# bobzhangbo2012/gnss-sdr-new

Hardware: AMD Instinct MI355X
Metric: IQ Msamples/s processed (acq+track), 32 PRN × 81 Doppler; % HBM roofline (higher is better)
Workload: dtype f32; 1 GPU; C2: GPS L1 C/A 4 Msps; per 1 ms block a 32 PRN x 81 Doppler (+-10 kHz, 250 Hz) CFAR PCPS grid + closed-loop DLL/PLL tracking (3-tap E-P-L, dll_pll_veml_tracking) of 8 channels over the same span; fs_sps=4000000, fft_size=4000, prns=32, doppler_bins=81, channels=8, taps=3, item_type=gr_complex, tracking=one continuous stream, one launch per timed region, acq_chains=2, acq_stagger=0, acq_input=each step acquires its own span of the continuous stream (new HBM addresses), carrier=exact, forward_spectra_per_block=4

## Files before the change

gnss-sdr-new_amd/csrc/acq.hip:

```cpp
#include <algorithm>
#include <cmath>
#include <cstring>
#include <memory>
#include <new>
#include <utility>

#include "acq_handle.h"
#include "acq_plans.h"
#include "gsdr_stream_internal.h"

using namespace gsdr_acq_impl;

namespace
{

int dispatch(gsdr_acq* a, const AcqView& v, const AcqOp& op)
{
    if (a->variant >= 20) return dispatch_four(a, v, op);
    if (a->variant >= 10) return dispatch_runtime(a, v, op);
    return dispatch_static(a, v, op);
}

int run_blocks(gsdr_acq* a, const AcqView& v, const void* iq, uint32_t nblocks, uint64_t stride, uint64_t stamp0,
    gsdr_acq_result* res, hipStream_t s)
// ... 226 lines not shown
{
    if (!a) return;
    gsdr::DeviceGuard g(a->device);
    if (a->stream) (void)hipStreamSynchronize(a->stream);
    for (auto& r : a->prof_recs)
        {
            (void)hipEventDestroy(r.a);
            (void)hipEventDestroy(r.b);
        }
    for (hipEvent_t e : a->prof_pool) (void)hipEventDestroy(e);
    for (int i = 0; i < gsdr_acq::kSubs; ++i)
        {
            if (a->sub_done[i]) (void)hipEventDestroy(a->sub_done[i]);
            if (a->h_res[i]) (void)hipHostFree(a->h_res[i]);
        }
    void* bufs[] = {a->st2.d_wipe, a->st2.d_freq, a->d_tw, a->d_wipe, a->d_code_fft, a->d_code_lane, a->d_code_stage, a->d_prn, a->d_X, a->d_stats, a->d_res,
        a->d_iq, a->d_grid, a->d_rowbuf, a->d_keys, a->d_psum, a->d_fscratch, a->d_dgrid, a->d_tw_sub, a->d_scratch, a->d_slots, a->d_resk, a->d_acc, a->d_acc_slots};
    for (void* p : bufs)
        if (p) (void)hipFree(p);
    if (a->stream) (void)hipStreamDestroy(a->stream);
    delete a;
}

int gsdr_acq_get_dims(const gsdr_acq* a, uint32_t* D, uint32_t* N)
{
    GSDR_REQUIRE(a, GSDR_E_ARG, "gsdr_acq_get_dims: null handle");
    if (D) *D = a->D;
    if (N) *N = a->N;
    return GSDR_OK;
}

int gsdr_acq_get_plan(const gsdr_acq* a, int32_t* variant, int32_t* nthreads, int32_t* r1, int32_t* nstages,
    int32_t radix[8])
{
    GSDR_REQUIRE(a, GSDR_E_ARG, "gsdr_acq_get_plan: null handle");
    static_assert(gsdr::fft::kMaxStages == 8, "gsdr_acq_get_plan reports 8 radices");
    const bool four = a->variant >= 20;
    const Plan& p = four ? a->plan4.sub : a->plan;
    if (variant) *variant = a->variant;
    if (nthreads) *nthreads = a->nt;
    if (r1) *r1 = four ? a->plan4.r1 : 0;
    if (nstages) *nstages = p.nstages;
    if (radix)
        for (int i = 0; i < gsdr::fft::kMaxStages; ++i) radix[i] = i < p.nstages ? p.radix[i] : 1;
    return GSDR_OK;
}

int gsdr_acq_get_split(const gsdr_acq* a, int32_t* split)
{
    GSDR_REQUIRE(a && split, GSDR_E_ARG, "gsdr_acq_get_split: null argument");
    *split = a->split;
    return GSDR_OK;
}

int gsdr_acq_set_local_codes(gsdr_acq* a, const float* codes, const uint32_t* prn, uint32_t nprn)
{
    GSDR_REQUIRE(a && codes && prn, GSDR_E_ARG, "gsdr_acq_set_local_codes: null argument");
    GSDR_REQUIRE(nprn > 0 && nprn <= a->conf.max_prns, GSDR_E_ARG, "gsdr_acq_set_local_codes: nprn %u outside [1,%u]",
        nprn, a->conf.max_prns);
    std::lock_guard<std::mutex> lk(a->mu);
    gsdr::DeviceGuard g(a->device);
    GSDR_HIP(hipMemcpyAsync(a->d_code_stage, codes, (size_t)nprn * a->consumed * sizeof(float2),
        hipMemcpyHostToDevice, a->stream));
    GSDR_HIP(hipMemcpyAsync(a->d_prn, prn, nprn * sizeof(uint32_t), hipMemcpyHostToDevice, a->stream));
    int rc = code_fft(a, 0, nprn);
    if (rc != GSDR_OK) return rc;
    GSDR_HIP(hipStreamSynchronize(a->stream));
    a->nprn = nprn;
    return GSDR_OK;
}

int gsdr_acq_set_local_code(gsdr_acq* a, uint32_t slot, const float* code, uint32_t prn)
{
    GSDR_REQUIRE(a && code, GSDR_E_ARG, "gsdr_acq_set_local_code: null argument");
    GSDR_REQUIRE(slot < a->conf.max_prns, GSDR_E_ARG, "gsdr_acq_set_local_code: slot %u outside [0,%u)",
        slot, a->conf.max_prns);
    std::lock_guard<std::mutex> lk(a->mu);
    gsdr::DeviceGuard g(a->device);
    GSDR_HIP(hipMemcpyAsync(a->d_code_stage + (size_t)slot * a->consumed, code, (size_t)a->consumed * sizeof(float2),
        hipMemcpyHostToDevice, a->stream));
    GSDR_HIP(hipMemcpyAsync(a->d_prn + slot, &prn, sizeof(uint32_t), hipMemcpyHostToDevice, a->stream));
    int rc = code_fft(a, slot, 1);
    if (rc != GSDR_OK) return rc;
    GSDR_HIP(hipStreamSynchronize(a->stream));
    if (a->nprn <= slot) a->nprn = slot + 1;
    return GSDR_OK;
}

int gsdr_acq_set_active_prns(gsdr_acq* a, uint32_t nprn)
{
    GSDR_REQUIRE(a, GSDR_E_ARG, "gsdr_acq_set_active_prns: null handle");
    GSDR_REQUIRE(nprn > 0 && nprn <= a->conf.max_prns, GSDR_E_ARG, "gsdr_acq_set_active_prns: %u outside [1,%u]", nprn,
        a->conf.max_prns);
    std::lock_guard<std::mutex> lk(a->mu);
    a->nprn = nprn;
    return GSDR_OK;
}

int gsdr_acq_set_doppler(gsdr_acq* a, int32_t doppler_max, uint32_t doppler_step, int32_t doppler_center)
{
    GSDR_REQUIRE(a, GSDR_E_ARG, "gsdr_acq_set_doppler: null handle");
    GSDR_REQUIRE(doppler_step > 0, GSDR_E_ARG, "gsdr_acq_set_doppler: doppler_step must be > 0");
    std::lock_guard<std::mutex> lk(a->mu);
    gsdr::DeviceGuard g(a->device);
    const uint32_t D = (uint32_t)std::ceil((double)(doppler_max - (-doppler_max)) / (double)doppler_step);
    GSDR_REQUIRE(a->conf.num_doppler_bins != 0 || D == a->D, GSDR_E_UNSUPPORTED,
        "gsdr_acq_set_doppler: changing the number of Doppler bins (%u -> %u) requires a new handle", a->D, D);
    a->conf.doppler_max = doppler_max;
    a->conf.doppler_step = doppler_step;
    a->conf.doppler_center = doppler_center;
    int rc = rebuild_wipeoffs(a);
    if (rc != GSDR_OK) return rc;
    compute_threshold(a);
    return GSDR_OK;
}

int gsdr_acq_set_wipeoff(gsdr_acq* a, int mode)
{
    GSDR_REQUIRE(a, GSDR_E_ARG, "gsdr_acq_set_wipeoff: null handle");
    GSDR_REQUIRE(mode == GSDR_WIPE_EXACT || mode == GSDR_WIPE_GENERIC || mode == GSDR_WIPE_AVX2, GSDR_E_ARG,
        "gsdr_acq_set_wipeoff: unknown mode %d", mode);
    std::lock_guard<std::mutex> lk(a->mu);
    gsdr::DeviceGuard g(a->device);
    a->wipe_mode = mode;
    return rebuild_wipeoffs(a);
}

int gsdr_acq_get_spectrum_reuse(const gsdr_acq* a, uint32_t* q, uint32_t* p)
{
    GSDR_REQUIRE(a, GSDR_E_ARG, "gsdr_acq_get_spectrum_reuse: null handle");
    if (q) *q = a->xm.q;
    if (p) *p = a->xm.p;
    return GSDR_OK;
}

int gsdr_acq_set_threshold(gsdr_acq* a, float threshold)
{
    GSDR_REQUIRE(a, GSDR_E_ARG, "gsdr_acq_set_threshold: null handle");
    a->threshold = threshold;
    return GSDR_OK;
}

int gsdr_acq_get_threshold(const gsdr_acq* a, float* threshold)
{
    GSDR_REQUIRE(a && threshold, GSDR_E_ARG, "gsdr_acq_get_threshold: null argument");
    *threshold = a->threshold;
    return GSDR_OK;
}

int gsdr_acq_run_device(gsdr_acq* a, const void* iq_dev, uint32_t nblocks, uint64_t stride, uint64_t stamp0,
    gsdr_acq_result* out_dev, void* stream)
{
    GSDR_REQUIRE(a && iq_dev && out_dev, GSDR_E_ARG, "gsdr_acq_run_device: null argument");
    GSDR_REQUIRE(a->nprn > 0, GSDR_E_STATE, "gsdr_acq_run_device: set_local_codes first");
    GSDR_REQUIRE(nblocks > 0 && nblocks <= a->conf.max_blocks, GSDR_E_ARG, "gsdr_acq_run_device: nblocks %u outside [1,%u]",
        nblocks, a->conf.max_blocks);
    GSDR_REQUIRE(stride >= a->consumed || nblocks == 1, GSDR_E_ARG, "gsdr_acq_run_device: block stride %llu < consumed %u",
        (unsigned long long)stride, a->consumed);
    std::lock_guard<std::mutex> lk(a->mu);
    gsdr::DeviceGuard g(a->device);
    hipStream_t s = stream ? (hipStream_t)stream : a->stream;
    return run_blocks(a, view_of(a), iq_dev, nblocks, stride, stamp0, out_dev, s);
}

int gsdr_acq_run(gsdr_acq* a, const void* iq_host, uint32_t nblocks, uint64_t stamp0, gsdr_acq_result* out)
{
    GSDR_REQUIRE(a && iq_host && out, GSDR_E_ARG, "gsdr_acq_run: null argument");
    GSDR_REQUIRE(a->nprn > 0, GSDR_E_STATE, "gsdr_acq_run: set_local_codes first");
    GSDR_REQUIRE(nblocks > 0 && nblocks <= a->conf.max_blocks, GSDR_E_ARG, "gsdr_acq_run: nblocks %u outside [1,%u]",
        nblocks, a->conf.max_blocks);
    std::lock_guard<std::mutex> lk(a->mu);
    gsdr::DeviceGuard g(a->device);
    const size_t bytes = (size_t)nblocks * a->K * a->consumed * gsdr::item_bytes(a->conf.item_type);
    GSDR_HIP(hipMemcpyAsync(a->d_iq, iq_host, bytes, hipMemcpyHostToDevice, a->stream));
    int rc = run_blocks(a, view_of(a), a->d_iq, nblocks, a->consumed, stamp0, a->d_res, a->stream);
    if (rc != GSDR_OK) return rc;
    return read_results(a, out, (size_t)nblocks * a->nprn);
}

int gsdr_acq_run_stream(gsdr_acq* a, gsdr_stream* ring, uint64_t first_sample, uint32_t nblocks, uint64_t stamp0,
    gsdr_acq_result* out)
{
    GSDR_REQUIRE(a && ring && out, GSDR_E_ARG, "gsdr_acq_run_stream: null argument");
    GSDR_REQUIRE(a->nprn > 0, GSDR_E_STATE, "gsdr_acq_run_stream: set_local_codes first");
    GSDR_REQUIRE(nblocks > 0 && nblocks <= a->conf.max_blocks, GSDR_E_ARG,
        "gsdr_acq_run_stream: nblocks %u outside [1,%u]", nblocks, a->conf.max_blocks);
    GSDR_REQUIRE(gsdr::stream_item_type(ring) == a->conf.item_type, GSDR_E_ARG,
        "gsdr_acq_run_stream: ring item type %d != acquisition item type %d", gsdr::stream_item_type(ring),
        a->conf.item_type);
    GSDR_REQUIRE(gsdr::stream_device(ring) == a->device, GSDR_E_ARG,
        "gsdr_acq_run_stream: ring on device %d, acquisition handle on device %d", gsdr::stream_device(ring), a->device);
    std::lock_guard<std::mutex> lk(a->mu);
    gsdr::DeviceGuard g(a->device);
    int rc = run_ring(a, ring, first_sample, nblocks, stamp0);
    if (rc != GSDR_OK) return rc;
    return read_results(a, out, (size_t)nblocks * a->nprn);
}

int gsdr_acq_submit_stream(gsdr_acq* a, gsdr_stream* ring, uint64_t first_sample, uint32_t nblocks, uint64_t stamp0)
{
    GSDR_REQUIRE(a && ring, GSDR_E_ARG, "gsdr_acq_submit_stream: null argument");
    GSDR_REQUIRE(a->nprn > 0, GSDR_E_STATE, "gsdr_acq_submit_stream: set_local_codes first");
    GSDR_REQUIRE(nblocks > 0 && nblocks <= a->conf.max_blocks, GSDR_E_ARG,
        "gsdr_acq_submit_stream: nblocks %u outside [1,%u]", nblocks, a->conf.max_blocks);
    GSDR_REQUIRE(gsdr::stream_item_type(ring) == a->conf.item_type, GSDR_E_ARG,
        "gsdr_acq_submit_stream: ring item type %d != acquisition item type %d", gsdr::stream_item_type(ring),
        a->conf.item_type);
    GSDR_REQUIRE(gsdr::stream_device(ring) == a->device, GSDR_E_ARG,
        "gsdr_acq_submit_stream: ring on device %d, acquisition handle on device %d", gsdr::stream_device(ring), a->device);
    std::lock_guard<std::mutex> lk(a->mu);
    GSDR_REQUIRE(a->sub_count < gsdr_acq::kSubs, GSDR_E_STATE,
        "gsdr_acq_submit_stream: %d submissions in flight, collect the oldest first", gsdr_acq::kSubs);
    gsdr::DeviceGuard g(a->device);
    const int slot = (a->sub_head + a->sub_count) % gsdr_acq::kSubs;
    if (!a->h_res[slot])
        {
            GSDR_HIP(hipHostMalloc(&a->h_res[slot],
                (size_t)a->conf.max_blocks * a->conf.max_prns * sizeof(gsdr_acq_result), hipHostMallocDefault));
            GSDR_HIP(hipEventCreateWithFlags(&a->sub_done[slot], hipEventDisableTiming));
        }
    int rc = run_ring(a, ring, first_sample, nblocks, stamp0);
    if (rc != GSDR_OK) return rc;
    GSDR_HIP(hipMemcpyAsync(a->h_res[slot], a->d_res, (size_t)nblocks * a->nprn * sizeof(gsdr_acq_result),
        hipMemcpyDeviceToHost, a->stream));
    GSDR_HIP(hipEventRecord(a->sub_done[slot], a->stream));
    a->sub_blocks[slot] = nblocks;
    a->sub_nprn[slot] = a->nprn;
    a->sub_count++;
    return GSDR_OK;
}

int gsdr_acq_collect(gsdr_acq* a, gsdr_acq_result* out, uint32_t* nblocks, uint32_t* nprn)
{
    GSDR_REQUIRE(a && out, GSDR_E_ARG, "gsdr_acq_collect: null argument");
    std::lock_guard<std::mutex> lk(a->mu);
    GSDR_REQUIRE(a->sub_count > 0, GSDR_E_STATE, "gsdr_acq_collect: nothing submitted");
    gsdr::DeviceGuard g(a->device);
    const int slot = a->sub_head;
    a->sub_head = (a->sub_head + 1) % gsdr_acq::kSubs;
    a->sub_count--;
    GSDR_HIP(hipEventSynchronize(a->sub_done[slot]));
    std::memcpy(out, a->h_res[slot], (size_t)a->sub_blocks[slot] * a->sub_nprn[slot] * sizeof(gsdr_acq_result));
    if (nblocks) *nblocks = a->sub_blocks[slot];
    if (nprn) *nprn = a->sub_nprn[slot];
    return GSDR_OK;
}

int gsdr_acq_run_dwell(gsdr_acq* a, const void* iq_host, uint32_t dwell, uint64_t stamp, gsdr_acq_result* out)
{
    GSDR_REQUIRE(a && iq_host && out, GSDR_E_ARG, "gsdr_acq_run_dwell: null argument");
    GSDR_REQUIRE(a->nprn > 0, GSDR_E_STATE, "gsdr_acq_run_dwell: set_local_codes first");
    GSDR_REQUIRE(dwell < a->conf.max_dwells, GSDR_E_ARG, "gsdr_acq_run_dwell: dwell %u outside [0,%u)", dwell,
        a->conf.max_dwells);
    std::lock_guard<std::mutex> lk(a->mu);
    gsdr::DeviceGuard g(a->device);
    if (!a->d_dgrid)
        GSDR_HIP(hipMalloc(&a->d_dgrid, (size_t)a->conf.max_prns * a->D * a->eff * sizeof(float)));
    GSDR_HIP(hipMemcpyAsync(a->d_iq, iq_host, (size_t)a->consumed * gsdr::item_bytes(a->conf.item_type),
        hipMemcpyHostToDevice, a->stream));
    AcqOp op{AcqOp::Dwell};
    op.dwell = dwell;
    op.stamp0 = stamp;
    op.res = a->d_res;
    op.s = a->stream;
    int rc = dispatch(a, view_of(a), op);
    if (rc != GSDR_OK) return rc;
    return read_results(a, out, a->nprn);
}

int gsdr_acq_dump_spectra(gsdr_acq* a, const void* iq_host, float* spectra_host)
{
    GSDR_REQUIRE(a && iq_host && spectra_host, GSDR_E_ARG, "gsdr_acq_dump_spectra: null argument");
    std::lock_guard<std::mutex> lk(a->mu);
    gsdr::DeviceGuard g(a->device);
    GSDR_HIP(hipMemcpyAsync(a->d_iq, iq_host, (size_t)a->consumed * gsdr::item_bytes(a->conf.item_type),
        hipMemcpyHostToDevice, a->stream));
    int rc = dispatch(a, view_of(a), AcqOp{AcqOp::DumpSpectra});
    if (rc != GSDR_OK) return rc;
    for (uint32_t d = 0; d < a->D; ++d)
        GSDR_HIP(hipMemcpyAsync(spectra_host + (size_t)d * a->N * 2, a->d_X + a->xm.off(0, d),
            (size_t)a->N * sizeof(float2), hipMemcpyDeviceToHost, a->stream));
    GSDR_HIP(hipStreamSynchronize(a->stream));
    return GSDR_OK;
}

int gsdr_acq_dump_grid(gsdr_acq* a, const void* iq_host, uint32_t prn_slot, float* grid_host)
{
    GSDR_REQUIRE(a && iq_host && grid_host, GSDR_E_ARG, "gsdr_acq_dump_grid: null argument");
    GSDR_REQUIRE(prn_slot < a->nprn, GSDR_E_ARG, "gsdr_acq_dump_grid: prn_slot %u >= nprn %u", prn_slot, a->nprn);
    std::lock_guard<std::mutex> lk(a->mu);
    gsdr::DeviceGuard g(a->device);
    GSDR_HIP(hipMemcpyAsync(a->d_iq, iq_host, (size_t)a->consumed * gsdr::item_bytes(a->conf.item_type),
        hipMemcpyHostToDevice, a->stream));
    AcqOp op{AcqOp::DumpGrid};
    op.prn_slot = prn_slot;
    int rc = dispatch(a, view_of(a), op);
    if (rc != GSDR_OK) return rc;
    GSDR_HIP(hipMemcpyAsync(grid_host, a->d_grid, (size_t)a->D * a->N * sizeof(float), hipMemcpyDeviceToHost,
        a->stream));
    GSDR_HIP(hipStreamSynchronize(a->stream));
    return GSDR_OK;
}

int gsdr_acq_dump_grid_step_two(gsdr_acq* a, const void* iq_host, uint32_t prn_slot, float doppler_center_hz,
    float* grid_host)
{
    GSDR_REQUIRE(a && iq_host && grid_host, GSDR_E_ARG, "gsdr_acq_dump_grid_step_two: null argument");
    GSDR_REQUIRE(prn_slot < a->nprn, GSDR_E_ARG, "gsdr_acq_dump_grid_step_two: prn_slot %u >= nprn %u", prn_slot,
        a->nprn);
    GSDR_REQUIRE(a->st2.nbins > 0, GSDR_E_STATE, "gsdr_acq_dump_grid_step_two: gsdr_acq_set_step_two first");
    GSDR_REQUIRE(a->st2.nbins <= a->D, GSDR_E_UNSUPPORTED,
        "gsdr_acq_dump_grid_step_two: %u narrow bins exceed the grid buffer's %u rows", a->st2.nbins, a->D);
    std::lock_guard<std::mutex> lk(a->mu);
    gsdr::DeviceGuard g(a->device);
    const uint32_t nb = a->st2.nbins;
    std::vector<float> freqs(nb);
    step_two_freqs(a, doppler_center_hz, freqs.data());
    GSDR_HIP(hipMemcpyAsync(a->d_iq, iq_host, (size_t)a->consumed * gsdr::item_bytes(a->conf.item_type),
        hipMemcpyHostToDevice, a->stream));
    GSDR_HIP(hipMemcpyAsync(a->st2.d_freq, freqs.data(), nb * sizeof(float), hipMemcpyHostToDevice, a->stream));
    int rc = launch_wipeoff(a, a->st2.d_wipe, nb, a->st2.d_freq);
    if (rc != GSDR_OK) return rc;
    AcqView v = view_of(a);
    v.D = nb;
    v.nprn = 1;
    v.wipe = a->st2.d_wipe;
    v.code_fft = a->d_code_fft + (size_t)prn_slot * a->N;
    v.code_lane = a->d_code_lane ? a->d_code_lane + (size_t)prn_slot * a->N : nullptr;
    v.xm = XMap{nb, 0u, a->N};
    rc = dispatch(a, v, AcqOp{AcqOp::DumpGrid});
    if (rc != GSDR_OK) return rc;
    GSDR_HIP(hipMemcpyAsync(grid_host, a->d_grid, (size_t)nb * a->N * sizeof(float), hipMemcpyDeviceToHost,
        a->stream));
    GSDR_HIP(hipStreamSynchronize(a->stream));
    return GSDR_OK;
}

int gsdr_acq_set_step_two(gsdr_acq* a, uint32_t num_doppler_bins_step2, float doppler_step2, float pfa2)
{
    GSDR_REQUIRE(a, GSDR_E_ARG, "gsdr_acq_set_step_two: null handle");
    GSDR_REQUIRE(num_doppler_bins_step2 > 0, GSDR_E_ARG, "gsdr_acq_set_step_two: zero bins");
    GSDR_REQUIRE(num_doppler_bins_step2 <= a->D * a->conf.max_blocks, GSDR_E_UNSUPPORTED,
        "gsdr_acq_set_step_two: %u bins exceed the handle's spectrum capacity (%u bins x %u blocks)",
        num_doppler_bins_step2, a->D, a->conf.max_blocks);
    std::lock_guard<std::mutex> lk(a->mu);
    gsdr::DeviceGuard g(a->device);
    GSDR_HIP(hipStreamSynchronize(a->stream));
    if (a->st2.d_wipe) (void)hipFree(a->st2.d_wipe);
    if (a->st2.d_freq) (void)hipFree(a->st2.d_freq);
    a->st2.d_wipe = nullptr;
    a->st2.d_freq = nullptr;
    const size_t rows = (size_t)a->conf.max_prns * num_doppler_bins_step2;
    GSDR_HIP(hipMalloc(&a->st2.d_wipe, rows * a->N * sizeof(float2)));
    GSDR_HIP(hipMalloc(&a->st2.d_freq, rows * sizeof(float)));
    a->st2.nbins = num_doppler_bins_step2;
    a->st2.step = doppler_step2;
    a->st2.pfa2 = (pfa2 <= 0.0f || pfa2 > 1.0f) ? a->conf.pfa : pfa2;
    return GSDR_OK;
}

int gsdr_acq_get_step_two_threshold(const gsdr_acq* a, float* threshold)
{
    GSDR_REQUIRE(a && threshold, GSDR_E_ARG, "gsdr_acq_get_step_two_threshold: null argument");
    GSDR_REQUIRE(a->st2.nbins > 0, GSDR_E_STATE, "gsdr_acq_get_step_two_threshold: gsdr_acq_set_step_two first");
    *threshold = step_two_threshold(a);
    return GSDR_OK;
}

int gsdr_acq_run_step_two(gsdr_acq* a, const void* iq_host, uint32_t nsel, const uint32_t* prn_slots,
    const float* doppler_center_hz, const float* coarse_input_power, uint64_t stamp, gsdr_acq_result* out)
{
    GSDR_REQUIRE(a && iq_host && prn_slots && doppler_center_hz && coarse_input_power && out, GSDR_E_ARG,
        "gsdr_acq_run_step_two: null argument");
    GSDR_REQUIRE(a->st2.nbins > 0, GSDR_E_STATE, "gsdr_acq_run_step_two: gsdr_acq_set_step_two first");
    GSDR_REQUIRE(nsel > 0 && nsel <= a->nprn, GSDR_E_ARG, "gsdr_acq_run_step_two: %u PRNs outside [1,%u]", nsel,
        a->nprn);
    for (uint32_t i = 0; i < nsel; ++i)
        GSDR_REQUIRE(prn_slots[i] < a->nprn, GSDR_E_ARG, "gsdr_acq_run_step_two: slot %u >= nprn %u", prn_slots[i],
            a->nprn);
    std::lock_guard<std::mutex> lk(a->mu);
    gsdr::DeviceGuard g(a->device);
    const uint32_t nb = a->st2.nbins;
    std::vector<float> freqs((size_t)nsel * nb);
    for (uint32_t i = 0; i < nsel; ++i) step_two_freqs(a, doppler_center_hz[i], freqs.data() + (size_t)i * nb);
    GSDR_HIP(hipMemcpyAsync(a->d_iq, iq_host, (size_t)a->K * a->consumed * gsdr::item_bytes(a->conf.item_type),
        hipMemcpyHostToDevice, a->stream));
    GSDR_HIP(hipMemcpyAsync(a->st2.d_freq, freqs.data(), freqs.size() * sizeof(float), hipMemcpyHostToDevice,
        a->stream));
    int rc = launch_wipeoff(a, a->st2.d_wipe, nsel * nb, a->st2.d_freq);
    const float thr = step_two_threshold(a);
    for (uint32_t i = 0; i < nsel && rc == GSDR_OK; ++i)
        {
            const AcqView v{nb, 1, a->st2.d_wipe + (size_t)i * nb * a->N, a->d_code_fft + (size_t)prn_slots[i] * a->N,
                a->d_code_lane ? a->d_code_lane + (size_t)prn_slots[i] * a->N : nullptr, a->d_prn + prn_slots[i], XMap{nb, 0u, a->N}, true, doppler_center_hz[i], coarse_input_power[i], thr};
            rc = run_blocks(a, v, a->d_iq, 1, a->consumed, stamp, a->d_res + i, a->stream);
        }
    if (rc != GSDR_OK) return rc;
    return read_results(a, out, nsel);
}

int gsdr_acq_set_cu_mask(gsdr_acq* a, const uint32_t* mask, int n_words)
{
    GSDR_REQUIRE(a, GSDR_E_ARG, "gsdr_acq_set_cu_mask: null handle");
    std::lock_guard<std::mutex> lk(a->mu);
    gsdr::DeviceGuard g(a->device);
    return gsdr::replace_stream(&a->stream, mask, n_words);
}

int gsdr_acq_set_profiling(gsdr_acq* a, int enable)
{
    GSDR_REQUIRE(a, GSDR_E_ARG, "gsdr_acq_set_profiling: null handle");
    std::lock_guard<std::mutex> lk(a->mu);
    a->profiling = enable != 0;
    if (a->profiling)
        {
            gsdr::DeviceGuard g(a->device);
            while (a->prof_pool.size() + 2 * a->prof_recs.size() < 1024)
                {
                    hipEvent_t e = nullptr;
                    if (hipEventCreate(&e) != hipSuccess) break;
                    a->prof_pool.push_back(e);
                }
        }
    return GSDR_OK;
}

int gsdr_acq_read_profile_ex(gsdr_acq* a, double* stage_ms, uint32_t* launches, double* stage_busy_ms)
{
    GSDR_REQUIRE(a && stage_ms && launches, GSDR_E_ARG, "gsdr_acq_read_profile: null argument");
    std::lock_guard<std::mutex> lk(a->mu);
    gsdr::DeviceGuard g(a->device);
    for (int i = 0; i < 4; ++i)
        {
            stage_ms[i] = 0.0;
            launches[i] = 0;
            if (stage_busy_ms) stage_busy_ms[i] = 0.0;
        }
    std::vector<std::pair<double, double>> iv[4];
    hipEvent_t ref = a->prof_recs.empty() ? nullptr : a->prof_recs.front().a;
    for (auto& r : a->prof_recs)
        {
            GSDR_HIP(hipEventSynchronize(r.b));
            float ms = 0.0f, t0 = 0.0f, t1 = 0.0f;
            GSDR_HIP(hipEventElapsedTime(&ms, r.a, r.b));
            GSDR_HIP(hipEventElapsedTime(&t0, ref, r.a));
            GSDR_HIP(hipEventElapsedTime(&t1, ref, r.b));
            stage_ms[r.stage] += ms;
            launches[r.stage] += 1;
            iv[r.stage].emplace_back(t0, t1);
        }
    if (stage_busy_ms)
        for (int i = 0; i < 4; ++i)
            {
                std::sort(iv[i].begin(), iv[i].end());
                double busy = 0.0, lo = 0.0, hi = -1e300;
                for (const auto& x : iv[i])
                    {
                        if (x.first > hi)
                            {
                                if (hi > lo) busy += hi - lo;
                                lo = x.first;
                                hi = x.second;
                            }
                        else if (x.second > hi)
                            hi = x.second;
                    }
                if (hi > lo) busy += hi - lo;
                stage_busy_ms[i] = busy;
            }
    for (auto& r : a->prof_recs)
        {
            a->prof_pool.push_back(r.a);
            a->prof_pool.push_back(r.b);
        }
    a->prof_recs.clear();
    return GSDR_OK;
}

int gsdr_acq_read_profile_intervals(gsdr_acq* a, const void* ref_event, int stage, double* start_ms, double* end_ms,
    uint32_t max_n, uint32_t* n)
{
    GSDR_REQUIRE(a && ref_event && n && (max_n == 0 || (start_ms && end_ms)), GSDR_E_ARG,
        "gsdr_acq_read_profile_intervals: null argument");
    GSDR_REQUIRE(stage >= 0 && stage < 4, GSDR_E_ARG, "gsdr_acq_read_profile_intervals: stage %d", stage);
    std::lock_guard<std::mutex> lk(a->mu);
    gsdr::DeviceGuard g(a->device);
    hipEvent_t ref = (hipEvent_t)const_cast<void*>(ref_event);
    uint32_t k = 0;
    for (auto& r : a->prof_recs)
        {
            if (r.stage != stage) continue;
            if (k < max_n)
                {
                    GSDR_HIP(hipEventSynchronize(r.b));
                    float t0 = 0.0f, t1 = 0.0f;
                    GSDR_HIP(hipEventElapsedTime(&t0, ref, r.a));
                    GSDR_HIP(hipEventElapsedTime(&t1, ref, r.b));
                    start_ms[k] = t0;
                    end_ms[k] = t1;
                }
            ++k;
        }
    *n = k;
    return GSDR_OK;
}

int gsdr_acq_read_profile(gsdr_acq* a, double* stage_ms, uint32_t* launches)
{
    return gsdr_acq_read_profile_ex(a, stage_ms, launches, nullptr);
}

}
```

gnss-sdr-new_amd/csrc/acq_common.hip:

```cpp
#include <cmath>
#include <cstdlib>
#include <string>

#include "acq_handle.h"

namespace
{

__device__ __forceinline__ float2 cephes_sincos_avx2(float x0)
{
    const float FOPI = 1.27323954473516f;
    const float DP1 = -0.78515625f, DP2 = -2.4187564849853515625e-4f, DP3 = -3.77489497744594108e-8f;
    const float C0 = 2.443315711809948E-005f, C1 = -1.388731625493765E-003f, C2 = 4.166664568298827E-002f;
    const float S0 = -1.9515295891E-4f, S1 = 8.3321608736E-3f, S2 = -1.6666654611E-1f;
    const uint32_t bits = __float_as_uint(x0);
    bool sign_sin = (bits >> 31) != 0;
    float x = __uint_as_float(bits & 0x7fffffffu);
    float y = __fmul_rn(x, FOPI);
    int32_t j = (int32_t)y;
    j = (j + 1) & ~1;
    y = (float)j;
    const bool swap = (j & 4) != 0;
    const bool poly = (j & 2) == 0;
    x = __fadd_rn(x, __fmul_rn(y, DP1));
    x = __fadd_rn(x, __fmul_rn(y, DP2));
    x = __fadd_rn(x, __fmul_rn(y, DP3));
    const bool sign_cos = ((~(j - 2)) & 4) != 0;
    sign_sin = sign_sin != swap;
    const float z = __fmul_rn(x, x);
    float yc = __fmul_rn(C0, z);
    yc = __fadd_rn(yc, C1);
    yc = __fmul_rn(yc, z);
    yc = __fadd_rn(yc, C2);
    yc = __fmul_rn(yc, z);
    yc = __fmul_rn(yc, z);
    yc = __fsub_rn(yc, __fmul_rn(z, 0.5f));
    yc = __fadd_rn(yc, 1.0f);
    float ys = __fmul_rn(S0, z);
    ys = __fadd_rn(ys, S1);
    ys = __fmul_rn(ys, z);
    ys = __fadd_rn(ys, S2);
    ys = __fmul_rn(ys, z);
    ys = __fmul_rn(ys, x);
    ys = __fadd_rn(ys, x);
    const float sv = poly ? ys : yc, cv = poly ? yc : ys;
    return make_float2(sign_cos ? -cv : cv, sign_sin ? -sv : sv);
}

__global__ void __launch_bounds__(256) acq_wipeoff_kernel(float2* __restrict__ wipe, uint32_t N, float fs,
    int32_t doppler_max, int32_t doppler_center, int32_t doppler_step, int32_t doppler_bias,
    const float* __restrict__ freqs, int mode)
{
    const uint32_t d = blockIdx.x;
    float2* row = wipe + (size_t)d * N;
    const int32_t doppler = -doppler_max + doppler_center + doppler_step * (int32_t)d;
    const float freq = freqs ? freqs[d] : (float)(doppler_bias + doppler);
    if (mode == GSDR_WIPE_EXACT)
        {
            for (uint32_t i = threadIdx.x; i < N; i += blockDim.x)
                {
                    const double t = (double)freq * (double)i / (double)fs;
                    double s, c;
                    sincos(-6.283185307179586 * (t - floor(t)), &s, &c);
                    row[i] = make_float2((float)c, (float)s);
                }
            return;
        }
    const float phase_step = __fdiv_rn(__fmul_rn(6.283185307179586f, freq), fs);
    const float inc = -phase_step;
    if (mode == GSDR_WIPE_AVX2)
        {
            const uint32_t iters = N / 8;
            if (threadIdx.x < 8)
                {
                    const uint32_t k = threadIdx.x;
                    float ph = k == 0 ? 0.0f : __fmul_rn((float)k, inc);
                    const float inc8 = __fmul_rn(8.0f, inc);
                    for (uint32_t it = 0; it < iters; ++it)
                        {
                            row[8 * it + k].x = ph;
                            ph = __fadd_rn(ph, inc8);
                        }
                }
            else if (threadIdx.x == 8)
                {
                    float ph = __fmul_rn(inc, (float)(iters * 8));
                    for (uint32_t i = iters * 8; i < N; ++i)
                        {
                            row[i].x = ph;
                            ph = __fadd_rn(ph, inc);
                        }
                }
            __syncthreads();
            for (uint32_t i = threadIdx.x; i < N; i += blockDim.x)
                {
                    if (i < iters * 8)
                        row[i] = cephes_sincos_avx2(row[i].x);
                    else
                        {
                            float s, c;
                            sincosf(row[i].x, &s, &c);
                            row[i] = make_float2(c, s);
                        }
                }
            return;
        }
    if (threadIdx.x == 0)
        {
            float ph = 0.0f;
            for (uint32_t i = 0; i < N; ++i)
                {
                    row[i].x = ph;
                    ph = __fadd_rn(ph, inc);
                }
        }
    __syncthreads();
    for (uint32_t i = threadIdx.x; i < N; i += blockDim.x)
        {
            float s, c;
            sincosf(row[i].x, &s, &c);
            row[i] = make_float2(c, s);
        }
}

__global__ void __launch_bounds__(64) acq_reduce_dwell_kernel(const RowStat* __restrict__ stats,
    gsdr_acq_result* __restrict__ resk, gsdr_acq_result* __restrict__ res, const uint32_t* __restrict__ prn_ids,
    AcqParams ap, uint64_t stamp0, uint64_t block_stride)
{
    const uint32_t bp = blockIdx.x;
    const uint32_t b = bp / ap.P, p = bp - b * ap.P;
    const uint32_t K = ap.dwells;
    bool done = false;
    for (uint32_t k = 0; k < K && !done; ++k)
        {
            const RowStat* s = stats + ((size_t)bp * K + k) * ap.D;
            float m = -1.0f;
            uint32_t dsel = 0xffffffffu, tsel = 0;
            for (uint32_t d = threadIdx.x; d < ap.D; d += 64)
                {
                    RowStat r = s[d];
                    if (r.max > m)
                        {
                            m = r.max;
                            dsel = d;
                            tsel = r.idx;
                        }
                }
#pragma unroll
            for (int off = 32; off > 0; off >>= 1)
                {
                    float om = __shfl_xor(m, off);
                    uint32_t od = __shfl_xor(dsel, off);
                    uint32_t ot = __shfl_xor(tsel, off);
                    if (stat_better(om, od, m, dsel))
                        {
                            m = om;
                            dsel = od;
                            tsel = ot;
                        }
                }
            gsdr_acq_result r;
            r.prn = prn_ids[p];
            r.doppler_index = dsel;
            r.code_phase = tsel;
            r.doppler_hz = doppler_of(ap, dsel);
            r.peak = m;
            r.second_peak = 0.0f;
            r.input_power = 0.0f;
            r.test_statistic = 0.0f;
            r.acq_delay_samples = (double)fmodf((float)tsel, ap.samples_per_code);
            r.samplestamp = stamp0 + (uint64_t)(b * K + k) * block_stride;
            r.positive = 0;
            r.num_dwells = (int32_t)(k + 1);
            if (ap.cfar)
                {
                    const uint32_t opp = (dsel + ap.D / 2) % ap.D;
                    const float acc = s[opp].sum;
                    const float ip = ap.step_two ? ap.ip2
                                                 : (float)((double)(acc / (float)(int32_t)ap.eff) / 2.0 / (double)(k + 1));
                    r.input_power = ip;
                    r.test_statistic = m / ip;
                    r.positive = r.test_statistic > ap.threshold ? 1 : 0;
                    done = r.positive || k + 1 == K;
                    if (done && threadIdx.x == 0) res[bp] = r;
                }
            if (threadIdx.x == 0) resk[(size_t)bp * K + k] = r;
        }
}

__global__ void acq_decide_kernel(const gsdr_acq_result* __restrict__ resk, gsdr_acq_result* __restrict__ res,
    uint32_t K, uint32_t n)
{
    const uint32_t bp = blockIdx.x * blockDim.x + threadIdx.x;
    if (bp >= n) return;
    uint32_t k = 0;
    while (k + 1 < K && !resk[(size_t)bp * K + k].positive) ++k;
    res[bp] = resk[(size_t)bp * K + k];
}

__global__ void __launch_bounds__(256) acq_code_lane_order_kernel(const float2* __restrict__ src,
    float2* __restrict__ dst, uint32_t N, int nb1, int r1)
{
    const float2* in = src + (size_t)blockIdx.x * N;
    float2* out = dst + (size_t)blockIdx.x * N;
    for (uint32_t i = threadIdx.x; i < N; i += blockDim.x) out[lane_order_slot((int)i, nb1, r1)] = in[i];
}

__global__ void __launch_bounds__(256) acq_grid_second_peak_kernel(const float* __restrict__ grid,
    gsdr_acq_result* __restrict__ res, AcqParams ap)
{
    __shared__ RowStat scratch[4];
    const uint32_t p = blockIdx.x;
    const uint32_t d = res[p].doppler_index;
    const int32_t ti = (int32_t)res[p].code_phase;
    const int32_t E = (int32_t)ap.N;
    int32_t e1 = ti - (int32_t)ap.samples_per_chip;
    int32_t e2 = ti + (int32_t)ap.samples_per_chip;
    if (e1 < 0)
        e1 = E + e1;
    else if (e2 >= E)
        e2 = e2 - E;
    const float* row = grid + ((size_t)p * ap.D + d) * ap.eff;
    float best = 0.0f, sum = 0.0f;
    uint32_t bidx = 0;
    for (uint32_t j = threadIdx.x; j < ap.eff; j += 256)
        {
            const int32_t jj = (int32_t)j;
            const bool excluded = (e1 < e2) ? (jj >= e1 && jj < e2) : (jj >= e1 || jj < e2);
            const float m = excluded ? 0.0f : row[j];
            if (stat_better(m, j, best, bidx))
                {
                    best = m;
                    bidx = j;
                }
        }
    block_reduce_stat<256>(best, bidx, sum, scratch);
    if (threadIdx.x == 0)
        {
            gsdr_acq_result r = res[p];
            r.second_peak = best;
            r.test_statistic = r.peak / best;
            r.positive = r.test_statistic > ap.threshold ? 1 : 0;
            res[p] = r;
        }
}

__global__ void __launch_bounds__(64) acq_reduce_kernel(const RowStat* __restrict__ stats,
    gsdr_acq_result* __restrict__ res, const uint32_t* __restrict__ prn_ids, AcqParams ap, uint64_t stamp0,
    uint64_t block_stride)
{
    const uint32_t bp = blockIdx.x;
    const uint32_t b = bp / ap.P, p = bp - b * ap.P;
    const RowStat* s = stats + (size_t)bp * ap.D;
    float m = -1.0f;
    uint32_t dsel = 0xffffffffu, tsel = 0;
    for (uint32_t d = threadIdx.x; d < ap.D; d += 64)
        {
            RowStat r = s[d];
            if (r.max > m)
                {
                    m = r.max;
                    dsel = d;
                    tsel = r.idx;
                }
        }
#pragma unroll
    for (int off = 32; off > 0; off >>= 1)
        {
            float om = __shfl_xor(m, off);
            uint32_t od = __shfl_xor(dsel, off);
            uint32_t ot = __shfl_xor(tsel, off);
            if (stat_better(om, od, m, dsel))
                {
                    m = om;
                    dsel = od;
                    tsel = ot;
                }
        }
    if (threadIdx.x != 0) return;
    gsdr_acq_result r;
    r.prn = prn_ids[p];
    r.doppler_index = dsel;
    r.code_phase = tsel;
    r.doppler_hz = doppler_of(ap, dsel);
    r.peak = m;
    r.second_peak = 0.0f;
    r.input_power = 0.0f;
    r.test_statistic = 0.0f;
    r.acq_delay_samples = (double)fmodf((float)tsel, ap.samples_per_code);
    r.samplestamp = stamp0 + (uint64_t)b * block_stride;
    r.positive = 0;
    r.num_dwells = (int32_t)ap.counter;
    if (ap.cfar)
        {
            const uint32_t opp = (dsel + ap.D / 2) % ap.D;
            const float acc = s[opp].sum;
            const float ip =
                ap.step_two ? ap.ip2 : (float)((double)(acc / (float)(int32_t)ap.eff) / 2.0 / (double)ap.counter);
            r.input_power = ip;
            r.test_statistic = m / ip;
            r.positive = r.test_statistic > ap.threshold ? 1 : 0;
        }
    res[bp] = r;
}

int env_int(const char* name, int dflt)
{
    const char* e = std::getenv(name);
    return e ? std::atoi(e) : dflt;
}

}

namespace gsdr_acq_impl
{

#ifndef GSDR_ACQ_PPW_DEFAULT
#define GSDR_ACQ_PPW_DEFAULT 1
#endif
#ifndef GSDR_ACQ_QPW_DEFAULT
#define GSDR_ACQ_QPW_DEFAULT 2
#endif

AcqEnv read_acq_env()
{
    AcqEnv e;
    if (const char* w = std::getenv("GSDR_ACQ_WIPE"))
        {
            const std::string m(w);
            e.wipe_mode = m == "generic" ? GSDR_WIPE_GENERIC : (m == "avx2" ? GSDR_WIPE_AVX2 : GSDR_WIPE_EXACT);
        }
    e.xshift = env_int("GSDR_ACQ_XSHIFT", 1) != 0;
    e.four_generic = env_int("GSDR_ACQ_FOUR_GENERIC", 0) != 0;
    e.split = env_int("GSDR_ACQ_SPLIT", 1) != 0;
    e.split_arg = env_int("GSDR_ACQ_SPLIT_ARG", 1) != 0;
    e.qpw = env_int("GSDR_ACQ_QPW", GSDR_ACQ_QPW_DEFAULT);
    e.ppw = env_int("GSDR_ACQ_PPW", GSDR_ACQ_PPW_DEFAULT);
    e.corr_variant = env_int("GSDR_ACQ_CORR_VARIANT", -1);
    return e;
}

AcqView view_of(const gsdr_acq* a)
{
    return AcqView{a->D, a->nprn, a->d_wipe, a->d_code_fft, a->d_code_lane, a->d_prn, a->xm, false, 0.0f, 0.0f, 0.0f};
}

AcqParams params_of(const gsdr_acq* a, const AcqView& v)
{
    AcqParams ap{};
    ap.xm = v.xm;
    ap.N = a->N;
    ap.consumed = a->consumed;
    ap.lead_zeros = a->lead;
    ap.D = v.D;
    ap.P = v.nprn;
    ap.doppler_max = a->conf.doppler_max;
    ap.doppler_center = a->conf.doppler_center;
    ap.doppler_step = (int32_t)a->conf.doppler_step;
    ap.samples_per_code = a->conf.samples_per_code;
    ap.samples_per_chip = a->conf.samples_per_chip;
    ap.dwells = a->K;
    ap.threshold = a->threshold;
    ap.cfar = a->conf.pfa > 0.0f ? 1 : 0;
    ap.eff = a->eff;
    ap.out_off = a->N - a->eff;
    ap.counter = a->K;
    if (v.step_two)
        {
            ap.step_two = 1;
            ap.center2 = v.center2;
            ap.step2 = a->st2.step;
            ap.half2 = (float)std::floor((double)a->st2.nbins / 2.0);
            ap.ip2 = v.ip2;
            ap.threshold = v.threshold2;
        }
    return ap;
}

static XMap grid_xmap(const gsdr_acq* a)
{
    XMap plain{a->D, 0u, a->N};
    if (a->wipe_mode != GSDR_WIPE_EXACT || !a->env.xshift) return plain;
    const int64_t fs = a->conf.fs_in;
    if (fs <= 0) return plain;
    int64_t num = (int64_t)a->conf.doppler_step * (int64_t)a->N, den = fs;
    int64_t g0 = num, g1 = den;
    while (g1)
        {
            const int64_t t = g0 % g1;
            g0 = g1;
            g1 = t;
        }
    if (g0 <= 0) return plain;
    const int64_t p = num / g0, q = den / g0;
    if (q < 1 || 2 * q > (int64_t)a->D) return plain;
    const int64_t ext = ((int64_t)(a->D - 1) / q) * p;
    if (ext > (int64_t)a->N) return plain;
    if (q * ((int64_t)a->N + ext) > (int64_t)a->D * (int64_t)a->N) return plain;
    return XMap{(uint32_t)q, (uint32_t)p, (uint32_t)(a->N + ext)};
}

int launch_wipeoff(gsdr_acq* a, float2* wipe, uint32_t rows, const float* freqs)
{
    const gsdr_acq_conf& c = a->conf;
    const bool g = !freqs;
    hipLaunchKernelGGL(acq_wipeoff_kernel, dim3(rows), dim3(256), 0, a->stream, wipe, a->N, (float)c.fs_in,
        g ? c.doppler_max : 0, g ? c.doppler_center : 0, g ? (int32_t)c.doppler_step : 0, g ? c.doppler_bias : 0, freqs,
        a->wipe_mode);
    GSDR_HIP(hipGetLastError());
    return GSDR_OK;
}

int rebuild_wipeoffs(gsdr_acq* a)
{
    a->xm = grid_xmap(a);
    const int rc = launch_wipeoff(a, a->d_wipe, a->xm.q, nullptr);
    if (rc != GSDR_OK) return rc;
    GSDR_HIP(hipStreamSynchronize(a->stream));
    return GSDR_OK;
}

int launch_reduce(gsdr_acq* a, const AcqParams& ap, bool dwells, uint32_t nblocks, gsdr_acq_result* res,
    const uint32_t* prn, uint64_t stamp0, uint64_t stride, hipStream_t s)
{
    if (dwells)
        hipLaunchKernelGGL(acq_reduce_dwell_kernel, dim3(nblocks * ap.P), dim3(64), 0, s, a->d_stats, a->d_resk, res,
            prn, ap, stamp0, stride);
    else
        hipLaunchKernelGGL(acq_reduce_kernel, dim3(nblocks * ap.P), dim3(64), 0, s, a->d_stats, res, prn, ap, stamp0,
            stride);
    GSDR_HIP(hipGetLastError());
    return GSDR_OK;
}

int launch_decide(gsdr_acq* a, uint32_t n, gsdr_acq_result* res, hipStream_t s)
{
    hipLaunchKernelGGL(acq_decide_kernel, dim3((n + 255) / 256), dim3(256), 0, s, a->d_resk, res, a->K, n);
    GSDR_HIP(hipGetLastError());
    return GSDR_OK;
}

int launch_code_lane_order(gsdr_acq* a, uint32_t first_slot, uint32_t nslots)
{
    const size_t off = (size_t)first_slot * a->N;
    hipLaunchKernelGGL(acq_code_lane_order_kernel, dim3(nslots), dim3(256), 0, a->stream, a->d_code_fft + off,
        a->d_code_lane + off, a->N, a->lane_nb1, a->lane_r1);
    GSDR_HIP(hipGetLastError());
    return GSDR_OK;
}

int launch_grid_second_peak(gsdr_acq* a, const AcqParams& ap, gsdr_acq_result* res, hipStream_t s)
{
    hipLaunchKernelGGL(acq_grid_second_peak_kernel, dim3(ap.P), dim3(256), 0, s, a->d_dgrid, res, ap);
    GSDR_HIP(hipGetLastError());
    return GSDR_OK;
}

void compute_threshold(gsdr_acq* a)
{
    const float pfa = a->conf.pfa;
    if (pfa <= 0.0f) return;
    const int num_bins = (int)(a->eff * a->D);
    const double p = std::pow(1.0 - (double)pfa, 1.0 / (double)(float)num_bins);
    a->threshold = (float)(2.0 * gsdr::gamma_p_inv_int(2 * (int)a->conf.max_dwells, p));
}

float step_two_threshold(const gsdr_acq* a)
{
    const float pfa = a->st2.pfa2;
    if (pfa <= 0.0f) return a->threshold;
    const int num_bins = (int)(a->eff * a->st2.nbins);
    const double p = std::pow(1.0 - (double)pfa, 1.0 / (double)(float)num_bins);
    return (float)(2.0 * gsdr::gamma_p_inv_int(2 * (int)a->conf.max_dwells, p));
}

}
```

gnss-sdr-new_amd/csrc/acq_handle.h:

```cpp
#pragma once
#include <mutex>
#include <type_traits>
#include <vector>

#include "acq_kernels.h"

struct AcqEnv
{
    int wipe_mode{GSDR_WIPE_EXACT};
    bool xshift{true}, four_generic{false}, split{true}, split_arg{true};
    int qpw{0}, ppw{0};
    int corr_variant{-1};
};

struct gsdr_acq
{
    int device{0};
    gsdr_acq_conf conf{};
    AcqEnv env{};
    uint32_t N{0}, D{0}, consumed{0}, lead{0};
    uint32_t K{1};
    int wipe_mode{GSDR_WIPE_EXACT};
    gsdr_acq_impl::XMap xm{};
    uint32_t eff{0};
    bool general{false};
    gsdr_acq_result* d_resk{nullptr};
    float* d_acc{nullptr};
    uint32_t* d_acc_slots{nullptr};
    int acc_words{0};
    float threshold{0.0f};
    int nt{256};
    int variant{0};
    int corr_variant{0};
    int split{0};
    int corr_stat{0};
    size_t corr_lds_bytes{0};
    int lane_nb1{0}, lane_r1{0};
    gsdr::fft::Plan plan{};
    gsdr::fft::Plan4 plan4{};
    size_t lds_bytes{0};
    hipStream_t stream{nullptr};
    float2* d_tw{nullptr};
    float2* d_wipe{nullptr};
    float2* d_code_fft{nullptr};
    float2* d_code_lane{nullptr};
    float2* d_code_stage{nullptr};
    uint32_t* d_prn{nullptr};
    uint32_t nprn{0};
    float2* d_X{nullptr};
    gsdr_acq_impl::RowStat* d_stats{nullptr};
    gsdr_acq_result* d_res{nullptr};
    static constexpr int kSubs = 2;
    gsdr_acq_result* h_res[kSubs]{};
    hipEvent_t sub_done[kSubs]{};
    uint32_t sub_blocks[kSubs]{}, sub_nprn[kSubs]{};
    int sub_head{0}, sub_count{0};
    void* d_iq{nullptr};
    float* d_grid{nullptr};
    float* d_rowbuf{nullptr};
    unsigned long long* d_keys{nullptr};
    float* d_psum{nullptr};
    float2* d_fscratch{nullptr};
    float* d_dgrid{nullptr};
    float2* d_tw_sub{nullptr};
    float2* d_scratch{nullptr};
    uint32_t* d_slots{nullptr};
    struct ProfRec
    {
        hipEvent_t a, b;
        int stage;
    };
    bool profiling{false};
    std::vector<ProfRec> prof_recs;
    std::vector<hipEvent_t> prof_pool;
    struct StepTwo
    {
        uint32_t nbins{0};
        float step{0.0f};
        float pfa2{0.0f};
        float2* d_wipe{nullptr};
        float* d_freq{nullptr};
    } st2;
    std::mutex mu;
};

namespace gsdr_acq_impl
{

struct AcqView
{
    uint32_t D, nprn;
    const float2* wipe;
    const float2* code_fft;
    const float2* code_lane;
    const uint32_t* prn;
    XMap xm;
    bool step_two;
    float center2, ip2, threshold2;
};

struct AcqOp
{
    enum Kind
    {
        Run,
        CodeFft,
        DumpSpectra,
        DumpGrid,
        SetAttrs,
        Dwell
    } kind;
    const void* iq{nullptr};
    uint32_t nblocks{0};
    uint64_t stride{0}, stamp0{0};
    gsdr_acq_result* res{nullptr};
    hipStream_t s{nullptr};
    uint32_t first_slot{0}, nslots{0}, prn_slot{0}, dwell{0};
};

inline int default_pk_variant(uint32_t N)
{
    switch (N)
        {
        case 4000: return 99;
        case 16000: return 94;
        case 8000: return 61;
        case 2000: return 62;
        default: return 0;
        }
}

template <class F>
auto with_item_type(int it, F&& f)
{
    if (it == GSDR_ITEM_GR_COMPLEX) return f(std::integral_constant<int, GSDR_ITEM_GR_COMPLEX>{});
    if (it == GSDR_ITEM_CSHORT) return f(std::integral_constant<int, GSDR_ITEM_CSHORT>{});
    return f(std::integral_constant<int, GSDR_ITEM_IBYTE>{});
}
constexpr int kItemTypes[] = {GSDR_ITEM_GR_COMPLEX, GSDR_ITEM_CSHORT, GSDR_ITEM_IBYTE};

inline int set_max_lds(const void* kernel, size_t bytes)
{
    GSDR_HIP(hipFuncSetAttribute(kernel, hipFuncAttributeMaxDynamicSharedMemorySize, (int)bytes));
    return GSDR_OK;
}

AcqEnv read_acq_env();
AcqView view_of(const gsdr_acq* a);
AcqParams params_of(const gsdr_acq* a, const AcqView& v);
int rebuild_wipeoffs(gsdr_acq* a);
void compute_threshold(gsdr_acq* a);
float step_two_threshold(const gsdr_acq* a);
int launch_wipeoff(gsdr_acq* a, float2* wipe, uint32_t rows, const float* freqs);
int launch_reduce(gsdr_acq* a, const AcqParams& ap, bool dwells, uint32_t nblocks, gsdr_acq_result* res,
    const uint32_t* prn, uint64_t stamp0, uint64_t stride, hipStream_t s);
int launch_decide(gsdr_acq* a, uint32_t n, gsdr_acq_result* res, hipStream_t s);
int launch_grid_second_peak(gsdr_acq* a, const AcqParams& ap, gsdr_acq_result* res, hipStream_t s);
int launch_code_lane_order(gsdr_acq* a, uint32_t first_slot, uint32_t nslots);

int launch_corr_variant(gsdr_acq* a, const AcqView& v, uint32_t nblocks, hipStream_t s);
int launch_argmax_variant(gsdr_acq* a, const AcqView& v, uint32_t nblocks, gsdr_acq_result* res, hipStream_t s);
int launch_forward_pk(gsdr_acq* a, const AcqView& v, const void* iq, uint32_t nblocks, uint64_t stride, hipStream_t s);
int setup_corr_variant(gsdr_acq* a, int id);
int setup_split(gsdr_acq* a);
int launch_split(gsdr_acq* a, const AcqView& v, uint32_t nblocks, hipStream_t s);
int launch_split_argmax(gsdr_acq* a, const AcqView& v, uint32_t nblocks, gsdr_acq_result* res, hipStream_t s);
int dispatch_static(gsdr_acq* a, const AcqView& v, const AcqOp& op);
int dispatch_runtime(gsdr_acq* a, const AcqView& v, const AcqOp& op);
int dispatch_four(gsdr_acq* a, const AcqView& v, const AcqOp& op);

}
```

gnss-sdr-new_amd/csrc/acq_kernels.h:

```cpp
#pragma once
#include <hip/hip_runtime.h>

#include <type_traits>

#include "fft_4step.h"
#include "fft_lds.h"
#include "fft_multi.h"
#include "fft_pk.h"
#include "fft_plan.h"
#include "gsdr_internal.h"

namespace gsdr_acq_impl
{

struct RowStat
{
    float max;
    uint32_t idx;
    float sum;
    uint32_t pad;
};

struct XMap
{
// ... 3 lines not shown
    __host__ __device__ __forceinline__ size_t off(uint32_t bk, uint32_t d) const
    {
        const uint32_t a = d / q, c = d - a * q;
        return ((size_t)bk * q + c) * stride + (size_t)a * p;
    }
};

struct AcqParams
{
    XMap xm;
    uint32_t N;
    uint32_t consumed;
    uint32_t lead_zeros;
    uint32_t D;
    uint32_t P;
    int32_t doppler_max;
    int32_t doppler_center;
    int32_t doppler_step;
    float samples_per_code;
    uint32_t samples_per_chip;
    uint32_t dwells;
    float threshold;
    int32_t cfar;
    uint32_t eff;
    uint32_t out_off;
    int32_t step_two;
    float center2;
    float step2;
    float half2;
    float ip2;
    uint32_t counter;
};

}

namespace
{

using gsdr::fft::Plan;
using gsdr_acq_impl::AcqParams;
using gsdr_acq_impl::RowStat;
using gsdr_acq_impl::XMap;

__device__ __forceinline__ int32_t doppler_of(const AcqParams& ap, uint32_t d)
{
    if (ap.step_two) return (int32_t)gsdr::add_rn(ap.center2, gsdr::mul_rn(gsdr::sub_rn((float)d, ap.half2), ap.step2));
    return -ap.doppler_max + ap.doppler_center + ap.doppler_step * (int32_t)d;
}

template <int IT>
__device__ __forceinline__ float2 load_item(const void* __restrict__ p, size_t i)
{
    if constexpr (IT == GSDR_ITEM_GR_COMPLEX)
        {
            return reinterpret_cast<const float2*>(p)[i];
        }
    else if constexpr (IT == GSDR_ITEM_CSHORT)
        {
            short2 s = reinterpret_cast<const short2*>(p)[i];
            return make_float2((float)s.x, (float)s.y);
        }
    else
        {
            char2 s = reinterpret_cast<const char2*>(p)[i];
            return make_float2((float)s.x, (float)s.y);
        }
}

__device__ __forceinline__ bool stat_better(float am, uint32_t ai, float bm, uint32_t bi)
{
    return am > bm || (am == bm && ai < bi);
}

template <int NT>
__device__ __forceinline__ void block_reduce_stat(float& m, uint32_t& idx, float& sum, RowStat* scratch)
{
#pragma unroll
    for (int off = 32; off > 0; off >>= 1)
        {
            float om = __shfl_xor(m, off);
            uint32_t oi = __shfl_xor(idx, off);
            float os = __shfl_xor(sum, off);
            if (stat_better(om, oi, m, idx))
                {
                    m = om;
                    idx = oi;
                }
            sum += os;
        }
    constexpr int NW = NT / 64;
    const int lane = threadIdx.x & 63, wave = threadIdx.x >> 6;
    if (NW > 1)
        {
            if (lane == 0) scratch[wave] = RowStat{m, idx, sum, 0};
            __syncthreads();
            if (threadIdx.x == 0)
                {
                    for (int w = 1; w < NW; ++w)
                        {
                            RowStat s = scratch[w];
                            if (stat_better(s.max, s.idx, m, idx))
                                {
                                    m = s.max;
                                    idx = s.idx;
                                }
                            sum += s.sum;
                        }
                }
        }
}

template <class PT>
__global__ void __launch_bounds__(PT::NT) acq_code_fft_kernel(const float2* __restrict__ codes,
    float2* __restrict__ code_fft, const float2* __restrict__ tw, typename PT::PlanT plan, uint32_t consumed, uint32_t lead)
{
    extern __shared__ float2 lds[];
    const uint32_t p = blockIdx.x;
    const float2* c = codes + (size_t)p * consumed;
    float2* out = code_fft + (size_t)p * plan.n;
    const int valid = (int)plan.n - (int)lead;
    auto load = [&](int i) -> float2 {
        int k = i - (int)lead;
        return (k >= 0 && k < valid) ? c[k] : make_float2(0.f, 0.f);
    };
    auto store = [&](int i, float2 v) { out[i] = v; };
    PT::run(plan, lds, tw, load, store);
}

template <class PT, int IT>
__global__ void __launch_bounds__(PT::NT) acq_forward_kernel(const void* __restrict__ iq, uint64_t block_stride,
    const float2* __restrict__ wipe, float2* __restrict__ X, const float2* __restrict__ tw, typename PT::PlanT plan,
    uint32_t consumed, XMap xm)
{
    extern __shared__ float2 lds[];
    const uint32_t b = blockIdx.x, d = blockIdx.y;
    const size_t base = (size_t)b * block_stride;
    const float2* w = wipe + (size_t)d * plan.n;
    float2* out = X + xm.off(b, d);
    const int ext = (int)(xm.stride - plan.n);
    auto load = [&](int i) -> float2 {
        if (i >= (int)consumed) return make_float2(0.f, 0.f);
        return gsdr::fft::cmul(load_item<IT>(iq, base + i), w[i]);
    };
    auto store = [&](int i, float2 v) {
        out[i] = v;
        if (i < ext) out[plan.n + i] = v;
    };
    PT::run(plan, lds, tw, load, store);
}

template <class PT, class = void>
struct requires_subplan : std::false_type
{
};
template <class PT>
struct requires_subplan<PT, std::void_t<typename PT::SubPlan>> : std::true_type
{
};

template <class PT, int IT>
__global__ void __launch_bounds__(256) acq_forward4_cols_kernel(const void* __restrict__ iq, uint64_t block_stride,
    const float2* __restrict__ wipe, float2* __restrict__ scratch, const float2* __restrict__ tw, uint32_t consumed,
    uint32_t D)
{
    using gsdr::pk::c2;
    constexpr int R = PT::R, N2 = PT::N2, N = PT::N;
    const uint32_t row = blockIdx.y;
    const uint32_t b = row / D, d = row - (row / D) * D;
    const int n2 = (int)(blockIdx.x * 256 + threadIdx.x);
    if (n2 >= N2) return;
    const size_t base = (size_t)b * block_stride;
    const float2* w = wipe + (size_t)d * N;
    c2 v[R];
#pragma unroll
    for (int n1 = 0; n1 < R; ++n1)
        {
            const int i = n1 * N2 + n2;
            v[n1] = i < (int)consumed ? gsdr::pk::from(gsdr::fft::cmul(load_item<IT>(iq, base + i), w[i]))
                                      : c2{0.0f, 0.0f};
        }
    gsdr::pk::Dft<R>::run(v);
    const gsdr::fft::ColTwiddles<R> cw(tw, n2);
    float2* out = scratch + (size_t)row * N;
    out[n2] = gsdr::pk::to(v[0]);
#pragma unroll
    for (int k1 = 1; k1 < R; ++k1) out[(size_t)k1 * N2 + n2] = gsdr::pk::to(gsdr::pk::mul(v[k1], cw(k1)));
}

template <class PT>
__global__ void __launch_bounds__(PT::NT) acq_forward4_rows_kernel(const float2* __restrict__ scratch,
    float2* __restrict__ X, const float2* __restrict__ tw_sub, uint32_t nrows, uint32_t xstride)
{
    using gsdr::pk::c2;
    using SP = typename PT::SubPlan;
    constexpr int R = PT::R, N2 = PT::N2, N = PT::N;
    extern __shared__ float2 lds_raw[];
    const uint32_t id = blockIdx.x, full = nrows >> 3;
    uint32_t row, k1;
    if (id < full * 8u * R)
        {
            const uint32_t xcd = id & 7u, slot = id >> 3;
            row = (slot / R) * 8u + xcd;
            k1 = slot - (slot / R) * R;
        }
    else
        {
            const uint32_t t = id - full * 8u * R;
            row = full * 8u + t / R;
            k1 = t - (t / R) * R;
        }
    const c2* rk = reinterpret_cast<const c2*>(scratch) + (size_t)row * N + (size_t)k1 * N2;
    float2* out = X + (size_t)row * xstride;
    const int ext = (int)(xstride - (uint32_t)N);
    auto ld = [&](int, int, int i) -> c2 { return rk[i]; };
    auto st = [&](int k2, c2 v, int) {
        const int k = (int)k1 + R * k2;
        out[k] = gsdr::pk::to(v);
        if (k < ext) out[N + k] = gsdr::pk::to(v);
    };
    SP::template run<false>(reinterpret_cast<c2*>(lds_raw), tw_sub, ld, st, [] {});
}

template <class PT, bool GRID>
__global__ void __launch_bounds__(PT::NT) acq_correlate_kernel(const float2* __restrict__ X,
    const float2* __restrict__ code_fft, RowStat* __restrict__ stats, float* __restrict__ grid,
    const float2* __restrict__ tw, typename PT::PlanT plan, uint32_t D, uint32_t P, uint32_t prn_slot_for_grid, XMap xm)
{
    extern __shared__ float2 lds[];
    RowStat* scratch = reinterpret_cast<RowStat*>(lds + gsdr::fft::lds_elems_dev(plan));
    const uint32_t N = plan.n;
    uint32_t d, p, b;
    if (GRID)
        {
            d = blockIdx.x;
            p = prn_slot_for_grid;
            b = blockIdx.y;
        }
    else
        {
            const uint32_t nrows = gridDim.y * D;
            const uint32_t id = blockIdx.y * gridDim.x + blockIdx.x;
            const uint32_t full = nrows >> 3;
            uint32_t row;
            if (id < full * 8u * P)
                {
                    const uint32_t xcd = id & 7u, slot = id >> 3;
                    row = (slot / P) * 8u + xcd;
                    p = slot - (slot / P) * P;
                }
            else
                {
                    const uint32_t t = id - full * 8u * P;
                    row = full * 8u + t / P;
                    p = t - (t / P) * P;
                }
            b = row / D;
            d = row - b * D;
        }
    const float2* x = X + xm.off(b, d);
    const float2* c = code_fft + (size_t)p * N;
    float best = -1.0f, sum = 0.0f;
    uint32_t bidx = 0xffffffffu;
    auto load = [&](int i) -> float2 {
        float2 a = x[i], k = c[i];
        return make_float2(a.x * k.x + a.y * k.y, a.x * k.y - a.y * k.x);
    };
    auto store = [&](int i, float2 v) {
        const float m = v.x * v.x + v.y * v.y;
        if (GRID) grid[(size_t)d * N + i] = m;
        if (stat_better(m, (uint32_t)i, best, bidx))
            {
                best = m;
                bidx = (uint32_t)i;
            }
        sum += m;
    };
    PT::run(plan, lds, tw, load, store);
    if (!GRID)
        {
            block_reduce_stat<PT::NT>(best, bidx, sum, scratch);
            if (threadIdx.x == 0) stats[((size_t)b * P + p) * D + d] = RowStat{best, bidx, sum, 0};
        }
}

enum CodeSrc
{
    kCodeVgpr = 0,
    kCodeDirect = 1,
    kCodeLds = 2,
    kCodeLane = 3
};

constexpr int lane_order_slot(int i, int nb1, int r1) { return (i % nb1) * r1 + i / nb1; }
constexpr bool lane_order_bijective(int nb1, int r1)
{
    for (int i = 0; i < nb1 * r1; ++i)
        {
            const int s = lane_order_slot(i, nb1, r1);
            if (s < 0 || s >= nb1 * r1 || (s % r1) * nb1 + s / r1 != i) return false;
        }
    return true;
}

template <class MP, int CS>
constexpr size_t pk_fft_bytes()
{
    constexpr size_t piece = (size_t)(MP::NT / 64) * 1024;
    return CS == kCodeLds || CS == kCodeLane ? (MP::lds_bytes() + piece - 1) / piece * piece : MP::lds_bytes();
}

enum TwSrc
{
    kTwGlobal = 0,
    kTwLds = 1
};

constexpr int tw_mid_index(int r, int k, int ns2) { return (r - 1) * ns2 + k; }
constexpr int tw_mid_elems(int tw, int r2, int ns2) { return tw == kTwLds ? (r2 - 1) * ns2 : 0; }
constexpr int tw_last_elems(int tw, int ns3) { return tw == kTwLds ? ns3 : 0; }

template <class MP, int CS>
constexpr size_t pk_tw_offset()
{
    return pk_fft_bytes<MP, CS>() + (size_t)2 * (MP::NT / 64) * sizeof(RowStat);
}
template <class MP, int TW>
constexpr size_t pk_tw_bytes()
{
    constexpr int R2 = MP::N / (MP::R1 * MP::RL);
    return (size_t)(tw_mid_elems(TW, R2, MP::R1) + tw_last_elems(TW, MP::NSL)) * sizeof(gsdr::pk::c2);
}
template <class MP, int CS, int TW>
constexpr size_t pk_corr_lds_bytes()
{
    return pk_tw_offset<MP, CS>() + pk_tw_bytes<MP, TW>();
}

template <int R2, int NS2>
struct TwLds
{
    const gsdr::pk::c2* mid;
    const gsdr::pk::c2* last;
    template <int R>
    struct Mid
    {
        gsdr::pk::c2 w[R - 1];
    };
    template <int R, int I>
    __device__ __forceinline__ static void read_powers(Mid<R>& m, unsigned a)
    {
        asm volatile("ds_read_b64 %0, %1 offset:%2" : "=v"(m.w[I - 1]) : "v"(a), "n"(tw_mid_index(I, 0, NS2) * 8));
        if constexpr (I + 1 < R) read_powers<R, I + 1>(m, a);
    }
    template <int R, int Ns>
    __device__ __forceinline__ Mid<R> load_middle(int k) const
    {
        static_assert(R == R2 && Ns == NS2 && NS2 <= 32, "the plan's middle stage");
        Mid<R> m;
        read_powers<R, 1>(m, (unsigned)(uintptr_t)(gsdr_lvoid*)const_cast<gsdr::pk::c2*>(mid + k));
        return m;
    }
    template <int R>
    __device__ __forceinline__ void middle(gsdr::pk::c2* v, const Mid<R>& m) const
    {
        Mid<R> t = m;
        asm volatile("s_waitcnt lgkmcnt(0)" ::: "memory");
#pragma unroll
        for (int r = 1; r < R; ++r) asm volatile("" : "+v"(t.w[r - 1]));
#pragma unroll
        for (int r = 1; r < R; ++r) v[r] = gsdr::pk::mul(v[r], t.w[r - 1]);
    }
    __device__ __forceinline__ gsdr::pk::c2 last_root(int k) const { return last[k]; }
};

template <class MP, int PG, int WPE, int STAT, int CS, int TW = kTwGlobal>
__global__ void __launch_bounds__(MP::NT) __attribute__((amdgpu_waves_per_eu(WPE))) acq_correlate_pk_kernel(const float2* __restrict__ X,
    const float2* __restrict__ code_fft, RowStat* __restrict__ stats, const float2* __restrict__ tw, uint32_t D,
    uint32_t P, uint32_t nblocks, XMap xm)
{
    static_assert(PG > 0, "PRN group");
    static_assert(CS == kCodeVgpr || CS == kCodeDirect || CS == kCodeLds || CS == kCodeLane, "code source");
    static_assert(TW == kTwGlobal || TW == kTwLds, "twiddle source");
    constexpr bool PREFETCH = CS == kCodeVgpr;
    constexpr bool LANE = CS == kCodeLane;
    constexpr bool STAGED = CS == kCodeLds || LANE;
    constexpr bool TABLES = TW != kTwGlobal;
    static_assert(!TABLES || (STAGED && MP::nstages == 3 && MP::TWP), "twiddle tables: a staged three-stage TWP plan");
    static_assert(!STAGED || pk_fft_bytes<MP, CS>() % ((MP::NT / 64) * 1024) == 0, "whole pieces fill the padded buffer");
    static_assert(pk_tw_offset<MP, CS>() >= pk_fft_bytes<MP, CS>() + 2 * (MP::NT / 64) * sizeof(RowStat), "tables behind the scratch");
    static_assert(!TABLES || pk_tw_offset<MP, CS>() % sizeof(gsdr::pk::c2) == 0, "table alignment");
    static_assert(!TABLES || pk_corr_lds_bytes<MP, CS, TW>() <= 40960, "LDS of four workgroups per CU");
    static_assert(!LANE || (MP::BPT1 == 1 && lane_order_bijective(MP::NB1, MP::R1)), "lane order of the first stage");
    constexpr int XT = CS == kCodeLds ? (MP::R1 + 4) / 5 : 0;
    constexpr int RA = LANE ? 5 : 0;
    static_assert(STAT == 1 || STAT == 2, "row statistic 1 (max + sum) or 2 (max)");
    using gsdr::pk::c2;
    constexpr int NT = MP::NT;
    constexpr int NW = NT / 64;
    constexpr int R1 = MP::R1, BPT1 = MP::BPT1, NB1 = MP::NB1;
    constexpr uint32_t N = MP::N;
    extern __shared__ float2 lds_raw[];
    c2* lds = reinterpret_cast<c2*>(lds_raw);
    RowStat* scratch = reinterpret_cast<RowStat*>(lds_raw + pk_fft_bytes<MP, CS>() / sizeof(float2));
    const uint32_t G = (P + PG - 1) / PG;
    const uint32_t nrows = nblocks * D;
    const uint32_t id = blockIdx.x;
    const uint32_t full = nrows >> 3;
    uint32_t row, g;
    if (id < full * 8u * G)
        {
            const uint32_t xcd = id & 7u, slot = id >> 3;
            row = (slot / G) * 8u + xcd;
            g = slot - (slot / G) * G;
        }
    else
        {
            const uint32_t t = id - full * 8u * G;
            row = full * 8u + t / G;
            g = t - (t / G) * G;
        }
    const uint32_t b = row / D, d = row - (row / D) * D;
    const uint32_t p0 = g * PG;
    const int np = (int)min((uint32_t)PG, P - p0);
    constexpr int R2 = MP::N / (MP::R1 * MP::RL);
    using Tws = std::conditional_t<TABLES, TwLds<R2, MP::R1>, gsdr::pk::TwGlobal>;
    Tws tws{};
    (void)tws;
    if constexpr (TABLES)
        {
            tws.mid = lds + pk_tw_offset<MP, CS>() / sizeof(c2);
            tws.last = tws.mid + tw_mid_elems(TW, R2, MP::R1);
        }
    const auto xrs = __builtin_amdgcn_make_buffer_rsrc(
        const_cast<float2*>(X) + xm.off(b, d), 0, (int)(N * sizeof(c2)), 0x00020000);
    const auto crs = __builtin_amdgcn_make_buffer_rsrc(
        const_cast<float2*>(code_fft) + (size_t)p0 * N, 0, (int)((size_t)np * N * sizeof(c2)), 0x00020000);
    auto bload = [](decltype(xrs) rs, int voff, int soff) -> c2 {
        const auto u = __builtin_amdgcn_raw_buffer_load_b64(rs, voff, soff, 0);
        return c2{__uint_as_float(u[0]), __uint_as_float(u[1])};
    };
    c2 xr[BPT1][R1], cr[BPT1][R1];
#pragma unroll
    for (int bb = 0; bb < BPT1; ++bb)
        {
            const int j = (int)threadIdx.x + bb * NT;
            const int j0 = (int)(threadIdx.x & ~63u) + bb * NT;
            if (NB1 % NT == 0 || j0 < NB1)
                {
                    const int jj = min(j, NB1 - 1);
#pragma unroll
                    for (int r = 0; r < R1 - XT; ++r)
                        {
                            xr[bb][r] = bload(xrs, jj * 8, r * NB1 * 8);
                            if constexpr (PREFETCH) cr[bb][r] = bload(crs, jj * 8, r * NB1 * 8);
                        }
                }
        }
    auto stage_code = [&](int qn) {
        constexpr int PIECE = NW * 1024;
        constexpr int PIECES = (int)(pk_fft_bytes<MP, CS>() / PIECE);
        const int wave = __builtin_amdgcn_readfirstlane((int)(threadIdx.x >> 6));
        char* dst = reinterpret_cast<char*>(lds_raw) + wave * 1024;
        const int voff = (int)threadIdx.x * 16;
#pragma unroll
        for (int k = 0; k < PIECES; ++k)
            __builtin_amdgcn_raw_ptr_buffer_load_lds(crs, (gsdr_lvoid*)(dst + k * PIECE), 16, voff,
                qn * (int)(N * 8) + k * PIECE, 0, 0);
    };
    if constexpr (STAGED)
        {
            stage_code(0);
            if constexpr (TABLES)
                {
                    c2* tmid = lds + pk_tw_offset<MP, CS>() / sizeof(c2);
                    c2* tlast = tmid + tw_mid_elems(TW, R2, MP::R1);
#pragma unroll
                    for (int k = (int)threadIdx.x; k < MP::NSL; k += NT) tlast[k] = gsdr::pk::from(tw[k]);
                    for (int k = (int)threadIdx.x; k < MP::R1; k += NT)
                        {
                            const c2 w1 = gsdr::pk::from(tw[k * MP::RL]);
                            c2 w = w1;
#pragma unroll
                            for (int r = 1; r < R2; ++r)
                                {
                                    if (r > 1) w = gsdr::pk::mul(w, w1);
                                    tmid[tw_mid_index(r, k, MP::R1)] = w;
                                }
                        }
                }
            asm volatile("s_waitcnt vmcnt(0)" ::: "memory");
            __syncthreads();
        }
    for (int q = 0; q < np; ++q)
        {
            {
                    float rmax = 0.0f, sum = 0.0f;
                    if constexpr (XT > 0)
                        {
#pragma unroll
                            for (int bb = 0; bb < BPT1; ++bb)
                                {
                                    const int jj = min((int)threadIdx.x + bb * NT, NB1 - 1);
#pragma unroll
                                    for (int r = R1 - XT; r < R1; ++r) xr[bb][r] = bload(xrs, jj * 8, r * NB1 * 8);
                                }
                            __builtin_amdgcn_sched_barrier(0);
                        }
                    c2 cb[2][RA > 0 ? RA : 1];
                    auto load = [&](int bb, int r, int i) -> c2 {
                        if constexpr (PREFETCH)
                            return gsdr::pk::conj_mul(xr[bb][r], cr[bb][r]);
                        else if constexpr (STAGED)
                            {
                                if (XT > 0 && r == R1 - XT) __builtin_amdgcn_sched_barrier(0);
                                if constexpr (LANE)
                                    {
                                        const c2* row = lds + min((int)threadIdx.x, NB1 - 1) * R1;
                                        if (r % RA == 0)
                                            {
                                                if (r == 0)
                                                    {
#pragma unroll
                                                        for (int k = 0; k < RA; ++k) cb[0][k] = row[k];
                                                    }
                                                const int g = r / RA + 1;
#pragma unroll
                                                for (int k = 0; k < RA; ++k)
                                                    if (g * RA + k < R1) cb[g & 1][k] = row[g * RA + k];
                                                __builtin_amdgcn_sched_barrier(0);
                                            }
                                        return gsdr::pk::conj_mul(xr[bb][r], cb[(r / RA) & 1][r % RA]);
                                    }
                                return gsdr::pk::conj_mul(xr[bb][r], lds[i]);
                            }
                        else
                            return gsdr::pk::conj_mul(xr[bb][r], bload(crs, i * 8, (int)(q * N * 8)));
                    };
                    auto hook = [&]() {
                        if (PREFETCH && q + 1 < np)
                            {
#pragma unroll
                                for (int bb = 0; bb < BPT1; ++bb)
                                    {
                                        const int j = (int)threadIdx.x + bb * NT;
                                        if (NB1 % NT == 0 || j < NB1)
                                            {
#pragma unroll
                                                for (int r = 0; r < R1; ++r)
                                                    cr[bb][r] = bload(crs, j * 8, (int)((q + 1) * N * 8) + r * NB1 * 8);
                                            }
                                    }
                            }
                    };
                    auto store = [&](int, c2 v, int) {
                        const float m = __builtin_fmaf(v.x, v.x, v.y * v.y);
                        rmax = __builtin_fmaxf(rmax, m);
                        if constexpr (STAT == 1) sum += m;
                    };
                    if constexpr (STAGED)
                        {
                            auto pre = [&]() { __syncthreads(); };
                            auto mid = [&]() {
                                if (q + 1 < np) stage_code(q + 1);
                            };
                            if constexpr (LANE)
                                MP::template run<false, true>(lds, tw, load, store, hook, gsdr::pk::NoHook{}, mid, tws);
                            else
                                MP::template run<false>(lds, tw, load, store, hook, pre, mid);
                        }
                    else
                        MP::template run<false>(lds, tw, load, store, hook);
                    rmax = gsdr::wave_max(rmax);
                    if constexpr (STAT == 1)
                        {
#pragma unroll
                            for (int off = 32; off > 0; off >>= 1) sum += __shfl_xor(sum, off);
                        }
                    RowStat* sc = scratch + (q & 1) * NW;
                    const int lane = threadIdx.x & 63, wave = threadIdx.x >> 6;
                    if (lane == 0) sc[wave] = RowStat{rmax, 0u, sum, 0};
                    if constexpr (STAGED) asm volatile("s_waitcnt vmcnt(0)" ::: "memory");
                    __syncthreads();
                    if (threadIdx.x == 0)
                        {
                            RowStat best = sc[0];
#pragma unroll
                            for (int w = 1; w < NW; ++w)
                                {
                                    best.max = __builtin_fmaxf(best.max, sc[w].max);
                                    best.sum += sc[w].sum;
                                }
                            stats[((size_t)b * P + p0 + q) * D + d] = best;
                        }
            }
        }
}

template <class PT>
__global__ void __launch_bounds__(PT::NT) acq_argmax_four_kernel(const float2* __restrict__ X,
    const float2* __restrict__ code_fft, gsdr_acq_result* __restrict__ res, const float2* __restrict__ tw,
    typename PT::PlanT plan, AcqParams ap)
{
    constexpr int NT = PT::NT;
    constexpr int NW = NT / 64;
    extern __shared__ float2 lds[];
    __shared__ unsigned long long s_key[NW];
    __shared__ float s_sum[NW];
    const uint32_t bp = blockIdx.x;
    const uint32_t b = bp / ap.P, p = bp - b * ap.P;
    const uint32_t N = ap.N;
    const uint32_t d = res[bp].doppler_index;
    if (d >= ap.D) return;
    const float2* c = code_fft + (size_t)p * N;
    const int off = (int)ap.out_off;
    auto row_load = [&](const float2* x) {
        return [x, c](int i) -> float2 {
            const float2 a = x[i], k = c[i];
            return make_float2(a.x * k.x + a.y * k.y, a.x * k.y - a.y * k.x);
        };
    };
    unsigned long long key = 0ull;
    auto store = [&](int i, float2 v) {
        const int j = i - off;
        if (j < 0) return;
        const float m = __builtin_fmaf(v.x, v.x, v.y * v.y);
        const unsigned long long k = ((unsigned long long)__float_as_uint(m) << 32) | (0xffffffffu - (uint32_t)j);
        key = k > key ? k : key;
    };
    PT::run(plan, lds, tw, row_load(X + ap.xm.off(b, d)), store);
#pragma unroll
    for (int o = 32; o > 0; o >>= 1)
        {
            const unsigned long long t = __shfl_xor(key, o);
            key = t > key ? t : key;
        }
    const int lane = threadIdx.x & 63, wave = threadIdx.x >> 6;
    if (lane == 0) s_key[wave] = key;
    __syncthreads();
#pragma unroll
    for (int w = 0; w < NW; ++w) key = s_key[w] > key ? s_key[w] : key;
    const uint32_t idx = 0xffffffffu - (uint32_t)(key & 0xffffffffu);
    const float peak = __uint_as_float((uint32_t)(key >> 32));
    float ip = 0.0f;
    if (ap.cfar && !ap.step_two)
        {
            const uint32_t opp = (d + ap.D / 2) % ap.D;
            const float2* xo = X + ap.xm.off(b, opp);
            float acc = 0.0f;
            if (off == 0)
                {
                    for (uint32_t i = threadIdx.x; i < N; i += NT)
                        {
                            const float2 a = xo[i], k = c[i];
                            const float yr = a.x * k.x + a.y * k.y, yi = a.x * k.y - a.y * k.x;
                            acc = __builtin_fmaf(yr, yr, __builtin_fmaf(yi, yi, acc));
                        }
                }
            else
                {
                    auto sum_store = [&](int i, float2 v) {
                        if (i >= off) acc += __builtin_fmaf(v.x, v.x, v.y * v.y);
                    };
                    __syncthreads();
                    PT::run(plan, lds, tw, row_load(xo), sum_store);
                }
#pragma unroll
            for (int o = 32; o > 0; o >>= 1) acc += __shfl_xor(acc, o);
            if (lane == 0) s_sum[wave] = acc;
            __syncthreads();
            float tot = 0.0f;
#pragma unroll
            for (int w = 0; w < NW; ++w) tot += s_sum[w];
            ip = off == 0 ? (float)((double)tot / 2.0 / (double)ap.counter)
                          : (float)((double)(tot / (float)(int32_t)ap.eff) / 2.0 / (double)ap.counter);
        }
    if (threadIdx.x == 0)
        {
            gsdr_acq_result r = res[bp];
            r.code_phase = idx;
            r.acq_delay_samples = (double)fmodf((float)idx, ap.samples_per_code);
            r.peak = peak;
            if (ap.cfar)
                {
                    if (!ap.step_two) r.input_power = ip;
                    r.test_statistic = r.peak / r.input_power;
                    r.positive = r.test_statistic > ap.threshold ? 1 : 0;
                }
            res[bp] = r;
        }
}

template <class MP, int STAT>
__global__ void __launch_bounds__(MP::NT) acq_argmax_pk_kernel(const float2* __restrict__ X,
    const float2* __restrict__ code_fft, gsdr_acq_result* __restrict__ res, const float2* __restrict__ tw, uint32_t D,
    uint32_t P, float samples_per_code, AcqParams ap)
{
    using gsdr::pk::c2;
    constexpr int NT = MP::NT;
    constexpr int NW = NT / 64;
    constexpr uint32_t N = MP::N;
    extern __shared__ float2 lds_raw[];
    c2* lds = reinterpret_cast<c2*>(lds_raw);
    unsigned long long* scratch = reinterpret_cast<unsigned long long*>(lds_raw + MP::lds_bytes() / sizeof(float2));
    const uint32_t bp = blockIdx.x;
    const uint32_t b = bp / P, p = bp - b * P;
    const uint32_t d = res[bp].doppler_index;
    if (d >= D) return;
    const c2* x = reinterpret_cast<const c2*>(X) + ap.xm.off(b, d);
    const c2* c = reinterpret_cast<const c2*>(code_fft) + (size_t)p * N;
    unsigned long long key = 0ull;
    auto load = [&](int, int, int i) -> c2 { return gsdr::pk::conj_mul(x[i], c[i]); };
    auto store = [&](int i, c2 v, int) {
        const float m = __builtin_fmaf(v.x, v.x, v.y * v.y);
        const unsigned long long k = ((unsigned long long)__float_as_uint(m) << 32) | (0xffffffffu - (uint32_t)i);
        key = k > key ? k : key;
    };
    MP::template run<false>(lds, tw, load, store, [] {});
#pragma unroll
    for (int off = 32; off > 0; off >>= 1)
        {
            const unsigned long long o = __shfl_xor(key, off);
            key = o > key ? o : key;
        }
    if ((threadIdx.x & 63) == 0) scratch[threadIdx.x >> 6] = key;
    __syncthreads();
    if (threadIdx.x == 0)
        {
#pragma unroll
            for (int w = 1; w < NW; ++w) key = scratch[w] > key ? scratch[w] : key;
            const uint32_t idx = 0xffffffffu - (uint32_t)(key & 0xffffffffu);
            res[bp].code_phase = idx;
            res[bp].acq_delay_samples = (double)fmodf((float)idx, samples_per_code);
        }
    if constexpr (STAT >= 2)
        {
            if (!ap.cfar || ap.step_two) return;
            const uint32_t opp = (d + D / 2) % D;
            const c2* xo = reinterpret_cast<const c2*>(X) + ap.xm.off(b, opp);
            float acc = 0.0f;
            for (uint32_t i = threadIdx.x; i < N; i += NT)
                {
                    const c2 y = gsdr::pk::conj_mul(xo[i], c[i]);
                    acc = __builtin_fmaf(y.x, y.x, __builtin_fmaf(y.y, y.y, acc));
                }
#pragma unroll
            for (int off = 32; off > 0; off >>= 1) acc += __shfl_xor(acc, off);
            float* fs = reinterpret_cast<float*>(scratch + NW);
            __syncthreads();
            if ((threadIdx.x & 63) == 0) fs[threadIdx.x >> 6] = acc;
            __syncthreads();
            if (threadIdx.x == 0)
                {
                    float tot = 0.0f;
#pragma unroll
                    for (int w = 0; w < NW; ++w) tot += fs[w];
                    const float ip = (float)((double)tot / 2.0 / (double)ap.counter);
                    gsdr_acq_result r = res[bp];
                    r.input_power = ip;
                    r.test_statistic = r.peak / ip;
                    r.positive = r.test_statistic > ap.threshold ? 1 : 0;
                    res[bp] = r;
                }
        }
}

__device__ __forceinline__ int pool_acquire(uint32_t* slots, int nwords)
{
    __shared__ int s_slot;
    if (threadIdx.x == 0)
        {
            int w = (int)((blockIdx.x + blockIdx.y * gridDim.x) % (unsigned)nwords);
            for (;;)
                {
                    const uint32_t cur = __hip_atomic_load(&slots[w], __ATOMIC_RELAXED, __HIP_MEMORY_SCOPE_AGENT);
                    if (cur != 0xffffffffu)
                        {
                            const int bit = __builtin_ctz(~cur);
                            const uint32_t old =
                                __hip_atomic_fetch_or(&slots[w], 1u << bit, __ATOMIC_ACQUIRE, __HIP_MEMORY_SCOPE_AGENT);
                            if (!(old & (1u << bit)))
                                {
                                    s_slot = w * 32 + bit;
                                    break;
                                }
                        }
                    else
                        {
                            w = w + 1 == nwords ? 0 : w + 1;
                            __builtin_amdgcn_s_sleep(2);
                        }
                }
        }
    __syncthreads();
    return s_slot;
}

__device__ __forceinline__ void pool_release(uint32_t* slots, int slot)
{
    __syncthreads();
    if (threadIdx.x == 0)
        __hip_atomic_fetch_and(&slots[slot >> 5], ~(1u << (slot & 31)), __ATOMIC_RELEASE, __HIP_MEMORY_SCOPE_AGENT);
}

__device__ __forceinline__ void dwell_cell(uint32_t D, uint32_t P, uint32_t nrows, uint32_t& b, uint32_t& d,
    uint32_t& p)
{
    const uint32_t id = blockIdx.x;
    const uint32_t full = nrows >> 3;
    const uint32_t PG = (P % 4u == 0u) ? 4u : ((P % 2u == 0u) ? 2u : 1u);
    uint32_t row;
    if (id < full * 8u * P)
        {
            const uint32_t xcd = id & 7u, slot = id >> 3;
            const uint32_t per_group = full * PG;
            const uint32_t pg = slot / per_group, rem = slot - pg * per_group;
            const uint32_t ri = rem / PG;
            row = ri * 8u + xcd;
            p = pg * PG + (rem - ri * PG);
        }
    else
        {
            const uint32_t t = id - full * 8u * P;
            row = full * 8u + t / P;
            p = t - (t / P) * P;
        }
    b = row / D;
    d = row - b * D;
}

template <class PT>
__global__ void __launch_bounds__(PT::NT) acq_correlate_dwell_kernel(const float2* __restrict__ X,
    const float2* __restrict__ code_fft, RowStat* __restrict__ stats, const float2* __restrict__ tw,
    typename PT::PlanT plan, AcqParams ap, float* __restrict__ acc_pool, uint32_t* __restrict__ acc_slots,
    int acc_words)
{
    extern __shared__ float2 lds[];
    RowStat* scratch = reinterpret_cast<RowStat*>(lds + gsdr::fft::lds_elems_dev(plan));
    const uint32_t N = plan.n;
    uint32_t b, d, p;
    dwell_cell(ap.D, ap.P, gridDim.x / ap.P, b, d, p);
    const uint32_t K = ap.dwells;
    const int slot = K > 1 ? pool_acquire(acc_slots, acc_words) : 0;
    float* acc = acc_pool + (size_t)slot * ap.eff;
    const float2* c = code_fft + (size_t)p * N;
    for (uint32_t k = 0; k < K; ++k)
        {
            const float2* x = X + ap.xm.off(b * K + k, d);
            float best = -1.0f, sum = 0.0f;
            uint32_t bidx = 0xffffffffu;
            auto load = [&](int i) -> float2 {
                float2 a = x[i], q = c[i];
                return make_float2(a.x * q.x + a.y * q.y, a.x * q.y - a.y * q.x);
            };
            auto store = [&](int i, float2 v) {
                const int j = i - (int)ap.out_off;
                if (j < 0) return;
                float m = v.x * v.x + v.y * v.y;
                if (K > 1)
                    {
                        if (k > 0) m = acc[j] + m;
                        acc[j] = m;
                    }
                if (stat_better(m, (uint32_t)j, best, bidx))
                    {
                        best = m;
                        bidx = (uint32_t)j;
                    }
                sum += m;
            };
            PT::run(plan, lds, tw, load, store);
            block_reduce_stat<PT::NT>(best, bidx, sum, scratch);
            if (threadIdx.x == 0) stats[(((size_t)b * ap.P + p) * K + k) * ap.D + d] = RowStat{best, bidx, sum, 0};
        }
    if (K > 1) pool_release(acc_slots, slot);
}

template <class PT>
__global__ void __launch_bounds__(PT::NT) acq_second_peak_dwell_kernel(const float2* __restrict__ X,
    const float2* __restrict__ code_fft, gsdr_acq_result* __restrict__ resk, const float2* __restrict__ tw,
    typename PT::PlanT plan, AcqParams ap, float* __restrict__ acc_pool, uint32_t* __restrict__ acc_slots,
    int acc_words)
{
    extern __shared__ float2 lds[];
    RowStat* scratch = reinterpret_cast<RowStat*>(lds + gsdr::fft::lds_elems_dev(plan));
    const uint32_t kk = blockIdx.x, bp = blockIdx.y;
    const uint32_t K = ap.dwells;
    const uint32_t b = bp / ap.P, p = bp - b * ap.P;
    const uint32_t N = plan.n;
    gsdr_acq_result* rr = resk + (size_t)bp * K + kk;
    const uint32_t d = rr->doppler_index;
    const int32_t ti = (int32_t)rr->code_phase;
    const int32_t E = (int32_t)ap.N;
    int32_t e1 = ti - (int32_t)ap.samples_per_chip;
    int32_t e2 = ti + (int32_t)ap.samples_per_chip;
    if (e1 < 0)
        e1 = E + e1;
    else if (e2 >= E)
        e2 = e2 - E;
    const int slot = kk > 0 ? pool_acquire(acc_slots, acc_words) : 0;
    float* acc = acc_pool + (size_t)slot * ap.eff;
    const float2* c = code_fft + (size_t)p * N;
    float best = 0.0f, sum = 0.0f;
    uint32_t bidx = 0;
    for (uint32_t k = 0; k <= kk; ++k)
        {
            const float2* x = X + ap.xm.off(b * K + k, d);
            const bool last = k == kk;
            auto load = [&](int i) -> float2 {
                float2 a = x[i], q = c[i];
                return make_float2(a.x * q.x + a.y * q.y, a.x * q.y - a.y * q.x);
            };
            auto store = [&](int i, float2 v) {
                const int j = i - (int)ap.out_off;
                if (j < 0) return;
                float m = v.x * v.x + v.y * v.y;
                if (kk > 0)
                    {
                        if (k > 0) m = acc[j] + m;
                        if (!last) acc[j] = m;
                    }
                if (last)
                    {
                        const bool excluded = (e1 < e2) ? (j >= e1 && j < e2) : (j >= e1 || j < e2);
                        if (excluded) m = 0.0f;
                        if (stat_better(m, (uint32_t)j, best, bidx))
                            {
                                best = m;
                                bidx = (uint32_t)j;
                            }
                    }
            };
            PT::run(plan, lds, tw, load, store);
        }
    block_reduce_stat<PT::NT>(best, bidx, sum, scratch);
    if (threadIdx.x == 0)
        {
            gsdr_acq_result r = *rr;
            r.second_peak = best;
            r.test_statistic = r.peak / best;
            r.positive = r.test_statistic > ap.threshold ? 1 : 0;
            *rr = r;
        }
    if (kk > 0) pool_release(acc_slots, slot);
}

template <class PT>
__global__ void __launch_bounds__(PT::NT) acq_dwell_grid_kernel(const float2* __restrict__ X,
    const float2* __restrict__ code_fft, RowStat* __restrict__ stats, const float2* __restrict__ tw,
    typename PT::PlanT plan, AcqParams ap, float* __restrict__ grid, uint32_t dwell)
{
    extern __shared__ float2 lds[];
    RowStat* scratch = reinterpret_cast<RowStat*>(lds + gsdr::fft::lds_elems_dev(plan));
    const uint32_t N = plan.n;
    const uint32_t d = blockIdx.x / ap.P, p = blockIdx.x - d * ap.P;
    float* row = grid + ((size_t)p * ap.D + d) * ap.eff;
    const float2* x = X + ap.xm.off(0, d);
    const float2* c = code_fft + (size_t)p * N;
    float best = -1.0f, sum = 0.0f;
    uint32_t bidx = 0xffffffffu;
    auto load = [&](int i) -> float2 {
        float2 a = x[i], q = c[i];
        return make_float2(a.x * q.x + a.y * q.y, a.x * q.y - a.y * q.x);
    };
    auto store = [&](int i, float2 v) {
        const int j = i - (int)ap.out_off;
        if (j < 0) return;
        float m = v.x * v.x + v.y * v.y;
        if (dwell > 0) m = row[j] + m;
        row[j] = m;
        if (stat_better(m, (uint32_t)j, best, bidx))
            {
                best = m;
                bidx = (uint32_t)j;
            }
        sum += m;
    };
    PT::run(plan, lds, tw, load, store);
    block_reduce_stat<PT::NT>(best, bidx, sum, scratch);
    if (threadIdx.x == 0) stats[(size_t)p * ap.D + d] = RowStat{best, bidx, sum, 0};
}

template <class MP, int IT>
__global__ void __launch_bounds__(MP::NT) acq_forward_pk_kernel(const void* __restrict__ iq, uint64_t block_stride,
    const float2* __restrict__ wipe, float2* __restrict__ X, const float2* __restrict__ tw, uint32_t consumed, XMap xm)
{
    using gsdr::pk::c2;
    extern __shared__ float2 lds_raw[];
    c2* lds = reinterpret_cast<c2*>(lds_raw);
    const uint32_t b = blockIdx.x, d = blockIdx.y;
    constexpr uint32_t N = MP::N;
    const size_t base = (size_t)b * block_stride;
    const c2* w = reinterpret_cast<const c2*>(wipe) + (size_t)d * N;
    c2* out = reinterpret_cast<c2*>(X) + xm.off(b, d);
    const int ext = (int)(xm.stride - N);
    auto load = [&](int, int, int i) -> c2 {
        if (i >= (int)consumed) return c2{0.f, 0.f};
        return gsdr::pk::mul(gsdr::pk::from(load_item<IT>(iq, base + i)), w[i]);
    };
    auto store = [&](int i, c2 v, int) {
        out[i] = v;
        if (i < ext) out[N + i] = v;
    };
    MP::run(lds, tw, load, store, [] {});
}

template <class PT>
__global__ void __launch_bounds__(PT::NT) acq_second_peak_kernel(const float2* __restrict__ X,
    const float2* __restrict__ code_fft, gsdr_acq_result* __restrict__ res, const float2* __restrict__ tw,
    typename PT::PlanT plan, AcqParams ap)
{
    extern __shared__ float2 lds[];
    RowStat* scratch = reinterpret_cast<RowStat*>(lds + gsdr::fft::lds_elems_dev(plan));
    const uint32_t bp = blockIdx.x;
    const uint32_t b = bp / ap.P, p = bp - b * ap.P;
    const uint32_t N = plan.n;
    const uint32_t d = res[bp].doppler_index;
    const int32_t ti = (int32_t)res[bp].code_phase;
    int32_t e1 = ti - (int32_t)ap.samples_per_chip;
    int32_t e2 = ti + (int32_t)ap.samples_per_chip;
    if (e1 < 0)
        e1 = (int32_t)N + e1;
    else if (e2 >= (int32_t)N)
        e2 = e2 - (int32_t)N;
    const float2* x = X + ap.xm.off(b, d);
    const float2* c = code_fft + (size_t)p * N;
    float best = 0.0f, sum = 0.0f;
    uint32_t bidx = 0;
    auto load = [&](int i) -> float2 {
        float2 a = x[i], k = c[i];
        return make_float2(a.x * k.x + a.y * k.y, a.x * k.y - a.y * k.x);
    };
    auto store = [&](int i, float2 v) {
        const int j = i - (int)ap.out_off;
        if (j < 0) return;
        const bool excluded = (e1 < e2) ? (j >= e1 && j < e2) : (j >= e1 || j < e2);
// ... 112 lines not shown
```

gnss-sdr-new_amd/csrc/acq_pk.hip:

```cpp
#include "acq_handle.h"
#include "acq_plans.h"
#include "acq_split_kernels.h"

namespace gsdr_acq_impl
{
namespace
{

using RegPlan93 = RegFourStep<16, 512, 8, 1 | (16 << 4), NoPads<1000>, 10, 10, 10>;
using RegPlan94 = RegFourStep<16, 512, 0, 1 | (16 << 4), NoPads<1000>, 10, 10, 10>;

template <int ID, class MP, int PG_, int WPE_, int ST, class REG = void, int CS_ = kCodeVgpr, int TW_ = kTwGlobal>
struct PkVariant
{
    static constexpr int id = ID, PG = PG_, WPE = WPE_, STAT = ST, CS = CS_, TW = TW_;
    using type = MP;
    using Reg = REG;
};
using PkVariants = PlanList<PkVariant<61, PkPlan<512, true, 20, 20, 20>, 1, 1, 1>,
    PkVariant<62, PkPlan<256, true, 20, 10, 10>, 1, 1, 1>,
    PkVariant<93, PkPlan<1024, 1, 16, 10, 10, 10>, 1, 1, 2, RegPlan93>,
    PkVariant<94, PkPlan<1024, 1, 16, 10, 10, 10>, 1, 1, 2, RegPlan94>,
    PkVariant<70, PkPlan<256, 1, 25, 16, 10>, 1, 1, 2>,
    PkVariant<97, PkPlan<256, 1, 25, 16, 10>, 16, 4, 2, void, kCodeLds>,
    PkVariant<98, PkPlan<256, 1, 25, 16, 10>, 16, 4, 2, void, kCodeLane>,
    PkVariant<99, PkPlan<256, 1, 25, 16, 10>, 16, 4, 2, void, kCodeLane, kTwLds>>;

template <class F>
int with_pk_variant(int id, F&& f, int unknown = GSDR_E_STATE)
{
    int rc = unknown;
    const bool found = find_plan(PkVariants{}, [&](auto e) {
        if (decltype(e)::id != id) return false;
        rc = f(e);
        return true;
    });
    if (!found && unknown != GSDR_OK) gsdr::set_error("internal: bad correlate variant %d", id);
    return rc;
}

}

int launch_corr_variant(gsdr_acq* a, const AcqView& v, uint32_t nblocks, hipStream_t s)
{
    return with_pk_variant(a->corr_variant, [&](auto e) {
        using V = decltype(e);
        using M = typename V::type;
        if constexpr (!std::is_void<typename V::Reg>::value)
            {
                using RP = typename V::Reg;
                hipLaunchKernelGGL((acq_correlate_reg_kernel<RP>), dim3(nblocks * v.D * v.nprn), dim3(RP::NT),
                    RP::lds_bytes(), s, a->d_X, v.code_fft, a->d_stats, a->d_tw, v.D, v.nprn, nblocks, v.xm);
            }
        else
            {
                const uint32_t groups = (v.nprn + V::PG - 1) / V::PG;
                hipLaunchKernelGGL((acq_correlate_pk_kernel<M, V::PG, V::WPE, V::STAT, V::CS, V::TW>), dim3(nblocks * v.D * groups),
                    dim3(M::NT), a->corr_lds_bytes, s, a->d_X, V::CS == kCodeLane ? v.code_lane : v.code_fft, a->d_stats, a->d_tw, v.D, v.nprn, nblocks,
                    v.xm);
            }
        return GSDR_OK;
    });
}

int launch_argmax_variant(gsdr_acq* a, const AcqView& v, uint32_t nblocks, gsdr_acq_result* res, hipStream_t s)
{
    return with_pk_variant(a->corr_variant, [&](auto e) {
        using V = decltype(e);
        using M = typename V::type;
        hipLaunchKernelGGL((acq_argmax_pk_kernel<M, V::STAT>), dim3(nblocks * v.nprn), dim3(M::NT), a->corr_lds_bytes,
            s, a->d_X, v.code_fft, res, a->d_tw, v.D, v.nprn, a->conf.samples_per_code, params_of(a, v));
        GSDR_HIP(hipGetLastError());
        return GSDR_OK;
    });
}

int launch_forward_pk(gsdr_acq* a, const AcqView& v, const void* iq, uint32_t nblocks, uint64_t stride, hipStream_t s)
{
    return with_pk_variant(a->corr_variant, [&](auto e) {
        using M = typename decltype(e)::type;
        with_item_type(a->conf.item_type, [&](auto t) {
            hipLaunchKernelGGL((acq_forward_pk_kernel<M, decltype(t)::value>), dim3(nblocks, v.xm.q), dim3(M::NT),
                M::lds_bytes(), s, iq, stride, v.wipe, a->d_X, a->d_tw, a->consumed, v.xm);
        });
        GSDR_HIP(hipGetLastError());
        return GSDR_OK;
    });
}

int setup_corr_variant(gsdr_acq* a, int id)
{
    a->corr_variant = 0;
    return with_pk_variant(id, [&](auto e) {
        using V = decltype(e);
        using M = typename V::type;
        if (M::N != (int)a->N)
            {
                gsdr::set_error("correlate variant %d is for N = %d, not %u", V::id, M::N, a->N);
                return GSDR_E_UNSUPPORTED;
            }
        a->corr_lds_bytes = pk_corr_lds_bytes<M, V::CS, V::TW>();
        int rc = set_max_lds((const void*)acq_correlate_pk_kernel<M, V::PG, V::WPE, V::STAT, V::CS, V::TW>, a->corr_lds_bytes);
        rc |= set_max_lds((const void*)acq_argmax_pk_kernel<M, V::STAT>, a->corr_lds_bytes);
        for (int it : kItemTypes)
            rc |= with_item_type(it, [&](auto t) {
                return set_max_lds((const void*)acq_forward_pk_kernel<M, decltype(t)::value>, M::lds_bytes());
            });
        if constexpr (!std::is_void<typename V::Reg>::value)
            rc |= set_max_lds((const void*)acq_correlate_reg_kernel<typename V::Reg>, V::Reg::lds_bytes());
        if (rc != GSDR_OK) return GSDR_E_DEVICE;
        a->corr_variant = V::id;
        a->lane_nb1 = V::CS == kCodeLane ? M::NB1 : 0;
        a->lane_r1 = V::CS == kCodeLane ? M::R1 : 0;
        a->corr_stat = V::STAT;
        return GSDR_OK;
    }, GSDR_OK);
}

}
```

gnss-sdr-new_amd/csrc/fft_pk.h:

```cpp
#pragma once

#include <hip/hip_runtime.h>

#include <cmath>
#include <type_traits>

#include "fft_lds.h"
#include "fft_multi.h"

namespace gsdr
{
namespace pk
{

typedef float c2 __attribute__((ext_vector_type(2)));

__device__ __forceinline__ c2 from(float2 v) { return c2{v.x, v.y}; }
__device__ __forceinline__ float2 to(c2 v) { return make_float2(v.x, v.y); }

__device__ __forceinline__ c2 mul(c2 a, c2 b)
{
    c2 r, o;
    asm("v_pk_mul_f32 %0, %1, %2 op_sel_hi:[0,1]" : "=v"(r) : "v"(a), "v"(b));
    asm("v_pk_fma_f32 %0, %1, %2, %3 op_sel:[1,1,0] op_sel_hi:[1,0,1] neg_lo:[1,0,0]"
// ... 99 lines not shown
        const c2 m = fmas(s, -0.5f, v[0]);
        const c2 t = scale(d, h);
        v[0] = v[0] + s;
        v[1] = add_mi(m, t);
        v[2] = sub_mi(m, t);
    }
};

template <>
struct Dft<4>
{
    __device__ __forceinline__ static void run(c2* v)
    {
        const c2 a = v[0] + v[2], b = v[0] - v[2];
        const c2 c = v[1] + v[3], d = v[1] - v[3];
        v[0] = a + c;
        v[2] = a - c;
        v[1] = add_mi(b, d);
        v[3] = sub_mi(b, d);
    }
};

template <>
struct Dft<5>
{
    __device__ __forceinline__ static void run(c2* v)
    {
        constexpr float c1 = 0.30901699437494742410f;
        constexpr float c2_ = -0.80901699437494742410f;
        constexpr float s1 = 0.95105651629515357212f;
        constexpr float s2 = 0.58778525229247312917f;
        const c2 a1 = v[1] + v[4], b1 = v[1] - v[4];
        const c2 a2 = v[2] + v[3], b2 = v[2] - v[3];
        const c2 x0 = v[0];
        const c2 p1 = fmas(a2, c2_, fmas(a1, c1, x0));
        const c2 p2 = fmas(a2, c1, fmas(a1, c2_, x0));
        const c2 q1 = fmas(b2, s2, scale(b1, s1));
        const c2 q2 = fmas(b2, -s1, scale(b1, s2));
        v[0] = x0 + a1 + a2;
        v[1] = add_mi(p1, q1);
        v[4] = sub_mi(p1, q1);
        v[2] = add_mi(p2, q2);
        v[3] = sub_mi(p2, q2);
    }
};

template <int R1, int R2>
struct DftCT
{
    template <int N2, int K1>
    __device__ __forceinline__ static void twiddle(c2* t)
    {
        t[K1] = mul_root<N2 * K1, R1 * R2>(t[K1]);
        if constexpr (K1 + 1 < R1) twiddle<N2, K1 + 1>(t);
    }
    template <int N2>
    __device__ __forceinline__ static void cols(c2* v, c2* y)
    {
        c2 t[R1];
#pragma unroll
        for (int n1 = 0; n1 < R1; ++n1) t[n1] = v[R2 * n1 + N2];
        Dft<R1>::run(t);
        twiddle<N2, 0>(t);
#pragma unroll
        for (int k1 = 0; k1 < R1; ++k1) y[N2 * R1 + k1] = t[k1];
        if constexpr (N2 + 1 < R2) cols<N2 + 1>(v, y);
    }
    __device__ __forceinline__ static void run(c2* v)
    {
        c2 y[R1 * R2];
        cols<0>(v, y);
#pragma unroll
        for (int k1 = 0; k1 < R1; ++k1)
            {
                c2 t[R2];
#pragma unroll
                for (int n2 = 0; n2 < R2; ++n2) t[n2] = y[n2 * R1 + k1];
                Dft<R2>::run(t);
#pragma unroll
                for (int k2 = 0; k2 < R2; ++k2) v[k1 + R1 * k2] = t[k2];
            }
    }
};

template <>
struct Dft<6> : DftCT<2, 3>
{
};
template <>
struct Dft<8> : DftCT<2, 4>
{
};
template <>
struct Dft<10> : DftCT<2, 5>
{
};
template <>
struct Dft<12> : DftCT<4, 3>
{
};
template <>
struct Dft<16> : DftCT<4, 4>
{
};
template <>
struct Dft<20> : DftCT<4, 5>
{
};
template <>
struct Dft<25> : DftCT<5, 5>
{
};
template <>
struct Dft<32> : DftCT<4, 8>
{
};

struct NoHook
{
    __device__ __forceinline__ void operator()() const {}
};

struct TwGlobal
{
    template <int R>
    using Mid = c2;
};

template <int R, int NT, int N, int Ns, bool TWP, bool FIRST, bool LAST, bool ORD, bool SKIPW, class Load, class Store,
    class Hook, class Pre, class Mid, class Tws>
__device__ __forceinline__ void stage(c2* lds, const float2* __restrict__ tw, Load& load, Store& store, Hook& hook,
    Pre& pre, Mid& mid, const Tws& tws)
{
    constexpr bool GLOBAL = std::is_same<Tws, TwGlobal>::value;
    static_assert(GLOBAL || TWP, "a twiddle source stands for the roots of a TWP plan");
    constexpr int BPT = fft::bpt_for(R);
    constexpr bool PRE = FIRST && !LAST && !std::is_same<Pre, NoHook>::value;
    constexpr bool MID = LAST && !FIRST && TWP && GLOBAL && !std::is_same<Mid, NoHook>::value;
    constexpr int NB = N / R;
    constexpr int TSTRIDE = N / (Ns * R);
    c2 v[BPT][R];
    c2 w1[BPT];
    std::conditional_t<LAST, c2, typename Tws::template Mid<R>> tf[BPT];
    if constexpr (MID)
        {
#pragma unroll
            for (int b = 0; b < BPT; ++b) w1[b] = from(tw[(min(threadIdx.x + (unsigned)(b * NT), (unsigned)(NB - 1)) % Ns) * TSTRIDE]);
        }
#pragma unroll
    for (int b = 0; b < BPT; ++b)
        {
            const int j = (int)threadIdx.x + b * NT;
            if constexpr (BPT == 1 && NB % NT != 0)
                {
                    const int jj = min(j, NB - 1);
                    if (!FIRST || !SKIPW || __builtin_amdgcn_readfirstlane((int)(threadIdx.x & ~63u)) < NB)
                        {
#pragma unroll
                            for (int r = 0; r < R; ++r)
                                {
                                    if constexpr (FIRST)
                                        v[b][r] = load(b, r, jj + r * NB);
                                    else
                                        v[b][r] = lds[jj + r * NB];
                                }
                        }
                }
            else if (NB % NT == 0 || j < NB)
                {
#pragma unroll
                    for (int r = 0; r < R; ++r)
                        {
                            if constexpr (FIRST)
                                v[b][r] = load(b, r, j + r * NB);
                            else
                                v[b][r] = lds[j + r * NB];
                        }
                }
        }
    if constexpr (FIRST)
        hook();
    else
        {
            if constexpr (!GLOBAL)
                {
#pragma unroll
                    for (int b = 0; b < BPT; ++b)
                        {
                            const int k = min((int)threadIdx.x + b * NT, NB - 1) % Ns;
                            if constexpr (LAST)
                                tf[b] = tws.last_root(k * TSTRIDE);
                            else
                                tf[b] = tws.template load_middle<R, Ns>(k);
                        }
                }
            if constexpr (MID)
                {
#pragma unroll
                    for (int b = 0; b < BPT; ++b) asm volatile("" : "+v"(w1[b]));
                }
            __syncthreads();
            if constexpr (LAST) mid();
        }
#pragma unroll
    for (int b = 0; b < BPT; ++b)
        {
            const int j = (int)threadIdx.x + b * NT;
            if (NB % NT == 0 || j < NB)
                {
                    int k = 0;
                    if constexpr (!FIRST)
                        {
                            k = j % Ns;
                            const int step = k * TSTRIDE;
                            if constexpr (!GLOBAL)
                                {
                                    if constexpr (LAST)
                                        apply_powers<R>(v[b], tf[b]);
                                    else
                                        tws.template middle<R>(v[b], tf[b]);
                                }
                            else if constexpr (MID)
                                apply_powers<R>(v[b], w1[b]);
                            else if constexpr (TWP)
                                apply_powers<R>(v[b], from(tw[step]));
                            else
                                {
#pragma unroll
                                    for (int r = 1; r < R; ++r) v[b][r] = mul(v[b][r], from(tw[r * step]));
                                }
                        }
                    Dft<R>::run(v[b]);
                    if constexpr (!LAST && !PRE)
                        {
                            const int base = (j - k) * R + k;
#pragma unroll
                            for (int r = 0; r < R; ++r) lds[base + r * Ns] = v[b][r];
                        }
                }
        }
    if constexpr (PRE)
        {
            pre();
#pragma unroll
            for (int b = 0; b < BPT; ++b)
                {
                    const int j = (int)threadIdx.x + b * NT;
                    if (NB % NT == 0 || j < NB)
                        {
#pragma unroll
                            for (int r = 0; r < R; ++r) lds[j * R + r * Ns] = v[b][r];
                        }
                }
        }
    if constexpr (LAST && ORD)
        {
            static_assert(!LAST || Ns * R == N, "last stage");
#pragma unroll
            for (int r = 0; r < R; ++r)
                {
#pragma unroll
                    for (int b = 0; b < BPT; ++b)
                        {
                            const int j = (int)threadIdx.x + b * NT;
                            if (NB % NT == 0 || j < NB) store(j + r * Ns, v[b][r], r * BPT + b);
                        }
                }
        }
    else if constexpr (LAST)
        {
            static_assert(!LAST || Ns * R == N, "last stage");
#pragma unroll
            for (int b = 0; b < BPT; ++b)
                {
                    const int j = (int)threadIdx.x + b * NT;
                    if (NB % NT == 0 || j < NB)
                        {
#pragma unroll
                            for (int r = 0; r < R; ++r) store(j + r * Ns, v[b][r], r * BPT + b);
                        }
                }
        }
    else
        __syncthreads();
}

template <int NT, int N, int Ns, bool TWP, bool FIRST, bool ORD, bool SKIPW, int R, int... Rest, class Load, class Store,
    class Hook, class Pre, class Mid, class Tws>
__device__ __forceinline__ void stages(c2* lds, const float2* __restrict__ tw, Load& load, Store& store, Hook& hook,
    Pre& pre, Mid& mid, const Tws& tws)
{
    constexpr bool LAST = sizeof...(Rest) == 0;
    stage<R, NT, N, Ns, TWP, FIRST, LAST, ORD, SKIPW>(lds, tw, load, store, hook, pre, mid, tws);
    if constexpr (!LAST) stages<NT, N, Ns * R, TWP, false, ORD, SKIPW, Rest...>(lds, tw, load, store, hook, pre, mid, tws);
}

template <int NT_, int TWP_, int... Rs>
struct PkPlan
{
    static constexpr int NT = NT_;
    static constexpr bool TWP = TWP_ != 0;
    static constexpr int N = (Rs * ...);
    static constexpr int nstages = sizeof...(Rs);
    static constexpr int R1 = fft::FirstRadix<Rs...>::value;
    static constexpr int BPT1 = fft::bpt_for(R1);
    static constexpr int NB1 = N / R1;
    static constexpr size_t lds_bytes() { return (size_t)N * sizeof(c2); }
    static constexpr int RL = (0, ..., Rs);
    static constexpr int BPTL = fft::bpt_for(RL);
    static constexpr int NSL = N / RL;
    static constexpr int NSLOTS = RL * BPTL;
    __device__ __forceinline__ static int index_of_slot(int slot)
    {
        return (int)threadIdx.x + (slot % BPTL) * NT + (slot / BPTL) * NSL;
    }
    template <bool ORD = true, bool SKIPW = false, class Load, class Store, class Hook, class Pre = NoHook, class Mid = NoHook,
        class Tws = TwGlobal>
    __device__ __forceinline__ static void run(c2* lds, const float2* __restrict__ tw, Load load, Store store, Hook hook,
        Pre pre = Pre{}, Mid mid = Mid{}, Tws tws = Tws{})
    {
        stages<NT, N, 1, TWP, true, ORD, SKIPW, Rs...>(lds, tw, load, store, hook, pre, mid, tws);
    }
};


}
}
```

gnss-sdr-new_amd/gsdr/__init__.py:

```python
import contextlib
import ctypes
import os

import numpy as np

_PKG = os.path.dirname(os.path.dirname(os.path.abspath(__file__)))
LIB_PATH = os.environ.get("GSDR_LIB", os.path.join(_PKG, "build", "libgsdr.so"))

GSDR_OK = 0
GSDR_E_ARG = -1
GSDR_E_DEVICE = -2
GSDR_E_ALLOC = -3
GSDR_E_STATE = -4
GSDR_E_UNSUPPORTED = -5

ITEM_GR_COMPLEX = 0
ITEM_CSHORT = 1
ITEM_IBYTE = 2
_ITEM_NP = {0: np.complex64, 1: np.int16, 2: np.int8}
ASSOC_GENERIC = 0
ASSOC_AVX = 1

EXPORTED = [
    "gsdr_last_error", "gsdr_abi_version", "gsdr_device_count",
    "gsdr_acq_create", "gsdr_acq_destroy", "gsdr_acq_get_dims", "gsdr_acq_set_local_codes",
    "gsdr_acq_set_doppler", "gsdr_acq_set_threshold", "gsdr_acq_get_threshold", "gsdr_acq_run",
    "gsdr_acq_run_device", "gsdr_acq_dump_grid", "gsdr_acq_dump_spectra", "gsdr_acq_set_profiling",
    "gsdr_acq_read_profile",
    "gsdr_corr_create", "gsdr_corr_destroy", "gsdr_corr_set_local_code_and_taps",
    "gsdr_corr_set_local_code_and_taps_complex", "gsdr_corr_set_high_dynamics_resampler",
    "gsdr_corr_set_resampler_assoc", "gsdr_corr_run", "gsdr_corr_run_batch", "gsdr_corr_run_batch_device",
    "gsdr_corr_dump_indices", "gsdr_corr_run_epochs", "gsdr_corr_set_profiling", "gsdr_corr_read_profile",
    "gsdr_trk_conf_default", "gsdr_trk_create", "gsdr_trk_destroy", "gsdr_trk_start", "gsdr_trk_stop",
    "gsdr_trk_run_device", "gsdr_trk_run", "gsdr_trk_get_channel", "gsdr_trk_save_state", "gsdr_trk_restore_state",
    "gsdr_trk_set_profiling", "gsdr_trk_read_profile", "gsdr_acq_set_cu_mask", "gsdr_trk_set_cu_mask",
    "gsdr_acq_run_dwell", "gsdr_acq_run_stream", "gsdr_trk_run_stream", "gsdr_trk_run_stream_host",
    "gsdr_stream_create", "gsdr_stream_destroy", "gsdr_stream_push", "gsdr_stream_span", "gsdr_stream_window",
    "gsdr_acq_set_step_two", "gsdr_acq_get_step_two_threshold", "gsdr_acq_run_step_two",
    "gsdr_trk_set_data_code", "gsdr_acq_read_profile_ex", "gsdr_stream_window_async", "gsdr_stream_release", "gsdr_stream_device",
    "gsdr_acq_dump_grid_step_two", "gsdr_acq_read_profile_intervals", "gsdr_acq_set_wipeoff",
    "gsdr_acq_get_spectrum_reuse", "gsdr_trk_force_loss_of_lock", "gsdr_acq_set_local_code",
    "gsdr_acq_set_active_prns", "gsdr_acq_submit_stream", "gsdr_acq_collect", "gsdr_host_register",
    "gsdr_host_unregister", "gsdr_trk_submit_stream", "gsdr_trk_collect", "gsdr_stream_landed",
    "gsdr_stream_wait_landed",
    "gsdr_stream_read", "gsdr_firdes_low_pass", "gsdr_acq_resampler_plan", "gsdr_decim_create", "gsdr_decim_destroy",
    "gsdr_decim_output", "gsdr_decim_advance", "gsdr_acq_get_plan", "gsdr_acq_get_split",
]

WIPE_EXACT, WIPE_GENERIC, WIPE_AVX2 = 0, 1, 2
SIGNAL_GPS_1C = 0
SIGNAL_GAL_1B = 1
SIGNAL_BDS_B1 = 2
TRK_F_VALID_OUTPUT, TRK_F_LOSS_OF_LOCK, TRK_F_PLL_180, TRK_F_BIT_SYNC, TRK_F_OVERRUN, TRK_F_LOGGED = 1, 2, 4, 8, 16, 32

TRK_CONF_DTYPE = np.dtype([
    ("fs_in", "f8"), ("carrier_lock_th", "f8"), ("vector_length", "u4"), ("signal", "i4"), ("item_type", "i4"),
    ("max_channels", "u4"), ("fll_bw_hz", "f4"), ("pll_bw_hz", "f4"), ("dll_bw_hz", "f4"), ("pll_bw_narrow_hz", "f4"),
    ("dll_bw_narrow_hz", "f4"), ("early_late_space_chips", "f4"), ("very_early_late_space_chips", "f4"),
    ("early_late_space_narrow_chips", "f4"), ("very_early_late_space_narrow_chips", "f4"),
    ("cn0_smoother_alpha", "f4"), ("carrier_lock_test_smoother_alpha", "f4"), ("pull_in_time_s", "u4"),
    ("bit_synchronization_time_limit_s", "u4"), ("pll_filter_order", "i4"), ("dll_filter_order", "i4"),
    ("extend_correlation_symbols", "i4"), ("cn0_samples", "i4"), ("cn0_smoother_samples", "i4"),
    ("carrier_lock_test_smoother_samples", "i4"), ("cn0_min", "i4"), ("max_code_lock_fail", "i4"),
    ("max_carrier_lock_fail", "i4"), ("enable_fll_pull_in", "i4"), ("enable_fll_steady_state", "i4"),
    ("carrier_aiding", "i4"), ("high_dyn", "i4"), ("track_pilot", "i4"), ("smoother_length", "u4")], align=True)
assert TRK_CONF_DTYPE.itemsize == 144

TRK_EPOCH_DTYPE = np.dtype([
    ("sample_counter", "u8"), ("state", "i4"), ("consumed", "i4"), ("taps", "f4", (10,)),
    ("rem_carr_phase_rad", "f4"), ("flags", "i4"), ("carrier_doppler_hz", "f8"), ("code_freq_chips", "f8"),
    ("rem_code_phase_samples", "f8"), ("acc_carrier_phase_rad", "f8"), ("cn0_db_hz", "f8"),
    ("carrier_lock_test", "f8"), ("prompt_i", "f8"), ("prompt_q", "f8"), ("evm", "f8"), ("data_prompt", "f4", (2,)),
    ("carrier_rate", "f4"), ("code_rate", "f4"), ("log_accu", "f4", (5,)), ("carr_phase_error_hz", "f4"),
    ("carr_error_filt_hz", "f4"), ("code_error_chips", "f4"), ("code_error_filt_chips", "f4"), ("reserved", "i4")], align=True)
assert TRK_EPOCH_DTYPE.itemsize == 192


TRK_DUMP_DTYPE = np.dtype([
    ("abs_VE", "<f4"), ("abs_E", "<f4"), ("abs_P", "<f4"), ("abs_L", "<f4"), ("abs_VL", "<f4"),
    ("Prompt_I", "<f4"), ("Prompt_Q", "<f4"), ("PRN_start_sample_count", "<u8"), ("acc_carrier_phase_rad", "<f4"),
    ("carrier_doppler_hz", "<f4"), ("carrier_doppler_rate_hz", "<f4"), ("code_freq_chips", "<f4"),
    ("code_freq_rate_chips", "<f4"), ("carr_error_hz", "<f4"), ("carr_error_filt_hz", "<f4"),
    ("code_error_chips", "<f4"), ("code_error_filt_chips", "<f4"), ("CN0_SNV_dB_Hz", "<f4"),
    ("carrier_lock_test", "<f4"), ("aux1", "<f4"), ("aux2", "<f8"), ("PRN", "<u4"),
    ("acq_code_phase_samples", "<f4"), ("acq_carrier_doppler_hz", "<f4"), ("EVM", "<f4")])
assert TRK_DUMP_DTYPE.itemsize == 108


def trk_dump_records(recs, fs_in, prn, acq_code_phase_samples, acq_carrier_doppler_hz, veml=False,
                     track_pilot=False):
    r = recs[(recs["flags"] & TRK_F_LOGGED) != 0]
    out = np.zeros(len(r), TRK_DUMP_DTYPE)
    ip = 2 if veml else 1
    acc = r["log_accu"]
    out["abs_VE"] = acc[:, 0] if veml else 0.0
    out["abs_E"], out["abs_P"], out["abs_L"] = acc[:, 1], acc[:, 2], acc[:, 3]
    out["abs_VL"] = acc[:, 4] if veml else 0.0
    out["Prompt_I"] = r["data_prompt"][:, 0] if track_pilot else r["taps"][:, 2 * ip]
    out["Prompt_Q"] = r["data_prompt"][:, 1] if track_pilot else r["taps"][:, 2 * ip + 1]
    stamp = r["sample_counter"] + r["consumed"].astype(np.uint64)
    out["PRN_start_sample_count"] = stamp
    out["acc_carrier_phase_rad"] = r["acc_carrier_phase_rad"].astype(np.float32)
    out["carrier_doppler_hz"] = r["carrier_doppler_hz"].astype(np.float32)
    two_pi = 2.0 * 3.1415926535897932384626433832795
    out["carrier_doppler_rate_hz"] = (r["carrier_rate"].astype(np.float64) * fs_in * fs_in / two_pi).astype(np.float32)
    out["code_freq_chips"] = r["code_freq_chips"].astype(np.float32)
    out["code_freq_rate_chips"] = (r["code_rate"].astype(np.float64) * fs_in * fs_in).astype(np.float32)
    out["carr_error_hz"] = r["carr_phase_error_hz"]
    out["carr_error_filt_hz"] = r["carr_error_filt_hz"]
    out["code_error_chips"] = r["code_error_chips"]
    out["code_error_filt_chips"] = r["code_error_filt_chips"]
    out["CN0_SNV_dB_Hz"] = r["cn0_db_hz"].astype(np.float32)
    out["carrier_lock_test"] = r["carrier_lock_test"].astype(np.float32)
    out["aux1"] = r["rem_code_phase_samples"].astype(np.float32)
    out["aux2"] = stamp.astype(np.float64)
    out["PRN"] = prn
    out["acq_code_phase_samples"] = np.float32(acq_code_phase_samples)
    out["acq_carrier_doppler_hz"] = np.float32(acq_carrier_doppler_hz)
    out["EVM"] = r["evm"].astype(np.float32)
    return out


def read_trk_dump(path):
    return np.fromfile(path, dtype=TRK_DUMP_DTYPE)


class GsdrError(RuntimeError):
    def __init__(self, code, msg):
        super().__init__("gsdr error %d: %s" % (code, msg))
        self.code = code


class AcqConf(ctypes.Structure):
    _fields_ = [
        ("fs_in", ctypes.c_int64),
        ("consumed_samples", ctypes.c_uint32),
        ("fft_size", ctypes.c_uint32),
        ("samples_per_code", ctypes.c_float),
        ("samples_per_chip", ctypes.c_uint32),
        ("doppler_max", ctypes.c_int32),
        ("doppler_step", ctypes.c_uint32),
        ("doppler_center", ctypes.c_int32),
        ("doppler_bias", ctypes.c_int32),
        ("num_doppler_bins", ctypes.c_uint32),
        ("pfa", ctypes.c_float),
        ("max_dwells", ctypes.c_uint32),
        ("bit_transition_flag", ctypes.c_int32),
        ("item_type", ctypes.c_int32),
        ("max_prns", ctypes.c_uint32),
        ("max_blocks", ctypes.c_uint32),
        ("sampled_ms", ctypes.c_uint32),
        ("ms_per_code", ctypes.c_uint32),
    ]


class AcqResult(ctypes.Structure):
    _fields_ = [
        ("prn", ctypes.c_uint32),
        ("doppler_index", ctypes.c_uint32),
        ("code_phase", ctypes.c_uint32),
        ("doppler_hz", ctypes.c_int32),
        ("peak", ctypes.c_float),
        ("input_power", ctypes.c_float),
        ("second_peak", ctypes.c_float),
        ("test_statistic", ctypes.c_float),
        ("acq_delay_samples", ctypes.c_double),
        ("samplestamp", ctypes.c_uint64),
        ("positive", ctypes.c_int32),
        ("num_dwells", ctypes.c_int32),
    ]


ACQ_RESULT_DTYPE = np.dtype([
    ("prn", np.uint32), ("doppler_index", np.uint32), ("code_phase", np.uint32), ("doppler_hz", np.int32),
    ("peak", np.float32), ("input_power", np.float32), ("second_peak", np.float32),
    ("test_statistic", np.float32), ("acq_delay_samples", np.float64), ("samplestamp", np.uint64),
    ("positive", np.int32), ("num_dwells", np.int32)])
assert ACQ_RESULT_DTYPE.itemsize == ctypes.sizeof(AcqResult)


class CorrJob(ctypes.Structure):
    _fields_ = [
        ("channel", ctypes.c_int32),
        ("n_samples", ctypes.c_int32),
        ("sample_offset", ctypes.c_int64),
        ("rem_carr_phase_rad", ctypes.c_float),
        ("carr_phase_step_rad", ctypes.c_float),
        ("carr_phase_rate_step_rad", ctypes.c_float),
        ("rem_code_phase_chips", ctypes.c_float),
        ("code_phase_step_chips", ctypes.c_float),
        ("code_phase_rate_step_chips", ctypes.c_float),
    ]


CORR_JOB_DTYPE = np.dtype([
    ("channel", np.int32), ("n_samples", np.int32), ("sample_offset", np.int64),
    ("rem_carr_phase_rad", np.float32), ("carr_phase_step_rad", np.float32),
    ("carr_phase_rate_step_rad", np.float32), ("rem_code_phase_chips", np.float32),
    ("code_phase_step_chips", np.float32), ("code_phase_rate_step_chips", np.float32)])
assert CORR_JOB_DTYPE.itemsize == ctypes.sizeof(CorrJob)

_lib = None


def load():
    global _lib
    if _lib is not None:
        return _lib
    if not os.path.exists(LIB_PATH):
        raise OSError("libgsdr.so not built: %s (run __graft_entry__.build())" % LIB_PATH)
    L = ctypes.CDLL(LIB_PATH)
    P, I, U32, U64, I64, F = (ctypes.c_void_p, ctypes.c_int, ctypes.c_uint32, ctypes.c_uint64, ctypes.c_int64,
                              ctypes.c_float)
    L.gsdr_last_error.restype = ctypes.c_char_p
    L.gsdr_abi_version.restype = I
    L.gsdr_device_count.argtypes = [P]
    L.gsdr_acq_create.argtypes = [I, ctypes.POINTER(AcqConf), P]
    L.gsdr_acq_destroy.argtypes = [P]
    L.gsdr_acq_destroy.restype = None
    L.gsdr_acq_get_dims.argtypes = [P, P, P]
    L.gsdr_acq_get_plan.argtypes = [P, P, P, P, P, P]
    L.gsdr_acq_get_split.argtypes = [P, P]
    L.gsdr_acq_set_local_codes.argtypes = [P, P, P, U32]
    L.gsdr_acq_set_doppler.argtypes = [P, ctypes.c_int32, U32, ctypes.c_int32]
    L.gsdr_acq_set_threshold.argtypes = [P, F]
    L.gsdr_acq_get_threshold.argtypes = [P, P]
    L.gsdr_acq_run.argtypes = [P, P, U32, U64, P]
    L.gsdr_acq_run_device.argtypes = [P, P, U32, U64, U64, P, P]
    L.gsdr_acq_dump_grid.argtypes = [P, P, U32, P]
    L.gsdr_acq_dump_grid_step_two.argtypes = [P, P, U32, ctypes.c_float, P]
    L.gsdr_acq_read_profile_intervals.argtypes = [P, P, ctypes.c_int, P, P, U32, P]
    L.gsdr_acq_set_wipeoff.argtypes = [P, ctypes.c_int]
    L.gsdr_acq_get_spectrum_reuse.argtypes = [P, P, P]
    L.gsdr_acq_dump_spectra.argtypes = [P, P, P]
    L.gsdr_corr_create.argtypes = [I, I, I, I, P]
    L.gsdr_corr_destroy.argtypes = [P]
    L.gsdr_corr_destroy.restype = None
    L.gsdr_corr_set_local_code_and_taps.argtypes = [P, I, I, P, P, I]
    L.gsdr_corr_set_local_code_and_taps_complex.argtypes = [P, I, I, P, P, I]
    L.gsdr_corr_set_high_dynamics_resampler.argtypes = [P, I, I]
    L.gsdr_corr_set_resampler_assoc.argtypes = [P, I]
    L.gsdr_corr_run.argtypes = [P, I, P, I, F, F, F, F, F, F, I, P]
    L.gsdr_corr_run_batch.argtypes = [P, P, I, P, I, I64, P, P]
    L.gsdr_corr_run_batch_device.argtypes = [P, P, I, P, I, I64, P, P]
    L.gsdr_corr_dump_indices.argtypes = [P, I, F, F, I, P]
    L.gsdr_acq_set_profiling.argtypes = [P, I]
    L.gsdr_acq_read_profile.argtypes = [P, P, P]
    L.gsdr_corr_run_epochs.argtypes = [P, P, I, I, P, I, I64, P, P]
    L.gsdr_corr_set_profiling.argtypes = [P, I]
    L.gsdr_corr_read_profile.argtypes = [P, P, P]
    L.gsdr_trk_conf_default.argtypes = [P]
    L.gsdr_trk_conf_default.restype = None
    L.gsdr_trk_create.argtypes = [I, P, P]
    L.gsdr_trk_destroy.argtypes = [P]
    L.gsdr_trk_destroy.restype = None
    L.gsdr_trk_start.argtypes = [P, I, U32, P, I, ctypes.c_double, ctypes.c_double, U64, U64, P]
    L.gsdr_trk_stop.argtypes = [P, I]
    L.gsdr_trk_force_loss_of_lock.argtypes = [P, I]
    L.gsdr_acq_set_local_code.argtypes = [P, U32, P, U32]
    L.gsdr_acq_set_active_prns.argtypes = [P, U32]
    L.gsdr_acq_submit_stream.argtypes = [P, P, U64, U32, U64]
    L.gsdr_acq_collect.argtypes = [P, P, P, P]
    L.gsdr_host_register.argtypes = [P, ctypes.c_size_t]
    L.gsdr_host_unregister.argtypes = [P]
    L.gsdr_trk_set_data_code.argtypes = [P, I, P, I]
    L.gsdr_trk_run_device.argtypes = [P, P, U64, U64, U32, P, P, P]
    L.gsdr_trk_run.argtypes = [P, P, U64, U64, U32, P, P]
    L.gsdr_trk_get_channel.argtypes = [P, I, P, P, P, P]
    L.gsdr_trk_save_state.argtypes = [P, I, P]
    L.gsdr_trk_restore_state.argtypes = [P, I, P]
    L.gsdr_trk_set_profiling.argtypes = [P, I]
    L.gsdr_trk_read_profile.argtypes = [P, P, P]
    L.gsdr_acq_set_cu_mask.argtypes = [P, P, I]
    L.gsdr_acq_set_step_two.argtypes = [P, U32, F, F]
    L.gsdr_acq_get_step_two_threshold.argtypes = [P, P]
    L.gsdr_acq_run_step_two.argtypes = [P, P, U32, P, P, P, U64, P]
    L.gsdr_trk_set_cu_mask.argtypes = [P, P, I]
    L.gsdr_acq_run_dwell.argtypes = [P, P, U32, U64, P]
    L.gsdr_stream_create.argtypes = [I, I, U64, U64, P]
    L.gsdr_stream_destroy.argtypes = [P]
    L.gsdr_stream_destroy.restype = None
    L.gsdr_stream_push.argtypes = [P, P, U64, U64]
    L.gsdr_stream_landed.argtypes = [P, P]
    L.gsdr_stream_wait_landed.argtypes = [P, U64]
    L.gsdr_stream_span.argtypes = [P, P, P]
    L.gsdr_stream_window.argtypes = [P, U64, U64, P]
    L.gsdr_acq_read_profile_ex.argtypes = [P, P, P, P]
    L.gsdr_stream_window_async.argtypes = [P, U64, U64, P, P]
    L.gsdr_stream_release.argtypes = [P, P]
    L.gsdr_stream_device.argtypes = [P, P]
    L.gsdr_acq_run_stream.argtypes = [P, P, U64, U32, U64, P]
    L.gsdr_trk_run_stream.argtypes = [P, P, U32, P, P, P]
    L.gsdr_trk_run_stream_host.argtypes = [P, P, U32, P, P]
    L.gsdr_trk_submit_stream.argtypes = [P, P, U32]
    L.gsdr_trk_collect.argtypes = [P, ctypes.c_int, P, P, P]
    L.gsdr_stream_read.argtypes = [P, U64, U64, P]
    L.gsdr_firdes_low_pass.argtypes = [ctypes.c_double, ctypes.c_double, ctypes.c_double, ctypes.c_double, P, P]
    L.gsdr_acq_resampler_plan.argtypes = [I64, ctypes.c_double, P, P, P]
    L.gsdr_decim_create.argtypes = [P, U32, P, U32, U64, U64, P]
    L.gsdr_decim_destroy.argtypes = [P]
    L.gsdr_decim_destroy.restype = None
    L.gsdr_decim_output.argtypes = [P, P]
    L.gsdr_decim_advance.argtypes = [P, P]
    _lib = L
    return L


def _check(rc):
    if rc != GSDR_OK:
        raise GsdrError(rc, load().gsdr_last_error().decode(errors="replace"))


def _ptr(a):
    return ctypes.c_void_p(a.ctypes.data)


def device_count():
    n = ctypes.c_int(0)
    _check(load().gsdr_device_count(ctypes.byref(n)))
    return n.value


class Acquisition:

    def __init__(self, fs_in, consumed_samples, doppler_max, doppler_step, pfa=0.0, max_prns=32, max_blocks=1,
                 samples_per_code=None, samples_per_chip=None, num_doppler_bins=0, doppler_center=0,
                 doppler_bias=0, item_type=ITEM_GR_COMPLEX, fft_size=0, sampled_ms=1, ms_per_code=1,
                 chip_rate=1023000.0, max_dwells=1, bit_transition=False, device=0):
        L = load()
        c = AcqConf()
        c.fs_in = int(fs_in)
        c.consumed_samples = int(consumed_samples)
        c.fft_size = int(fft_size)
        spms = np.float32(np.float32(fs_in) * np.float32(0.001))
        c.samples_per_code = float(samples_per_code if samples_per_code is not None else spms * ms_per_code)
        c.samples_per_chip = int(samples_per_chip if samples_per_chip is not None
                                 else int(np.ceil(float(np.float32(fs_in)) / chip_rate)))
        c.doppler_max = int(doppler_max)
        c.doppler_step = int(doppler_step)
        c.doppler_center = int(doppler_center)
        c.doppler_bias = int(doppler_bias)
        c.num_doppler_bins = int(num_doppler_bins)
        c.pfa = float(pfa)
        c.max_dwells = int(max_dwells)
        c.bit_transition_flag = int(bool(bit_transition))
        c.item_type = int(item_type)
        c.max_prns = int(max_prns)
        c.max_blocks = int(max_blocks)
        c.sampled_ms = int(sampled_ms)
        c.ms_per_code = int(ms_per_code)
        self.conf = c
        self._h = ctypes.c_void_p()
        _check(L.gsdr_acq_create(int(device), ctypes.byref(c), ctypes.byref(self._h)))
        D, N = ctypes.c_uint32(), ctypes.c_uint32()
        _check(L.gsdr_acq_get_dims(self._h, ctypes.byref(D), ctypes.byref(N)))
        self.num_doppler_bins, self.fft_size = D.value, N.value
        self.nprn = 0
        self.item_type = item_type
        self.dwells = 1 if bit_transition else max(1, int(max_dwells))

    def close(self):
        if self._h:
            load().gsdr_acq_destroy(self._h)
            self._h = ctypes.c_void_p()

    def __del__(self):
        try:
            self.close()
        except Exception:
            pass

    def set_local_codes(self, codes, prns):
        codes = np.ascontiguousarray(codes, np.complex64)
        prns = np.ascontiguousarray(prns, np.uint32)
        assert codes.ndim == 2 and codes.shape[0] == len(prns)
        _check(load().gsdr_acq_set_local_codes(self._h, _ptr(codes), _ptr(prns), len(prns)))
        self.nprn = len(prns)

    def set_local_code(self, slot, code, prn):
        code = np.ascontiguousarray(code, np.complex64)
        assert code.ndim == 1 and len(code) >= self.conf.consumed_samples
        _check(load().gsdr_acq_set_local_code(self._h, int(slot), _ptr(code), int(prn)))
        self.nprn = max(self.nprn, int(slot) + 1)

    def set_active_prns(self, nprn):
        _check(load().gsdr_acq_set_active_prns(self._h, int(nprn)))
        self.nprn = int(nprn)

    @property
    def plan(self):
        v = np.zeros(4, np.int32)
        radix = np.zeros(8, np.int32)
        split = ctypes.c_int32()
        L = load()
        _check(L.gsdr_acq_get_plan(self._h, _ptr(v[0:]), _ptr(v[1:]), _ptr(v[2:]), _ptr(v[3:]), _ptr(radix)))
        _check(L.gsdr_acq_get_split(self._h, ctypes.byref(split)))
        return {"variant": int(v[0]), "nthreads": int(v[1]), "r1": int(v[2]), "nstages": int(v[3]),
                "radix": [int(r) for r in radix[:v[3]]], "split": split.value}

    def set_doppler(self, doppler_max, doppler_step, doppler_center=0):
        _check(load().gsdr_acq_set_doppler(self._h, int(doppler_max), int(doppler_step), int(doppler_center)))

    def set_wipeoff(self, mode):
        if isinstance(mode, str):
            mode = {"exact": WIPE_EXACT, "generic": WIPE_GENERIC, "avx2": WIPE_AVX2}[mode]
        _check(load().gsdr_acq_set_wipeoff(self._h, int(mode)))
        self._wipe_mode = int(mode)

    @property
    def wipe_mode(self):
        if getattr(self, "_wipe_mode", None) is None:
            env = os.environ.get("GSDR_ACQ_WIPE", "exact")
            self._wipe_mode = {"generic": WIPE_GENERIC, "avx2": WIPE_AVX2}.get(env, WIPE_EXACT)
        return self._wipe_mode

    @property
    def spectrum_reuse(self):
        q = np.zeros(1, np.uint32)
        p = np.zeros(1, np.uint32)
        _check(load().gsdr_acq_get_spectrum_reuse(self._h, _ptr(q), _ptr(p)))
        return int(q[0]), int(p[0])

    def set_threshold(self, t):
        _check(load().gsdr_acq_set_threshold(self._h, float(t)))

    @property
    def threshold(self):
        t = ctypes.c_float()
        _check(load().gsdr_acq_get_threshold(self._h, ctypes.byref(t)))
        return t.value

    def _items(self, iq):
        return np.ascontiguousarray(iq, _ITEM_NP[int(self.item_type)])

    def run(self, iq, nblocks=1, stamp0=0):
        iq = self._items(iq)
        out = np.zeros(nblocks * self.nprn, ACQ_RESULT_DTYPE)
        _check(load().gsdr_acq_run(self._h, _ptr(iq), int(nblocks), int(stamp0), _ptr(out)))
        return out.reshape(nblocks, self.nprn)

    def run_dwell(self, iq, dwell, stamp=0):
        iq = self._items(iq)
        out = np.zeros(self.nprn, ACQ_RESULT_DTYPE)
        _check(load().gsdr_acq_run_dwell(self._h, _ptr(iq), int(dwell), int(stamp), _ptr(out)))
        return out

    def run_stream(self, ring, first_sample, nblocks=1, stamp0=0):
        out = np.zeros(nblocks * self.nprn, ACQ_RESULT_DTYPE)
        _check(load().gsdr_acq_run_stream(self._h, ring._h, int(first_sample), int(nblocks), int(stamp0), _ptr(out)))
        return out.reshape(nblocks, self.nprn)

    def submit_stream(self, ring, first_sample, nblocks=1, stamp0=0):
        _check(load().gsdr_acq_submit_stream(self._h, ring._h, int(first_sample), int(nblocks), int(stamp0)))

    def collect(self):
        out = np.zeros(int(self.conf.max_blocks) * int(self.conf.max_prns), ACQ_RESULT_DTYPE)
        nb, npr = ctypes.c_uint32(), ctypes.c_uint32()
        _check(load().gsdr_acq_collect(self._h, _ptr(out), ctypes.byref(nb), ctypes.byref(npr)))
        return out[:nb.value * npr.value].reshape(nb.value, npr.value).copy()

    def set_step_two(self, num_doppler_bins_step2=4, doppler_step2=125.0, pfa2=0.0):
        _check(load().gsdr_acq_set_step_two(self._h, int(num_doppler_bins_step2), float(doppler_step2),
                                            float(pfa2)))
        self._st2_bins = int(num_doppler_bins_step2)

    @property
    def step_two_threshold(self):
        t = ctypes.c_float()
        _check(load().gsdr_acq_get_step_two_threshold(self._h, ctypes.byref(t)))
        return t.value

    def run_step_two(self, iq, prn_slots, doppler_centers_hz, coarse_input_power, stamp=0):
        iq = self._items(iq)
        slots = np.ascontiguousarray(prn_slots, np.uint32)
        cen = np.ascontiguousarray(doppler_centers_hz, np.float32)
        ip = np.ascontiguousarray(coarse_input_power, np.float32)
        assert len(slots) == len(cen) == len(ip)
        out = np.zeros(len(slots), ACQ_RESULT_DTYPE)
        _check(load().gsdr_acq_run_step_two(self._h, _ptr(iq), len(slots), _ptr(slots), _ptr(cen), _ptr(ip),
                                            int(stamp), _ptr(out)))
        return out

    def run_device(self, iq_dev_ptr, nblocks, stride_items, stamp0, out_dev_ptr, stream_ptr=0):
        _check(load().gsdr_acq_run_device(self._h, ctypes.c_void_p(iq_dev_ptr), int(nblocks), int(stride_items),
                                          int(stamp0), ctypes.c_void_p(out_dev_ptr), ctypes.c_void_p(stream_ptr)))

    def set_profiling(self, enable):
        _check(load().gsdr_acq_set_profiling(self._h, int(bool(enable))))

    def set_cu_mask(self, mask_words):
        m = np.ascontiguousarray(mask_words, np.uint32)
        _check(load().gsdr_acq_set_cu_mask(self._h, _ptr(m) if len(m) else None, len(m)))

    def read_profile(self):
        ms = np.zeros(4, np.float64)
        n = np.zeros(4, np.uint32)
        _check(load().gsdr_acq_read_profile(self._h, _ptr(ms), _ptr(n)))
        return ms, n

    def read_profile_ex(self):
        ms = np.zeros(4, np.float64)
        n = np.zeros(4, np.uint32)
        busy = np.zeros(4, np.float64)
        _check(load().gsdr_acq_read_profile_ex(self._h, _ptr(ms), _ptr(n), _ptr(busy)))
        return ms, n, busy

    def read_profile_intervals(self, ref_event, stage, max_n=4096):
        st = np.zeros(max_n, np.float64)
        en = np.zeros(max_n, np.float64)
        n = ctypes.c_uint32(0)
        _check(load().gsdr_acq_read_profile_intervals(self._h, ctypes.c_void_p(ref_event), int(stage), _ptr(st),
                                                      _ptr(en), int(max_n), ctypes.byref(n)))
        k = min(n.value, max_n)
        return st[:k], en[:k]

    def dump_grid(self, iq, prn_slot):
        iq = self._items(iq)
        g = np.zeros((self.num_doppler_bins, self.fft_size), np.float32)
        _check(load().gsdr_acq_dump_grid(self._h, _ptr(iq), int(prn_slot), _ptr(g)))
        return g

    def dump_grid_step_two(self, iq, prn_slot, doppler_center_hz):
        iq = self._items(iq)
        g = np.zeros((self._st2_bins, self.fft_size), np.float32)
        _check(load().gsdr_acq_dump_grid_step_two(self._h, _ptr(iq), int(prn_slot), float(doppler_center_hz), _ptr(g)))
        return g

    def dump_spectra(self, iq):
        iq = self._items(iq)
        X = np.zeros((self.num_doppler_bins, self.fft_size), np.complex64)
        _check(load().gsdr_acq_dump_spectra(self._h, _ptr(iq), _ptr(X)))
        return X


class Correlator:

    def __init__(self, max_channels, max_len, max_taps=8, device=0):
        self._h = ctypes.c_void_p()
        _check(load().gsdr_corr_create(int(device), int(max_channels), int(max_len), int(max_taps),
                                       ctypes.byref(self._h)))
        self.max_taps = max_taps
        self.ntaps = {}

    def close(self):
        if self._h:
            load().gsdr_corr_destroy(self._h)
            self._h = ctypes.c_void_p()

    def __del__(self):
        try:
            self.close()
        except Exception:
            pass

    def set_local_code_and_taps(self, channel, code, shifts):
        if np.iscomplexobj(code):
            code = np.ascontiguousarray(code, np.complex64)
            shifts = np.ascontiguousarray(shifts, np.float32)
            _check(load().gsdr_corr_set_local_code_and_taps_complex(self._h, channel, len(code), _ptr(code),
                                                                    _ptr(shifts), len(shifts)))
        else:
            code = np.ascontiguousarray(code, np.float32)
            shifts = np.ascontiguousarray(shifts, np.float32)
            _check(load().gsdr_corr_set_local_code_and_taps(self._h, channel, len(code), _ptr(code), _ptr(shifts),
                                                            len(shifts)))
        self.ntaps[channel] = len(shifts)

    def set_high_dynamics_resampler(self, channel, enable):
        _check(load().gsdr_corr_set_high_dynamics_resampler(self._h, channel, int(bool(enable))))

    def set_resampler_assoc(self, assoc):
        _check(load().gsdr_corr_set_resampler_assoc(self._h, int(assoc)))

    def run(self, channel, sig, rem_carr, carr_step, rem_code, code_step, n, carr_rate=0.0, code_rate=0.0,
            item_type=ITEM_GR_COMPLEX):
        sig = np.ascontiguousarray(sig, _ITEM_NP[int(item_type)])
        out = np.zeros(self.ntaps[channel], np.complex64)
        _check(load().gsdr_corr_run(self._h, channel, _ptr(sig), item_type, rem_carr, carr_step, carr_rate, rem_code,
                                    code_step, code_rate, int(n), _ptr(out)))
        return out

    def run_batch(self, jobs, iq_dev_ptr, iq_items, out_dev_ptr, item_type=ITEM_GR_COMPLEX, stream_ptr=0):
        jobs = np.ascontiguousarray(jobs, CORR_JOB_DTYPE)
        _check(load().gsdr_corr_run_batch(self._h, _ptr(jobs), len(jobs), ctypes.c_void_p(iq_dev_ptr), item_type,
                                          int(iq_items), ctypes.c_void_p(out_dev_ptr), ctypes.c_void_p(stream_ptr)))

    def run_batch_device(self, jobs_dev_ptr, njobs, iq_dev_ptr, iq_items, out_dev_ptr, item_type=ITEM_GR_COMPLEX,
                         stream_ptr=0):
        _check(load().gsdr_corr_run_batch_device(self._h, ctypes.c_void_p(jobs_dev_ptr), int(njobs),
                                                 ctypes.c_void_p(iq_dev_ptr), item_type, int(iq_items),
                                                 ctypes.c_void_p(out_dev_ptr), ctypes.c_void_p(stream_ptr)))

    def run_epochs(self, jobs_dev_ptr, jobs_per_epoch, n_epochs, iq_dev_ptr, iq_items, out_dev_ptr,
                   item_type=ITEM_GR_COMPLEX, stream_ptr=0):
        _check(load().gsdr_corr_run_epochs(self._h, ctypes.c_void_p(jobs_dev_ptr), int(jobs_per_epoch), int(n_epochs),
                                           ctypes.c_void_p(iq_dev_ptr), item_type, int(iq_items),
                                           ctypes.c_void_p(out_dev_ptr), ctypes.c_void_p(stream_ptr)))

    def set_profiling(self, enable):
        _check(load().gsdr_corr_set_profiling(self._h, int(bool(enable))))

    def read_profile(self):
        ms = ctypes.c_double()
        n = ctypes.c_uint32()
        _check(load().gsdr_corr_read_profile(self._h, ctypes.byref(ms), ctypes.byref(n)))
        return ms.value, n.value

    def dump_indices(self, channel, rem_code, code_step, n):
        out = np.zeros((self.ntaps[channel], n), np.int32)
        _check(load().gsdr_corr_dump_indices(self._h, channel, rem_code, code_step, int(n), _ptr(out)))
        return out


def trk_conf_default():
    c = np.zeros(1, TRK_CONF_DTYPE)
    load().gsdr_trk_conf_default(_ptr(c))
    return c


class Tracking:

    def __init__(self, conf, device=0):
        self.conf = np.ascontiguousarray(conf, TRK_CONF_DTYPE).copy()
        self._h = ctypes.c_void_p()
        _check(load().gsdr_trk_create(int(device), _ptr(self.conf), ctypes.byref(self._h)))
        self.max_channels = int(self.conf["max_channels"][0])

    def close(self):
        if self._h:
            load().gsdr_trk_destroy(self._h)
            self._h = ctypes.c_void_p()

    def __del__(self):
        try:
            self.close()
        except Exception:
            pass

    def start(self, ch, prn, code, acq_delay_samples, acq_doppler_hz, acq_samplestamp, nitems_read, data_code=None):
        code = np.ascontiguousarray(code, np.float32)
        if data_code is not None:
            dc = np.ascontiguousarray(data_code, np.float32)
            _check(load().gsdr_trk_set_data_code(self._h, int(ch), _ptr(dc), len(dc)))
        first = ctypes.c_uint64()
        _check(load().gsdr_trk_start(self._h, int(ch), int(prn), _ptr(code), len(code), float(acq_delay_samples),
                                     float(acq_doppler_hz), int(acq_samplestamp), int(nitems_read),
                                     ctypes.byref(first)))
        return first.value

    def stop(self, ch):
        _check(load().gsdr_trk_stop(self._h, int(ch)))

    def force_loss_of_lock(self, ch):
        _check(load().gsdr_trk_force_loss_of_lock(self._h, int(ch)))

    def run(self, iq, iq_first_sample, max_epochs):
        item = int(self.conf["item_type"][0])
        iq = np.ascontiguousarray(iq, _ITEM_NP[item])
        n_items = len(iq) if item == ITEM_GR_COMPLEX else len(iq) // 2
        out = np.zeros(self.max_channels * max_epochs, TRK_EPOCH_DTYPE)
        n = np.zeros(self.max_channels, np.uint32)
        _check(load().gsdr_trk_run(self._h, _ptr(iq), int(iq_first_sample), int(n_items), int(max_epochs), _ptr(out),
                                   _ptr(n)))
        return out.reshape(self.max_channels, max_epochs), n

    def run_device(self, iq_dev_ptr, iq_first_sample, iq_items, max_epochs, out_dev_ptr, nout_dev_ptr, stream_ptr=0):
        _check(load().gsdr_trk_run_device(self._h, ctypes.c_void_p(iq_dev_ptr), int(iq_first_sample), int(iq_items),
                                          int(max_epochs), ctypes.c_void_p(out_dev_ptr), ctypes.c_void_p(nout_dev_ptr),
                                          ctypes.c_void_p(stream_ptr)))

    def run_stream(self, ring, max_epochs, out_dev_ptr, nout_dev_ptr, stream_ptr=0):
        _check(load().gsdr_trk_run_stream(self._h, ring._h, int(max_epochs), ctypes.c_void_p(out_dev_ptr),
                                          ctypes.c_void_p(nout_dev_ptr), ctypes.c_void_p(stream_ptr)))

    def run_stream_host(self, ring, max_epochs):
        out = np.zeros(self.max_channels * max_epochs, TRK_EPOCH_DTYPE)
        n = np.zeros(self.max_channels, np.uint32)
        _check(load().gsdr_trk_run_stream_host(self._h, ring._h, int(max_epochs), _ptr(out), _ptr(n)))
        return out.reshape(self.max_channels, max_epochs), n

    def submit_stream(self, ring, max_epochs):
        _check(load().gsdr_trk_submit_stream(self._h, ring._h, int(max_epochs)))
        self._sub_epochs = getattr(self, "_sub_epochs", [])
        self._sub_epochs.append(int(max_epochs))

    def collect(self, wait=True):
        pending = getattr(self, "_sub_epochs", [])
        me = pending[0] if pending else 1
        out = np.zeros(self.max_channels * me, TRK_EPOCH_DTYPE)
        n = np.zeros(self.max_channels, np.uint32)
        got = ctypes.c_uint32()
        rc = load().gsdr_trk_collect(self._h, 1 if wait else 0, _ptr(out), _ptr(n), ctypes.byref(got))
        if rc == 1:
            return None
        _check(rc)
        pending.pop(0)
        return out.reshape(self.max_channels, me), n

    def channel(self, ch):
        st, nxt, dop, cn0 = ctypes.c_int32(), ctypes.c_uint64(), ctypes.c_double(), ctypes.c_double()
        _check(load().gsdr_trk_get_channel(self._h, int(ch), ctypes.byref(st), ctypes.byref(nxt), ctypes.byref(dop),
                                           ctypes.byref(cn0)))
        return {"state": st.value, "next_sample": nxt.value, "carrier_doppler_hz": dop.value, "cn0_db_hz": cn0.value}

    def save_state(self, slot=0, stream_ptr=0):
        _check(load().gsdr_trk_save_state(self._h, int(slot), ctypes.c_void_p(stream_ptr)))

    def restore_state(self, slot=0, stream_ptr=0):
        _check(load().gsdr_trk_restore_state(self._h, int(slot), ctypes.c_void_p(stream_ptr)))

    def set_profiling(self, enable):
        _check(load().gsdr_trk_set_profiling(self._h, int(bool(enable))))

    def set_cu_mask(self, mask_words):
        m = np.ascontiguousarray(mask_words, np.uint32)
        _check(load().gsdr_trk_set_cu_mask(self._h, _ptr(m) if len(m) else None, len(m)))

    def read_profile(self):
        ms = ctypes.c_double()
        n = ctypes.c_uint32()
        _check(load().gsdr_trk_read_profile(self._h, ctypes.byref(ms), ctypes.byref(n)))
        return ms.value, n.value


class Stream:

    def __init__(self, item_type, capacity_items, max_window_items, device=0):
        self._h = ctypes.c_void_p()
        _check(load().gsdr_stream_create(int(device), int(item_type), int(capacity_items), int(max_window_items),
                                         ctypes.byref(self._h)))
        self.item_type = int(item_type)
        self._inflight = []

    def close(self):
        if self._h:
            load().gsdr_stream_destroy(self._h)
            self._h = ctypes.c_void_p()
        self._inflight = []

    def __del__(self):
        try:
            self.close()
        except Exception:
            pass

    def push(self, iq, first_sample):
        iq = np.ascontiguousarray(iq, _ITEM_NP[self.item_type])
        n = len(iq) if self.item_type == ITEM_GR_COMPLEX else len(iq) // 2
        _check(load().gsdr_stream_push(self._h, _ptr(iq), int(first_sample), int(n)))
        self._inflight.append((int(first_sample) + n, iq))
        self.landed()
        return n

    def landed(self):
        v = ctypes.c_uint64()
        _check(load().gsdr_stream_landed(self._h, ctypes.byref(v)))
        self._inflight = [(e, a) for e, a in self._inflight if e > v.value]
        return v.value

    def wait_landed(self, upto):
        _check(load().gsdr_stream_wait_landed(self._h, int(upto)))
        return self.landed()

    def span(self):
        f, n = ctypes.c_uint64(), ctypes.c_uint64()
        _check(load().gsdr_stream_span(self._h, ctypes.byref(f), ctypes.byref(n)))
        return f.value, n.value

    def window(self, first_sample, n_items):
        p = ctypes.c_void_p()
        _check(load().gsdr_stream_window(self._h, int(first_sample), int(n_items), ctypes.byref(p)))
        return p.value

    def window_async(self, first_sample, n_items, consumer_stream):
        p = ctypes.c_void_p()
        _check(load().gsdr_stream_window_async(self._h, int(first_sample), int(n_items),
                                               ctypes.c_void_p(consumer_stream), ctypes.byref(p)))
        return p.value

    def release(self, consumer_stream):
        _check(load().gsdr_stream_release(self._h, ctypes.c_void_p(consumer_stream)))

    @contextlib.contextmanager
    def reading(self, first_sample, n_items, consumer_stream):
        p = self.window_async(first_sample, n_items, consumer_stream)
        try:
            yield p
        finally:
            self.release(consumer_stream)

    def read(self, first, n):
        n = int(n)
        out = np.zeros(n if self.item_type == ITEM_GR_COMPLEX else 2 * n, _ITEM_NP[self.item_type])
        _check(load().gsdr_stream_read(self._h, int(first), n, _ptr(out)))
        return out

    @property
    def device(self):
        d = ctypes.c_int()
        _check(load().gsdr_stream_device(self._h, ctypes.byref(d)))
        return d.value


class _BorrowedStream(Stream):

    def __init__(self, handle, item_type, owner):
        self._h = handle
        self.item_type = int(item_type)
        self._inflight = []
        self._owner = owner

    def close(self):
        self._h = ctypes.c_void_p()
        self._owner = None


def firdes_low_pass(gain, fs, cutoff, transition_width):
    if not transition_width > 0 or not fs > 0:
        raise GsdrError(GSDR_E_ARG, "firdes_low_pass: need fs > 0 and transition_width > 0")
    cap = int(min(1e6, 53.0 * float(fs) / (22.0 * float(transition_width)))) + 2
    taps = np.zeros(cap, np.float32)
    n = ctypes.c_uint32(cap)
    _check(load().gsdr_firdes_low_pass(float(gain), float(fs), float(cutoff), float(transition_width), _ptr(taps),
                                       ctypes.byref(n)))
# ... 53 lines not shown
```

include/gsdr.h:

```cpp
#ifndef GSDR_H
#define GSDR_H

#include <stddef.h>
#include <stdint.h>

#ifdef __cplusplus
extern "C" {
#endif

#define GSDR_ABI_VERSION 1

#define GSDR_OK 0
#define GSDR_E_ARG (-1)
#define GSDR_E_DEVICE (-2)
#define GSDR_E_ALLOC (-3)
#define GSDR_E_STATE (-4)
#define GSDR_E_UNSUPPORTED (-5)

#define GSDR_ITEM_GR_COMPLEX 0
#define GSDR_ITEM_CSHORT 1
#define GSDR_ITEM_IBYTE 2

#define GSDR_ASSOC_GENERIC 0
#define GSDR_ASSOC_AVX 1

const char* gsdr_last_error(void);
int gsdr_abi_version(void);
int gsdr_device_count(int* count);
int gsdr_host_register(void* ptr, size_t bytes);
int gsdr_host_unregister(void* ptr);

typedef struct gsdr_stream gsdr_stream;

int gsdr_stream_create(int device, int item_type, uint64_t capacity_items, uint64_t max_window_items, gsdr_stream** out);
void gsdr_stream_destroy(gsdr_stream* stream);
int gsdr_stream_push(gsdr_stream* stream, const void* iq_host, uint64_t first_sample, uint64_t n);
int gsdr_stream_landed(gsdr_stream* stream, uint64_t* landed);
int gsdr_stream_wait_landed(gsdr_stream* stream, uint64_t upto);
int gsdr_stream_span(gsdr_stream* stream, uint64_t* first_sample, uint64_t* n_items);
int gsdr_stream_window(gsdr_stream* stream, uint64_t first_sample, uint64_t n_items, const void** iq_dev);
int gsdr_stream_window_async(gsdr_stream* stream, uint64_t first_sample, uint64_t n_items, void* consumer_stream,
    const void** iq_dev);
int gsdr_stream_release(gsdr_stream* stream, void* consumer_stream);
int gsdr_stream_device(const gsdr_stream* stream, int* device);
int gsdr_stream_read(gsdr_stream* stream, uint64_t first, uint64_t n, void* host_out);

typedef struct gsdr_decim gsdr_decim;

int gsdr_firdes_low_pass(double gain, double fs, double cutoff, double transition_width, float* taps, uint32_t* ntaps);
int gsdr_acq_resampler_plan(int64_t fs_in, double opt_fs, uint32_t* decimation, uint32_t* ntaps, uint32_t* latency);
int gsdr_decim_create(gsdr_stream* source, uint32_t decimation, const float* taps, uint32_t ntaps, uint64_t capacity_items,
    uint64_t max_window_items, gsdr_decim** out);
void gsdr_decim_destroy(gsdr_decim* decim);
int gsdr_decim_output(gsdr_decim* decim, gsdr_stream** out);
int gsdr_decim_advance(gsdr_decim* decim, uint64_t* out_head);


typedef struct gsdr_acq gsdr_acq;

typedef struct gsdr_acq_conf
{
    int64_t fs_in;
    uint32_t consumed_samples;
    uint32_t fft_size;
    float samples_per_code;
    uint32_t samples_per_chip;
    int32_t doppler_max;
    uint32_t doppler_step;
    int32_t doppler_center;
    int32_t doppler_bias;
    uint32_t num_doppler_bins;
    float pfa;
    uint32_t max_dwells;
    int32_t bit_transition_flag;
    int32_t item_type;
    uint32_t max_prns;
    uint32_t max_blocks;
    uint32_t sampled_ms;
    uint32_t ms_per_code;
} gsdr_acq_conf;

typedef struct gsdr_acq_result
{
    uint32_t prn;
    uint32_t doppler_index;
    uint32_t code_phase;
    int32_t doppler_hz;
    float peak;
    float input_power;
    float second_peak;
    float test_statistic;
    double acq_delay_samples;
    uint64_t samplestamp;
    int32_t positive;
    int32_t num_dwells;
} gsdr_acq_result;

int gsdr_acq_create(int device, const gsdr_acq_conf* conf, gsdr_acq** out);
void gsdr_acq_destroy(gsdr_acq* acq);

int gsdr_acq_get_dims(const gsdr_acq* acq, uint32_t* num_doppler_bins, uint32_t* fft_size);
int gsdr_acq_get_plan(const gsdr_acq* acq, int32_t* variant, int32_t* nthreads, int32_t* r1, int32_t* nstages,
    int32_t radix[8]);
int gsdr_acq_get_split(const gsdr_acq* acq, int32_t* split);

int gsdr_acq_set_local_codes(gsdr_acq* acq, const float* codes, const uint32_t* prn, uint32_t nprn);
int gsdr_acq_set_local_code(gsdr_acq* acq, uint32_t slot, const float* code, uint32_t prn);
int gsdr_acq_set_active_prns(gsdr_acq* acq, uint32_t nprn);

int gsdr_acq_set_doppler(gsdr_acq* acq, int32_t doppler_max, uint32_t doppler_step, int32_t doppler_center);

#define GSDR_WIPE_EXACT 0
#define GSDR_WIPE_GENERIC 1
#define GSDR_WIPE_AVX2 2
int gsdr_acq_set_wipeoff(gsdr_acq* acq, int mode);
int gsdr_acq_get_spectrum_reuse(const gsdr_acq* acq, uint32_t* q, uint32_t* p);

int gsdr_acq_set_threshold(gsdr_acq* acq, float threshold);
int gsdr_acq_get_threshold(const gsdr_acq* acq, float* threshold);

int gsdr_acq_run(gsdr_acq* acq, const void* iq_host, uint32_t nblocks, uint64_t stamp0, gsdr_acq_result* out);

int gsdr_acq_run_dwell(gsdr_acq* acq, const void* iq_host, uint32_t dwell, uint64_t stamp, gsdr_acq_result* out);

int gsdr_acq_run_device(gsdr_acq* acq, const void* iq_dev, uint32_t nblocks, uint64_t block_stride_items,
    uint64_t stamp0, gsdr_acq_result* out_dev, void* stream);

int gsdr_acq_run_stream(gsdr_acq* acq, gsdr_stream* stream, uint64_t first_sample, uint32_t nblocks, uint64_t stamp0,
    gsdr_acq_result* out_host);
int gsdr_acq_submit_stream(gsdr_acq* acq, gsdr_stream* stream, uint64_t first_sample, uint32_t nblocks,
    uint64_t stamp0);
int gsdr_acq_collect(gsdr_acq* acq, gsdr_acq_result* out_host, uint32_t* nblocks, uint32_t* nprn);

int gsdr_acq_dump_grid(gsdr_acq* acq, const void* iq_host, uint32_t prn_slot, float* grid_host);
int gsdr_acq_dump_grid_step_two(gsdr_acq* acq, const void* iq_host, uint32_t prn_slot, float doppler_center_hz,
    float* grid_host);

int gsdr_acq_set_step_two(gsdr_acq* acq, uint32_t num_doppler_bins_step2, float doppler_step2, float pfa2);
int gsdr_acq_get_step_two_threshold(const gsdr_acq* acq, float* threshold);
int gsdr_acq_run_step_two(gsdr_acq* acq, const void* iq_host, uint32_t nsel, const uint32_t* prn_slots,
    const float* doppler_center_hz, const float* coarse_input_power, uint64_t stamp, gsdr_acq_result* out);

int gsdr_acq_set_profiling(gsdr_acq* acq, int enable);
int gsdr_acq_read_profile(gsdr_acq* acq, double* stage_ms, uint32_t* launches);
int gsdr_acq_read_profile_ex(gsdr_acq* acq, double* stage_ms, uint32_t* launches, double* stage_busy_ms);
int gsdr_acq_read_profile_intervals(gsdr_acq* acq, const void* ref_event, int stage, double* start_ms, double* end_ms,
    uint32_t max_n, uint32_t* n);

int gsdr_acq_dump_spectra(gsdr_acq* acq, const void* iq_host, float* spectra_host);


typedef struct gsdr_corr gsdr_corr;

typedef struct gsdr_corr_job
{
    int32_t channel;
    int32_t n_samples;
    int64_t sample_offset;
    float rem_carr_phase_rad;
    float carr_phase_step_rad;
    float carr_phase_rate_step_rad;
    float rem_code_phase_chips;
    float code_phase_step_chips;
    float code_phase_rate_step_chips;
} gsdr_corr_job;

int gsdr_corr_create(int device, int max_channels, int max_len, int max_taps, gsdr_corr** out);
void gsdr_corr_destroy(gsdr_corr* corr);

int gsdr_corr_set_local_code_and_taps(gsdr_corr* corr, int channel, int code_length_chips, const float* code,
    const float* shifts_chips, int n_taps);
int gsdr_corr_set_local_code_and_taps_complex(gsdr_corr* corr, int channel, int code_length_chips,
    const float* code_cf32, const float* shifts_chips, int n_taps);
int gsdr_corr_set_high_dynamics_resampler(gsdr_corr* corr, int channel, int enable);
int gsdr_corr_set_resampler_assoc(gsdr_corr* corr, int assoc);

int gsdr_corr_run(gsdr_corr* corr, int channel, const void* sig_in_host, int item_type, float rem_carr_phase_rad,
    float carr_phase_step_rad, float carr_phase_rate_step_rad, float rem_code_phase_chips,
    float code_phase_step_chips, float code_phase_rate_step_chips, int signal_length_samples, float* corr_out_host);

int gsdr_corr_run_batch(gsdr_corr* corr, const gsdr_corr_job* jobs_host, int njobs, const void* iq_dev,
    int item_type, int64_t iq_items, float* out_dev, void* stream);

int gsdr_corr_run_batch_device(gsdr_corr* corr, const gsdr_corr_job* jobs_dev, int njobs, const void* iq_dev,
    int item_type, int64_t iq_items, float* out_dev, void* stream);

int gsdr_corr_run_epochs(gsdr_corr* corr, const gsdr_corr_job* jobs_dev, int jobs_per_epoch, int n_epochs,
    const void* iq_dev, int item_type, int64_t iq_items, float* out_dev, void* stream);

int gsdr_corr_set_profiling(gsdr_corr* corr, int enable);
int gsdr_corr_read_profile(gsdr_corr* corr, double* kernel_ms, uint32_t* launches);

int gsdr_corr_dump_indices(gsdr_corr* corr, int channel, float rem_code_phase_chips, float code_phase_step_chips,
    int n, int32_t* idx_host);

typedef struct gsdr_trk gsdr_trk;

#define GSDR_SIGNAL_GPS_1C 0
#define GSDR_SIGNAL_GAL_1B 1
#define GSDR_SIGNAL_BDS_B1 2

typedef struct gsdr_trk_conf
{
    double fs_in;
    double carrier_lock_th;
    uint32_t vector_length;
    int32_t signal;
    int32_t item_type;
    uint32_t max_channels;
    float fll_bw_hz;
    float pll_bw_hz;
    float dll_bw_hz;
    float pll_bw_narrow_hz;
    float dll_bw_narrow_hz;
    float early_late_space_chips;
    float very_early_late_space_chips;
    float early_late_space_narrow_chips;
    float very_early_late_space_narrow_chips;
    float cn0_smoother_alpha;
    float carrier_lock_test_smoother_alpha;
    uint32_t pull_in_time_s;
    uint32_t bit_synchronization_time_limit_s;
    int32_t pll_filter_order;
    int32_t dll_filter_order;
    int32_t extend_correlation_symbols;
    int32_t cn0_samples;
    int32_t cn0_smoother_samples;
    int32_t carrier_lock_test_smoother_samples;
    int32_t cn0_min;
    int32_t max_code_lock_fail;
    int32_t max_carrier_lock_fail;
    int32_t enable_fll_pull_in;
    int32_t enable_fll_steady_state;
    int32_t carrier_aiding;
    int32_t high_dyn;
    int32_t track_pilot;
    uint32_t smoother_length;
} gsdr_trk_conf;

typedef struct gsdr_trk_epoch
{
    uint64_t sample_counter;
    int32_t state;
    int32_t consumed;
    float taps[10];
    float rem_carr_phase_rad;
    int32_t flags;
    double carrier_doppler_hz;
    double code_freq_chips;
    double rem_code_phase_samples;
    double acc_carrier_phase_rad;
    double cn0_db_hz;
    double carrier_lock_test;
    double prompt_i;
    double prompt_q;
    double evm;
    float data_prompt[2];
    float carrier_rate;
    float code_rate;
    float log_accu[5];
    float carr_phase_error_hz, carr_error_filt_hz, code_error_chips, code_error_filt_chips;
    int32_t reserved;
} gsdr_trk_epoch;

#define GSDR_TRK_F_VALID_OUTPUT 1
#define GSDR_TRK_F_LOSS_OF_LOCK 2
#define GSDR_TRK_F_PLL_180 4
#define GSDR_TRK_F_BIT_SYNC 8
#define GSDR_TRK_F_OVERRUN 16
#define GSDR_TRK_F_LOGGED 32

void gsdr_trk_conf_default(gsdr_trk_conf* conf);
int gsdr_trk_create(int device, const gsdr_trk_conf* conf, gsdr_trk** out);
void gsdr_trk_destroy(gsdr_trk* trk);

int gsdr_trk_start(gsdr_trk* trk, int ch, uint32_t prn, const float* code, int code_samples,
    double acq_delay_samples, double acq_doppler_hz, uint64_t acq_samplestamp, uint64_t nitems_read,
    uint64_t* first_sample);
int gsdr_trk_set_data_code(gsdr_trk* trk, int ch, const float* data_code, int code_samples);
int gsdr_trk_stop(gsdr_trk* trk, int ch);
int gsdr_trk_force_loss_of_lock(gsdr_trk* trk, int ch);

int gsdr_trk_run_device(gsdr_trk* trk, const void* iq_dev, uint64_t iq_first_sample, uint64_t iq_items,
    uint32_t max_epochs, gsdr_trk_epoch* out_dev, uint32_t* n_out_dev, void* stream);

int gsdr_trk_run_stream(gsdr_trk* trk, gsdr_stream* ring, uint32_t max_epochs, gsdr_trk_epoch* out_dev,
    uint32_t* n_out_dev, void* stream);

int gsdr_trk_run_stream_host(gsdr_trk* trk, gsdr_stream* ring, uint32_t max_epochs, gsdr_trk_epoch* out_host,
    uint32_t* n_out_host);

int gsdr_trk_submit_stream(gsdr_trk* trk, gsdr_stream* ring, uint32_t max_epochs);
int gsdr_trk_collect(gsdr_trk* trk, int wait, gsdr_trk_epoch* out_host, uint32_t* n_out_host, uint32_t* max_epochs);

int gsdr_trk_run(gsdr_trk* trk, const void* iq_host, uint64_t iq_first_sample, uint64_t iq_items,
    uint32_t max_epochs, gsdr_trk_epoch* out_host, uint32_t* n_out_host);

int gsdr_trk_get_channel(gsdr_trk* trk, int ch, int32_t* state, uint64_t* next_sample, double* carrier_doppler_hz,
    double* cn0_db_hz);

int gsdr_trk_save_state(gsdr_trk* trk, int slot, void* stream);
int gsdr_trk_restore_state(gsdr_trk* trk, int slot, void* stream);

int gsdr_trk_set_profiling(gsdr_trk* trk, int enable);

int gsdr_acq_set_cu_mask(gsdr_acq* acq, const uint32_t* mask, int n_words);
int gsdr_trk_set_cu_mask(gsdr_trk* trk, const uint32_t* mask, int n_words);
int gsdr_trk_read_profile(gsdr_trk* trk, double* kernel_ms, uint32_t* launches);

#ifdef __cplusplus
}
#endif

#endif
```

Baseline: 272.8 Msamples/s.

## Add prime-factor 32x125 inverse FFT plan for N=4000 correlate kernel

Adds a Good-Thomas prime-factor plan for the 4000-point inverse FFT inside the packed correlate kernel (radix 25, 16, then a fused 2x5x5 last stage). Because the plan has coprime factors, it needs only small twiddle tables (16 + 25 roots) in LDS instead of full mid/last stage tables. Code rows are reordered with a new prime-factor lane order, and the default variant for N=4000 switches to 101. The argmax kernel now also fills peak and test statistic for step two, and a row-maxima dump API is added for verification. The cost is hand-written LDS inline assembly and index maps with scattered outputs.

```diff
diff --git a/gnss-sdr-new_amd/csrc/acq.hip b/gnss-sdr-new_amd/csrc/acq.hip
--- a/gnss-sdr-new_amd/csrc/acq.hip
+++ b/gnss-sdr-new_amd/csrc/acq.hip
@@ -552,6 +552,29 @@
     return GSDR_OK;
 }
 
+int gsdr_acq_dump_row_maxima(gsdr_acq* a, const void* iq_host, float* out_host)
+{
+    GSDR_REQUIRE(a && iq_host && out_host, GSDR_E_ARG, "gsdr_acq_dump_row_maxima: null argument");
+    GSDR_REQUIRE(a->nprn > 0, GSDR_E_STATE, "gsdr_acq_dump_row_maxima: set_local_codes first");
+    GSDR_REQUIRE(a->corr_variant > 0 && !a->general && a->split == 0, GSDR_E_UNSUPPORTED,
+        "gsdr_acq_dump_row_maxima: the handle runs no packed correlate variant");
+    std::lock_guard<std::mutex> lk(a->mu);
+    gsdr::DeviceGuard g(a->device);
+    const AcqView v = view_of(a);
+    GSDR_HIP(hipMemcpyAsync(a->d_iq, iq_host, (size_t)a->consumed * gsdr::item_bytes(a->conf.item_type),
+        hipMemcpyHostToDevice, a->stream));
+    int rc = launch_forward_pk(a, v, a->d_iq, 1, a->consumed, a->stream);
+    if (rc == GSDR_OK) rc = launch_corr_variant(a, v, 1, a->stream);
+    if (rc != GSDR_OK) return rc;
+    GSDR_HIP(hipGetLastError());
+    std::vector<RowStat> st((size_t)v.nprn * v.D);
+    GSDR_HIP(hipMemcpyAsync(st.data(), a->d_stats, st.size() * sizeof(RowStat), hipMemcpyDeviceToHost, a->stream));
+    GSDR_HIP(hipStreamSynchronize(a->stream));
+    for (uint32_t d = 0; d < v.D; ++d)
+        for (uint32_t p = 0; p < v.nprn; ++p) out_host[(size_t)d * v.nprn + p] = st[(size_t)p * v.D + d].max;
+    return GSDR_OK;
+}
+
 int gsdr_acq_dump_grid_step_two(gsdr_acq* a, const void* iq_host, uint32_t prn_slot, float doppler_center_hz,
     float* grid_host)
 {
diff --git a/gnss-sdr-new_amd/csrc/acq_common.hip b/gnss-sdr-new_amd/csrc/acq_common.hip
--- a/gnss-sdr-new_amd/csrc/acq_common.hip
+++ b/gnss-sdr-new_amd/csrc/acq_common.hip
@@ -199,11 +199,12 @@
 }
 
 __global__ void __launch_bounds__(256) acq_code_lane_order_kernel(const float2* __restrict__ src,
-    float2* __restrict__ dst, uint32_t N, int nb1, int r1)
+    float2* __restrict__ dst, uint32_t N, int nb1, int r1, int pfa)
 {
     const float2* in = src + (size_t)blockIdx.x * N;
     float2* out = dst + (size_t)blockIdx.x * N;
-    for (uint32_t i = threadIdx.x; i < N; i += blockDim.x) out[lane_order_slot((int)i, nb1, r1)] = in[i];
+    for (uint32_t i = threadIdx.x; i < N; i += blockDim.x)
+        out[pfa ? pfa_lane_order_slot((int)i) : lane_order_slot((int)i, nb1, r1)] = in[i];
 }
 
 __global__ void __launch_bounds__(256) acq_grid_second_peak_kernel(const float* __restrict__ grid,
@@ -444,7 +445,7 @@
 {
     const size_t off = (size_t)first_slot * a->N;
     hipLaunchKernelGGL(acq_code_lane_order_kernel, dim3(nslots), dim3(256), 0, a->stream, a->d_code_fft + off,
-        a->d_code_lane + off, a->N, a->lane_nb1, a->lane_r1);
+        a->d_code_lane + off, a->N, a->lane_nb1, a->lane_r1, a->lane_pfa);
     GSDR_HIP(hipGetLastError());
     return GSDR_OK;
 }
diff --git a/gnss-sdr-new_amd/csrc/acq_handle.h b/gnss-sdr-new_amd/csrc/acq_handle.h
--- a/gnss-sdr-new_amd/csrc/acq_handle.h
+++ b/gnss-sdr-new_amd/csrc/acq_handle.h
@@ -36,6 +36,7 @@
     int corr_stat{0};
     size_t corr_lds_bytes{0};
     int lane_nb1{0}, lane_r1{0};
+    int lane_pfa{0};
     gsdr::fft::Plan plan{};
     gsdr::fft::Plan4 plan4{};
     size_t lds_bytes{0};
@@ -122,7 +123,7 @@
 {
     switch (N)
         {
-        case 4000: return 99;
+        case 4000: return 101;
         case 16000: return 94;
         case 8000: return 61;
         case 2000: return 62;
diff --git a/gnss-sdr-new_amd/csrc/acq_kernels.h b/gnss-sdr-new_amd/csrc/acq_kernels.h
--- a/gnss-sdr-new_amd/csrc/acq_kernels.h
+++ b/gnss-sdr-new_amd/csrc/acq_kernels.h
@@ -329,6 +329,62 @@
     return true;
 }
 
+constexpr int pfa_lane_order_slot(int i)
+{
+    const int n1 = 21 * i % 32, n2 = 43 * i % 125;
+    return (5 * n1 + n2 % 5) * 25 + n2 / 5;
+}
+template <class MP>
+constexpr bool pfa_lane_order_bijective()
+{
+    for (int i = 0; i < MP::N; ++i)
+        {
+            const int s = pfa_lane_order_slot(i);
+            if (s < 0 || s >= MP::N || MP::first_index(s / MP::R1, s % MP::R1) != i) return false;
+        }
+    return true;
+}
+template <class MP>
+constexpr bool pfa_lane_classes()
+{
+    for (int j = 0; j < MP::NB1; ++j)
+        for (int m = 1; m < MP::R1; ++m)
+            if (MP::first_index(j, m) % MP::NB1 != MP::first_index(j, 0) % MP::NB1) return false;
+    return true;
+}
+template <class MP>
+constexpr bool pfa_slots_chain()
+{
+    for (int j = 0; j < MP::NB2; ++j)
+        {
+            const int e = j / 125, c = j / 25 % 5, k25 = j % 25;
+            for (int r = 0; r < MP::R2; ++r)
+                {
+                    if (MP::middle_slot(j, r) != MP::first_slot(5 * (2 * r + e) + c, k25)) return false;
+                    if (MP::middle_slot(j, r) != MP::last_slot(r, k25, e, c)) return false;
+                    if (MP::middle_slot(j, r) % MP::NB2 != j || MP::middle_slot(j, r) >= MP::N) return false;
+                }
+        }
+    return true;
+}
+template <class MP>
+constexpr bool pfa_outputs_bijective()
+{
+    bool seen[MP::N] = {};
+    for (int j = 0; j < MP::NSL; ++j)
+        for (int r = 0; r < MP::RL; ++r)
+            {
+                const int f = MP::output_index(j % 16, j / 16, r / 5, r % 5);
+                if (f < 0 || f >= MP::N || seen[f]) return false;
+                seen[f] = true;
+            }
+    return true;
+}
+static_assert(pfa_lane_order_bijective<gsdr::pk::PkPfaPlan4000<256>>(), "prime-factor lane order");
+static_assert(pfa_lane_classes<gsdr::pk::PkPfaPlan4000<256>>(), "prime-factor first stage: residue classes mod 160");
+static_assert(pfa_slots_chain<gsdr::pk::PkPfaPlan4000<256>>(), "prime-factor middle stage in place");
+static_assert(pfa_outputs_bijective<gsdr::pk::PkPfaPlan4000<256>>(), "prime-factor output map");
+
 template <class MP, int CS>
 constexpr size_t pk_fft_bytes()
 {
@@ -339,7 +395,8 @@
 enum TwSrc
 {
     kTwGlobal = 0,
-    kTwLds = 1
+    kTwLds = 1,
+    kTwPfa = 2
 };
 
 constexpr int tw_mid_index(int r, int k, int ns2) { return (r - 1) * ns2 + k; }
@@ -355,6 +412,7 @@
 constexpr size_t pk_tw_bytes()
 {
     constexpr int R2 = MP::N / (MP::R1 * MP::RL);
+    if (TW == kTwPfa) return (size_t)(16 + 25) * sizeof(gsdr::pk::c2);
     return (size_t)(tw_mid_elems(TW, R2, MP::R1) + tw_last_elems(TW, MP::NSL)) * sizeof(gsdr::pk::c2);
 }
 template <class MP, int CS, int TW>
@@ -400,6 +458,20 @@
     __device__ __forceinline__ gsdr::pk::c2 last_root(int k) const { return last[k]; }
 };
 
+struct TwPfa
+{
+    const gsdr::pk::c2* t32;
+    const gsdr::pk::c2* t125;
+    __device__ __forceinline__ static void build(gsdr::pk::c2* t32, const float2* __restrict__ tw, int nt)
+    {
+        gsdr::pk::c2* t125 = t32 + 16;
+        for (int k = (int)threadIdx.x; k < 16; k += nt) t32[k] = gsdr::pk::from(tw[125 * k]);
+        for (int k = (int)threadIdx.x; k < 25; k += nt) t125[k] = gsdr::pk::from(tw[32 * k]);
+    }
+    __device__ __forceinline__ gsdr::pk::c2 root32(int k) const { return t32[k]; }
+    __device__ __forceinline__ gsdr::pk::c2 root125(int k) const { return t125[k]; }
+};
+
 template <class MP, int PG, int WPE, int STAT, int CS, int TW = kTwGlobal>
 __global__ void __launch_bounds__(MP::NT) __attribute__((amdgpu_waves_per_eu(WPE))) acq_correlate_pk_kernel(const float2* __restrict__ X,
     const float2* __restrict__ code_fft, RowStat* __restrict__ stats, const float2* __restrict__ tw, uint32_t D,
@@ -407,7 +479,10 @@
 {
     static_assert(PG > 0, "PRN group");
     static_assert(CS == kCodeVgpr || CS == kCodeDirect || CS == kCodeLds || CS == kCodeLane, "code source");
-    static_assert(TW == kTwGlobal || TW == kTwLds, "twiddle source");
+    static_assert(TW == kTwGlobal || TW == kTwLds || TW == kTwPfa, "twiddle source");
+    constexpr bool PFA = MP::PRIME_FACTOR;
+    static_assert(PFA == (TW == kTwPfa), "the prime-factor plan and its tables go together");
+    static_assert(!PFA || (CS == kCodeLane && STAT == 2), "prime-factor plan: lane-order code rows, row maximum only");
     constexpr bool PREFETCH = CS == kCodeVgpr;
     constexpr bool LANE = CS == kCodeLane;
     constexpr bool STAGED = CS == kCodeLds || LANE;
@@ -417,7 +492,7 @@
     static_assert(pk_tw_offset<MP, CS>() >= pk_fft_bytes<MP, CS>() + 2 * (MP::NT / 64) * sizeof(RowStat), "tables behind the scratch");
     static_assert(!TABLES || pk_tw_offset<MP, CS>() % sizeof(gsdr::pk::c2) == 0, "table alignment");
     static_assert(!TABLES || pk_corr_lds_bytes<MP, CS, TW>() <= 40960, "LDS of four workgroups per CU");
-    static_assert(!LANE || (MP::BPT1 == 1 && lane_order_bijective(MP::NB1, MP::R1)), "lane order of the first stage");
+    static_assert(!LANE || (MP::BPT1 == 1 && (PFA || lane_order_bijective(MP::NB1, MP::R1))), "lane order of the first stage");
     constexpr int XT = CS == kCodeLds ? (MP::R1 + 4) / 5 : 0;
     constexpr int RA = LANE ? 5 : 0;
     static_assert(STAT == 1 || STAT == 2, "row statistic 1 (max + sum) or 2 (max)");
@@ -450,10 +525,15 @@
     const uint32_t p0 = g * PG;
     const int np = (int)min((uint32_t)PG, P - p0);
     constexpr int R2 = MP::N / (MP::R1 * MP::RL);
-    using Tws = std::conditional_t<TABLES, TwLds<R2, MP::R1>, gsdr::pk::TwGlobal>;
+    using Tws = std::conditional_t<PFA, TwPfa, std::conditional_t<TABLES, TwLds<R2, MP::R1>, gsdr::pk::TwGlobal>>;
     Tws tws{};
     (void)tws;
-    if constexpr (TABLES)
+    if constexpr (PFA)
+        {
+            tws.t32 = lds + pk_tw_offset<MP, CS>() / sizeof(c2);
+            tws.t125 = tws.t32 + 16;
+        }
+    else if constexpr (TABLES)
         {
             tws.mid = lds + pk_tw_offset<MP, CS>() / sizeof(c2);
             tws.last = tws.mid + tw_mid_elems(TW, R2, MP::R1);
@@ -475,11 +555,25 @@
             if (NB1 % NT == 0 || j0 < NB1)
                 {
                     const int jj = min(j, NB1 - 1);
-#pragma unroll
-                    for (int r = 0; r < R1 - XT; ++r)
+                    if constexpr (PFA)
                         {
-                            xr[bb][r] = bload(xrs, jj * 8, r * NB1 * 8);
-                            if constexpr (PREFETCH) cr[bb][r] = bload(crs, jj * 8, r * NB1 * 8);
+                            int i = MP::first_index(jj, 0);
+#pragma unroll
+                            for (int r = 0; r < R1; ++r)
+                                {
+                                    xr[bb][r] = bload(xrs, i * 8, 0);
+                                    i += NB1;
+                                    i = i >= (int)N ? i - (int)N : i;
+                                }
+                        }
+                    else
+                        {
+#pragma unroll
+                            for (int r = 0; r < R1 - XT; ++r)
+                                {
+                                    xr[bb][r] = bload(xrs, jj * 8, r * NB1 * 8);
+                                    if constexpr (PREFETCH) cr[bb][r] = bload(crs, jj * 8, r * NB1 * 8);
+                                }
                         }
                 }
         }
@@ -497,7 +591,9 @@
     if constexpr (STAGED)
         {
             stage_code(0);
-            if constexpr (TABLES)
+            if constexpr (PFA)
+                Tws::build(lds + pk_tw_offset<MP, CS>() / sizeof(c2), tw, NT);
+            else if constexpr (TABLES)
                 {
                     c2* tmid = lds + pk_tw_offset<MP, CS>() / sizeof(c2);
                     c2* tlast = tmid + tw_mid_elems(TW, R2, MP::R1);
@@ -717,7 +813,7 @@
         }
 }
 
-template <class MP, int STAT>
+template <class MP, int STAT, bool PEAK = false>
 __global__ void __launch_bounds__(MP::NT) acq_argmax_pk_kernel(const float2* __restrict__ X,
     const float2* __restrict__ code_fft, gsdr_acq_result* __restrict__ res, const float2* __restrict__ tw, uint32_t D,
     uint32_t P, float samples_per_code, AcqParams ap)
@@ -758,6 +854,17 @@
             const uint32_t idx = 0xffffffffu - (uint32_t)(key & 0xffffffffu);
             res[bp].code_phase = idx;
             res[bp].acq_delay_samples = (double)fmodf((float)idx, samples_per_code);
+            if constexpr (PEAK)
+                {
+                    const float peak = __uint_as_float((uint32_t)(key >> 32));
+                    res[bp].peak = peak;
+                    if (ap.cfar && ap.step_two)
+                        {
+                            const float stat = peak / res[bp].input_power;
+                            res[bp].test_statistic = stat;
+                            res[bp].positive = stat > ap.threshold ? 1 : 0;
+                        }
+                }
         }
     if constexpr (STAT >= 2)
         {
diff --git a/gnss-sdr-new_amd/csrc/acq_pk.hip b/gnss-sdr-new_amd/csrc/acq_pk.hip
--- a/gnss-sdr-new_amd/csrc/acq_pk.hip
+++ b/gnss-sdr-new_amd/csrc/acq_pk.hip
@@ -10,12 +10,14 @@
 using RegPlan93 = RegFourStep<16, 512, 8, 1 | (16 << 4), NoPads<1000>, 10, 10, 10>;
 using RegPlan94 = RegFourStep<16, 512, 0, 1 | (16 << 4), NoPads<1000>, 10, 10, 10>;
 
-template <int ID, class MP, int PG_, int WPE_, int ST, class REG = void, int CS_ = kCodeVgpr, int TW_ = kTwGlobal>
+template <int ID, class MP, int PG_, int WPE_, int ST, class REG = void, int CS_ = kCodeVgpr, int TW_ = kTwGlobal, class CP = MP>
 struct PkVariant
 {
     static constexpr int id = ID, PG = PG_, WPE = WPE_, STAT = ST, CS = CS_, TW = TW_;
     using type = MP;
     using Reg = REG;
+    using Corr = CP;
+    static constexpr bool PEAK = !std::is_same<CP, MP>::value;
 };
 using PkVariants = PlanList<PkVariant<61, PkPlan<512, true, 20, 20, 20>, 1, 1, 1>,
     PkVariant<62, PkPlan<256, true, 20, 10, 10>, 1, 1, 1>,
@@ -24,7 +26,8 @@
     PkVariant<70, PkPlan<256, 1, 25, 16, 10>, 1, 1, 2>,
     PkVariant<97, PkPlan<256, 1, 25, 16, 10>, 16, 4, 2, void, kCodeLds>,
     PkVariant<98, PkPlan<256, 1, 25, 16, 10>, 16, 4, 2, void, kCodeLane>,
-    PkVariant<99, PkPlan<256, 1, 25, 16, 10>, 16, 4, 2, void, kCodeLane, kTwLds>>;
+    PkVariant<99, PkPlan<256, 1, 25, 16, 10>, 16, 4, 2, void, kCodeLane, kTwLds>,
+    PkVariant<101, PkPlan<256, 1, 25, 16, 10>, 16, 4, 2, void, kCodeLane, kTwPfa, gsdr::pk::PkPfaPlan4000<256>>>;
 
 template <class F>
 int with_pk_variant(int id, F&& f, int unknown = GSDR_E_STATE)
@@ -55,7 +58,7 @@
         else
             {
                 const uint32_t groups = (v.nprn + V::PG - 1) / V::PG;
-                hipLaunchKernelGGL((acq_correlate_pk_kernel<M, V::PG, V::WPE, V::STAT, V::CS, V::TW>), dim3(nblocks * v.D * groups),
+                hipLaunchKernelGGL((acq_correlate_pk_kernel<typename V::Corr, V::PG, V::WPE, V::STAT, V::CS, V::TW>), dim3(nblocks * v.D * groups),
                     dim3(M::NT), a->corr_lds_bytes, s, a->d_X, V::CS == kCodeLane ? v.code_lane : v.code_fft, a->d_stats, a->d_tw, v.D, v.nprn, nblocks,
                     v.xm);
             }
@@ -68,7 +71,7 @@
     return with_pk_variant(a->corr_variant, [&](auto e) {
         using V = decltype(e);
         using M = typename V::type;
-        hipLaunchKernelGGL((acq_argmax_pk_kernel<M, V::STAT>), dim3(nblocks * v.nprn), dim3(M::NT), a->corr_lds_bytes,
+        hipLaunchKernelGGL((acq_argmax_pk_kernel<M, V::STAT, V::PEAK>), dim3(nblocks * v.nprn), dim3(M::NT), a->corr_lds_bytes,
             s, a->d_X, v.code_fft, res, a->d_tw, v.D, v.nprn, a->conf.samples_per_code, params_of(a, v));
         GSDR_HIP(hipGetLastError());
         return GSDR_OK;
@@ -99,9 +102,11 @@
                 gsdr::set_error("correlate variant %d is for N = %d, not %u", V::id, M::N, a->N);
                 return GSDR_E_UNSUPPORTED;
             }
-        a->corr_lds_bytes = pk_corr_lds_bytes<M, V::CS, V::TW>();
-        int rc = set_max_lds((const void*)acq_correlate_pk_kernel<M, V::PG, V::WPE, V::STAT, V::CS, V::TW>, a->corr_lds_bytes);
-        rc |= set_max_lds((const void*)acq_argmax_pk_kernel<M, V::STAT>, a->corr_lds_bytes);
+        using C = typename V::Corr;
+        static_assert(C::N == M::N && C::NT == M::NT && C::lds_bytes() >= M::lds_bytes(), "one size, one workgroup, one allocation");
+        a->corr_lds_bytes = pk_corr_lds_bytes<C, V::CS, V::TW>();
+        int rc = set_max_lds((const void*)acq_correlate_pk_kernel<C, V::PG, V::WPE, V::STAT, V::CS, V::TW>, a->corr_lds_bytes);
+        rc |= set_max_lds((const void*)acq_argmax_pk_kernel<M, V::STAT, V::PEAK>, a->corr_lds_bytes);
         for (int it : kItemTypes)
             rc |= with_item_type(it, [&](auto t) {
                 return set_max_lds((const void*)acq_forward_pk_kernel<M, decltype(t)::value>, M::lds_bytes());
@@ -110,8 +115,9 @@
             rc |= set_max_lds((const void*)acq_correlate_reg_kernel<typename V::Reg>, V::Reg::lds_bytes());
         if (rc != GSDR_OK) return GSDR_E_DEVICE;
         a->corr_variant = V::id;
-        a->lane_nb1 = V::CS == kCodeLane ? M::NB1 : 0;
-        a->lane_r1 = V::CS == kCodeLane ? M::R1 : 0;
+        a->lane_nb1 = V::CS == kCodeLane ? C::NB1 : 0;
+        a->lane_r1 = V::CS == kCodeLane ? C::R1 : 0;
+        a->lane_pfa = V::CS == kCodeLane && C::PRIME_FACTOR ? 1 : 0;
         a->corr_stat = V::STAT;
         return GSDR_OK;
     }, GSDR_OK);
diff --git a/gnss-sdr-new_amd/csrc/fft_pk.h b/gnss-sdr-new_amd/csrc/fft_pk.h
--- a/gnss-sdr-new_amd/csrc/fft_pk.h
+++ b/gnss-sdr-new_amd/csrc/fft_pk.h
@@ -425,6 +425,7 @@
     static constexpr bool TWP = TWP_ != 0;
     static constexpr int N = (Rs * ...);
     static constexpr int nstages = sizeof...(Rs);
+    static constexpr bool PRIME_FACTOR = false;
     static constexpr int R1 = fft::FirstRadix<Rs...>::value;
     static constexpr int BPT1 = fft::bpt_for(R1);
     static constexpr int NB1 = N / R1;
@@ -446,6 +447,131 @@
     }
 };
 
-
-}
-}
+template <int NT_>
+struct PkPfaPlan4000
+{
+    static_assert(NT_ == 256, "160 / 250 / 2 x 200 butterflies on 256 lanes");
+    static constexpr int NT = NT_;
+    static constexpr bool TWP = true;
+    static constexpr int N = 4000;
+    static constexpr int nstages = 3;
+    static constexpr bool PRIME_FACTOR = true;
+    static constexpr int R1 = 25, BPT1 = 1, NB1 = 160;
+    static constexpr int R2 = 16, NB2 = 250;
+    static constexpr int RL = 10, BPTL = 2, NSL = 400, NSLOTS = RL * BPTL;
+    static constexpr size_t lds_bytes() { return (size_t)N * sizeof(c2); }
+    static constexpr int first_index(int j, int m) { return (125 * (j / 5) + 32 * (j % 5) + 160 * m) % N; }
+    static constexpr int first_slot(int j, int k25) { return 25 * j + k25; }
+    static constexpr int middle_slot(int j, int r) { return j + NB2 * r; }
+    static constexpr int last_slot(int k16, int k25, int e, int c) { return 250 * k16 + k25 + 125 * e + 25 * c; }
+    static constexpr int output_index(int k16, int k25, int k2, int k5)
+    {
+        return (2625 * (k16 + 16 * k2) + 1376 * (k25 + 25 * k5)) % N;
+    }
+
+    template <bool ORD = false, bool SKIPW = false, class Load, class Store, class Hook, class Pre, class Mid, class Tws>
+    __device__ __forceinline__ static void run(c2* lds, const float2* __restrict__, Load load, Store store, Hook hook, Pre,
+        Mid mid, Tws tws)
+    {
+        static_assert(!ORD, "the outputs are not visited in index order");
+        static_assert(std::is_same<Pre, NoHook>::value, "no pre() hook: the first stage takes the ordinary write path");
+        const int t = (int)threadIdx.x;
+        {
+            c2 v[R1];
+            const int jj = min(t, NB1 - 1);
+            if (!SKIPW || __builtin_amdgcn_readfirstlane((int)(threadIdx.x & ~63u)) < NB1)
+                {
+#pragma unroll
+                    for (int r = 0; r < R1; ++r) v[r] = load(0, r, first_index(jj, r));
+                }
+            hook();
+            if (t < NB1)
+                {
+                    Dft<R1>::run(v);
+#pragma unroll
+                    for (int r = 0; r < R1; ++r) lds[first_slot(t, r)] = v[r];
+                }
+            __syncthreads();
+        }
+        {
+            c2 v[R2];
+            const int jj = min(t, NB2 - 1);
+#pragma unroll
+            for (int r = 0; r < R2; ++r) v[r] = lds[middle_slot(jj, r)];
+            if (t < NB2)
+                {
+                    Dft<R2>::run(v);
+#pragma unroll
+                    for (int r = 0; r < R2; ++r) lds[middle_slot(t, r)] = v[r];
+                }
+            __syncthreads();
+        }
+        {
+            c2 v[BPTL][RL];
+            c2 w125[BPTL][4];
+            const int k16 = t & 15, k25 = t >> 4;
+            const int k25b = min(k25 + 16, 24);
+            const c2 w32 = tws.root32(k16);
+            w125[0][0] = tws.root125(k25);
+            w125[1][0] = tws.root125(k25b);
+            const unsigned a0 = (unsigned)(uintptr_t)(__attribute__((address_space(3))) void*)(lds + last_slot(k16, k25, 0, 0));
+            const unsigned a1 = (unsigned)(uintptr_t)(__attribute__((address_space(3))) void*)(lds + last_slot(k16, k25b, 0, 0));
+            static_assert(last_slot(0, 0, 0, 1) * 8 == 200 && last_slot(0, 0, 1, 0) * 8 == 1000, "the offsets below");
+#define GSDR_PFA_READS                                                                                           \
+    "ds_read_b64 %0, %10\n\tds_read_b64 %1, %10 offset:200\n\tds_read_b64 %2, %10 offset:400\n\t"              \
+    "ds_read_b64 %3, %10 offset:600\n\tds_read_b64 %4, %10 offset:800\n\tds_read_b64 %5, %10 offset:1000\n\t"  \
+    "ds_read_b64 %6, %10 offset:1200\n\tds_read_b64 %7, %10 offset:1400\n\tds_read_b64 %8, %10 offset:1600\n\t" \
+    "ds_read_b64 %9, %10 offset:1800"
+#define GSDR_PFA_REGS(B)                                                                                         \
+    "=&v"(v[B][0]), "=&v"(v[B][1]), "=&v"(v[B][2]), "=&v"(v[B][3]), "=&v"(v[B][4]), "=&v"(v[B][5]), "=&v"(v[B][6]),  \
+        "=&v"(v[B][7]), "=&v"(v[B][8]), "=&v"(v[B][9])
+            asm volatile(GSDR_PFA_READS : GSDR_PFA_REGS(0) : "v"(a0) : "memory");
+            if (__builtin_amdgcn_readfirstlane((int)(threadIdx.x & ~63u)) < NSL - NT)
+                asm volatile(GSDR_PFA_READS "\n\ts_waitcnt lgkmcnt(0)" : GSDR_PFA_REGS(1) : "v"(a1) : "memory");
+            else
+                asm volatile("s_waitcnt lgkmcnt(0)" ::: "memory");
+#undef GSDR_PFA_READS
+#undef GSDR_PFA_REGS
+#pragma unroll
+            for (int r = 0; r < RL; ++r) asm volatile("" : "+v"(v[0][r]));
+            __syncthreads();
+            mid();
+#pragma unroll
+            for (int b = 0; b < BPTL; ++b)
+                {
+                    if (b == 0 || t < NSL - NT)
+                        {
+                            c2* u = v[b];
+#pragma unroll
+                            for (int c = 0; c < 5; ++c) u[5 + c] = mul(u[5 + c], w32);
+#pragma unroll
+                            for (int c = 0; c < 5; ++c)
+                                {
+                                    const c2 p = u[c], q = u[5 + c];
+                                    u[c] = p + q;
+                                    u[5 + c] = p - q;
+                                }
+                            c2* w = w125[b];
+                            w[1] = mul(w[0], w[0]);
+                            w[2] = mul(w[1], w[0]);
+                            w[3] = mul(w[2], w[0]);
+#pragma unroll
+                            for (int c = 1; c < 5; ++c)
+                                {
+                                    u[c] = mul(u[c], w[c - 1]);
+                                    u[5 + c] = mul(u[5 + c], w[c - 1]);
+                                }
+                            Dft<5>::run(u);
+                            Dft<5>::run(u + 5);
+                            const int kk = k25 + 16 * b;
+#pragma unroll
+                            for (int r = 0; r < RL; ++r) store(output_index(k16, kk, r / 5, r % 5), u[r], r * BPTL + b);
+                        }
+                }
+        }
+    }
+};
+
+
+}
+}
diff --git a/gnss-sdr-new_amd/gsdr/__init__.py b/gnss-sdr-new_amd/gsdr/__init__.py
--- a/gnss-sdr-new_amd/gsdr/__init__.py
+++ b/gnss-sdr-new_amd/gsdr/__init__.py
@@ -45,6 +45,7 @@
     "gsdr_stream_wait_landed",
     "gsdr_stream_read", "gsdr_firdes_low_pass", "gsdr_acq_resampler_plan", "gsdr_decim_create", "gsdr_decim_destroy",
     "gsdr_decim_output", "gsdr_decim_advance", "gsdr_acq_get_plan", "gsdr_acq_get_split",
+    "gsdr_acq_dump_row_maxima",
 ]
 
 WIPE_EXACT, WIPE_GENERIC, WIPE_AVX2 = 0, 1, 2
@@ -229,6 +230,8 @@
     L.gsdr_acq_run_device.argtypes = [P, P, U32, U64, U64, P, P]
     L.gsdr_acq_dump_grid.argtypes = [P, P, U32, P]
     L.gsdr_acq_dump_grid_step_two.argtypes = [P, P, U32, ctypes.c_float, P]
+    if hasattr(L, "gsdr_acq_dump_row_maxima"):
+        L.gsdr_acq_dump_row_maxima.argtypes = [P, P, P]
     L.gsdr_acq_read_profile_intervals.argtypes = [P, P, ctypes.c_int, P, P, U32, P]
     L.gsdr_acq_set_wipeoff.argtypes = [P, ctypes.c_int]
     L.gsdr_acq_get_spectrum_reuse.argtypes = [P, P, P]
@@ -520,6 +523,12 @@
         _check(load().gsdr_acq_dump_grid(self._h, _ptr(iq), int(prn_slot), _ptr(g)))
         return g
 
+    def dump_row_maxima(self, iq):
+        iq = self._items(iq)
+        m = np.zeros((self.num_doppler_bins, self.nprn), np.float32)
+        _check(load().gsdr_acq_dump_row_maxima(self._h, _ptr(iq), _ptr(m)))
+        return m
+
     def dump_grid_step_two(self, iq, prn_slot, doppler_center_hz):
         iq = self._items(iq)
         g = np.zeros((self._st2_bins, self.fft_size), np.float32)
diff --git a/include/gsdr.h b/include/gsdr.h
--- a/include/gsdr.h
+++ b/include/gsdr.h
@@ -133,6 +133,7 @@
 int gsdr_acq_collect(gsdr_acq* acq, gsdr_acq_result* out_host, uint32_t* nblocks, uint32_t* nprn);
 
 int gsdr_acq_dump_grid(gsdr_acq* acq, const void* iq_host, uint32_t prn_slot, float* grid_host);
+int gsdr_acq_dump_row_maxima(gsdr_acq* acq, const void* iq_host, float* out_host);
 int gsdr_acq_dump_grid_step_two(gsdr_acq* acq, const void* iq_host, uint32_t prn_slot, float doppler_center_hz,
     float* grid_host);
 
```

Result: faster. 296.7 Msamples/s, median of 6 (+8.7%).
